# gorgonia/agogo

Measured on AMD Instinct MI355X. Metric: mcts_sims_per_sec, higher is better.
Workload: dtype f32 (Winograd F(5x5,3x3): fp32 transforms; transform-domain products as fp16x2 = each fp32 operand scaled by a power of two and split into 2 fp16 pieces (22-23 significand bits, absolute error <= 2^-38 of the tensor range), 3 fp16 MFMAs per product, fp32 accumulate)

## Files before the change

### agogo_amd/capi.py

```python
import ctypes as C
import os

import numpy as np

_HERE = os.path.dirname(os.path.abspath(__file__))
_LIB = None

NONE, BLACK, WHITE = 0, 1, 2
PASS, RESIGN = -1, -2
NO_MOVE = -32768
GAME_MNK, GAME_C4, GAME_KOMI, GAME_WQ = 0, 1, 2, 3
ENC_TWOPLANE, ENC_WQ = 0, 1
INF_NET, INF_DUMMY, INF_SCRIPT, INF_HASH, INF_UNIFORM, INF_CALLBACK = 0, 1, 2, 3, 4, 5
BN_DEGENERATE_EPS, BN_RUNNING, BN_IDENTITY = 0, 1, 2
COMPUTE_F32_MFMA, COMPUTE_BF16X3, COMPUTE_FP16X2, COMPUTE_WINO, COMPUTE_AUTO, COMPUTE_WINO_H2 = 0, 1, 2, 3, 4, 5
COMPUTE_FORCE = 0x100
LOSS_REFERENCE, LOSS_ALPHAZERO = 0, 1
PATH_FWD_F32, PATH_FWD_BF16X3, PATH_FWD_H2W, PATH_FWD_H2DMA, PATH_FWD_H2DMA3 = 1, 2, 3, 4, 5
PATH_WGRAD_F32, PATH_WGRAD_X3, PATH_WGRAD_H2, PATH_WGRAD_H2T3 = 1, 2, 3, 4
PATH_DGRAD_RAW, PATH_DGRAD_X3, PATH_DGRAD_WINO_H2 = 1, 2, 3
PATH_BN2_SCALAR, PATH_BN2_V = 1, 2
ROWS_WGRAD_CHUNKS, ROWS_SINGLE_PASS, ROWS_APPLY_RPB, ROWS_BWD2_RPB = 0, 1, 2, 3
ROWS_APPLY_BOARD_WORDS, ROWS_BWD2_BOARD_WORDS, ROWS_SPLIT_BLOCKS, ROWS_SPLIT_NEED = 4, 5, 6, 7
ROWS_HEAD_SECOND_FORM, ROWS_HEAD_CONV2_GRID, ROWS_HEAD_STATS_GRID, ROWS_HEAD_COST_GRID = 0, 1, 2, 3
# ... 148 lines not shown
    sig("agz_net_set_param", i32, vp, i32, pf, C.c_size_t)
    sig("agz_net_get_param", i32, vp, i32, pf, C.c_size_t)
    sig("agz_net_set_bn_stats", i32, vp, i32, pf, pf, C.c_size_t)
    sig("agz_net_init_random", i32, vp, u64)
    sig("agz_net_commit", i32, vp)
    sig("agz_net_infer", i32, vp, pf, i32, pf, pf)
    sig("agz_net_infer_dev", i32, vp, vp, i32, vp, vp)
    sig("agz_host_alloc", i32, vp, C.c_size_t, pvp)
    sig("agz_host_free", i32, vp, vp)
    sig("agz_mcts_to_dot", i32, vp, i32, C.c_char_p, C.c_size_t, C.POINTER(C.c_size_t))
    sig("agz_mcts_set_timeout_ms", i32, vp, i32)
    sig("agz_mcts_last_simulations", i32, vp, C.POINTER(C.c_int64))
    sig("agz_net_set_latency_mode", i32, vp, i32)
    sig("agz_net_set_tower_queues", i32, vp, i32)
    sig("agz_net_set_compute_mode", i32, vp, i32)
    sig("agz_net_flops_per_eval", f64, vp)
    sig("agz_net_save", i32, vp, C.c_char_p)
    sig("agz_net_load", i32, vp, C.c_char_p)
    sig("agz_arena_get_results", i32, vp, C.POINTER(C.c_int64), C.POINTER(C.c_int64), C.POINTER(C.c_int64))
    sig("agz_trainer_create", i32, vp, C.POINTER(NetConf), pvp)
    sig("agz_trainer_create_tied", i32, vp, C.POINTER(NetConf), pvp)
    sig("agz_trainer_is_tied", i32, vp, C.POINTER(i32))
    sig("agz_trainer_destroy", None, vp)
    sig("agz_trainer_num_params", i32, vp)
    sig("agz_trainer_param_info", i32, vp, i32, C.c_char_p, C.c_size_t, C.POINTER(C.c_size_t))
    sig("agz_trainer_set_param", i32, vp, i32, pf, C.c_size_t)
    sig("agz_trainer_get_param", i32, vp, i32, pf, C.c_size_t)
    sig("agz_trainer_get_grad", i32, vp, i32, pf, C.c_size_t)
    sig("agz_trainer_init_random", i32, vp, u64)
    sig("agz_trainer_batch", i32, vp, pf, pf, pf, C.c_float, pf)
    sig("agz_trainer_forward_backward", i32, vp, pf, pf, pf, pf)
    sig("agz_trainer_forward_backward_dev", i32, vp, vp, vp, vp, pf)
    sig("agz_trainer_apply", i32, vp, C.c_float, C.c_float)
    sig("agz_trainer_grads_dev", i32, vp, pvp, C.POINTER(C.c_size_t))
    sig("agz_trainer_set_solver", i32, vp, C.POINTER(SolverConf))
    sig("agz_trainer_get_solver", i32, vp, C.POINTER(SolverConf))
    sig("agz_trainer_get_velocity", i32, vp, i32, pf, C.c_size_t)
    sig("agz_trainer_set_velocity", i32, vp, i32, pf, C.c_size_t)
    sig("agz_trainer_reset_solver", i32, vp)
    sig("agz_trainer_set_adam", i32, vp, C.POINTER(AdamConf))
    sig("agz_trainer_get_adam", i32, vp, C.POINTER(AdamConf), C.POINTER(C.c_uint64))
    sig("agz_trainer_get_moments", i32, vp, i32, pf, pf, C.c_size_t)
    sig("agz_trainer_set_moments", i32, vp, i32, pf, pf, C.c_size_t)
    sig("agz_trainer_set_bn_tracking", i32, vp, i32, C.c_float)
    sig("agz_trainer_get_bn_tracking", i32, vp, C.POINTER(C.c_int), C.POINTER(C.c_float), C.POINTER(C.c_double))
    sig("agz_trainer_num_bn", i32, vp)
    sig("agz_trainer_get_bn_stats", i32, vp, i32, pf, pf, C.c_size_t)
    sig("agz_trainer_set_bn_stats", i32, vp, i32, pf, pf, C.c_size_t, C.c_double)
    sig("agz_trainer_reset_bn_stats", i32, vp)
    sig("agz_trainer_eval", i32, vp, pf, pf, pf, pf)
    sig("agz_trainer_eval_dev", i32, vp, vp, vp, vp, pf)
    sig("agz_trainer_set_loss", i32, vp, i32)
    sig("agz_trainer_get_loss", i32, vp, C.POINTER(C.c_int))
    sig("agz_trainer_get_costs", i32, vp, pf, pf)
    sig("agz_trainer_set_compute_mode", i32, vp, i32)
    sig("agz_train", i32, vp, pf, pf, pf, i32, i32, u64, pf)
    sig("agz_trainer_export", i32, vp, vp)
    sig("agz_trainer_save", i32, vp, C.c_char_p)
    sig("agz_trainer_load", i32, vp, C.c_char_p)
    sig("agz_arena_create", i32, vp, C.POINTER(GameConf), C.POINTER(MctsConf), i32, u64, i32, pvp)
    sig("agz_arena_destroy", None, vp)
    sig("agz_arena_set_inferencer", i32, vp, i32, i32, vp)
    sig("agz_arena_reset", i32, vp, pu8)
    sig("agz_arena_play", i32, vp, i32, i32)
    sig("agz_arena_selfplay", i32, vp, C.c_int64, i32)
    sig("agz_arena_set_parallel", i32, vp, i32)
    sig("agz_arena_set_leaf_symmetry", i32, vp, i32, u64)
    sig("agz_mcts_set_leaf_symmetry", i32, vp, i32, u64)
    sig("agz_symmetry_map", i32, i32, i32, pi)
    sig("agz_symmetry_inverse", i32, i32)
    sig("agz_leaf_symmetry_of", i32, u64, pi, i32, i32, C.POINTER(C.c_int))
    sig("agz_examples_augment_dihedral", i32, vp)
    sig("agz_symmetry_boards", i32, vp, pf, i32, i32, i32, pf)
    pnc, pu64 = C.POINTER(NoiseConf), C.POINTER(C.c_uint64)
    sig("agz_arena_set_root_noise", i32, vp, pnc)
    sig("agz_arena_get_root_noise", i32, vp, pnc)
    sig("agz_arena_root_noise", i32, vp, i32, i32, pu64, pi, pf, i32, C.POINTER(C.c_int))
    sig("agz_mcts_set_root_noise", i32, vp, pnc)
    sig("agz_mcts_root_noise", i32, vp, pu64, pi, pf, i32, C.POINTER(C.c_int))
    sig("agz_root_noise_of", i32, u64, i32, C.c_float, pf)
    ppc, pi32, pi64 = C.POINTER(PlayoutCapConf), C.POINTER(C.c_int32), C.POINTER(C.c_int64)
    sig("agz_arena_set_playout_cap", i32, vp, ppc)
    sig("agz_arena_get_playout_cap", i32, vp, ppc)
    sig("agz_arena_playout_cap", i32, vp, i32, pu64, pi32, pi32, pi32)
    sig("agz_arena_playout_cap_counts", i32, vp, pi64, pi64)
    sig("agz_playout_cap_of", i32, u64, u64, C.c_int32, C.c_float, pi32)
    pfc, pu8, pu32 = C.POINTER(ForcedConf), C.POINTER(C.c_uint8), C.POINTER(C.c_uint32)
    sig("agz_arena_set_forced_playouts", i32, vp, pfc)
    sig("agz_arena_get_forced_playouts", i32, vp, pfc)
    sig("agz_root_select_of", i32, pu32, pf, pf, pu8, i32, i32, C.c_float, C.c_float, C.POINTER(C.c_int), C.POINTER(C.c_int))
    sig("agz_pruned_target_of", i32, pi, pu32, pf, pf, i32, i32, i32, C.c_float, C.c_float, C.c_float, pu32, pf)
    ptc = C.POINTER(TargetConf)
    sig("agz_arena_set_policy_target", i32, vp, ptc)
    sig("agz_arena_get_policy_target", i32, vp, ptc)
    sig("agz_visit_target_of", i32, pi, C.POINTER(C.c_uint32), i32, i32, C.c_float, pf)
    sig("agz_arena_begin_move", i32, vp)
    sig("agz_arena_simulate", i32, vp, i32)
    sig("agz_arena_end_move", i32, vp, i32)
    sig("agz_arena_apply_moves", i32, vp, pi)
    sig("agz_arena_get_stats", i32, vp, C.POINTER(ArenaStats))
    sig("agz_arena_get_game", i32, vp, i32, pi, C.POINTER(GameState))
    sig("agz_arena_get_history", i32, vp, i32, pi, i32, pi)
    sig("agz_arena_root_children", i32, vp, i32, i32, pi, pu, pf, pf, i32, pi)
    sig("agz_arena_tree_nodes", i32, vp, i32, i32, pi)
    sig("agz_arena_get_examples", i32, vp, pf, pf, pf, pi, i32, pi)
    sig("agz_arena_clear_examples", i32, vp)
    sig("agz_arena_drop_labelled_examples", i32, vp)
    sig("agz_arena_examples_dev", i32, vp, pvp, pvp, pvp, pi)
    i64, pi64 = C.c_int64, C.POINTER(C.c_int64)
    sig("agz_train_dev", i32, vp, vp, vp, vp, i32, i32, u64, pf)
    sig("agz_examples_create", i32, vp, i32, i32, i32, i32, pvp)
    sig("agz_examples_destroy", None, vp)
    sig("agz_examples_count", i32, vp, pi64)
    sig("agz_examples_clear", i32, vp)
    sig("agz_examples_append_arena", i32, vp, vp)
    sig("agz_examples_append_dev", i32, vp, vp, vp, vp, i64)
    sig("agz_examples_append_host", i32, vp, pf, pf, pf, i64)
    sig("agz_examples_get", i32, vp, pf, pf, pf, i64, pi64)
    sig("agz_examples_augment_rotate", i32, vp)
    sig("agz_examples_prepare", i32, vp, i32, i32, u64, pi)
    sig("agz_examples_tensors_dev", i32, vp, pvp, pvp, pvp, pi64, pi)
    sig("agz_examples_get_tensors", i32, vp, pf, pf, pf)
    sig("agz_examples_raw_dev", i32, vp, pvp, pvp, pvp)
    sig("agz_replay_create", i32, vp, i32, i32, i32, i32, i64, pvp)
    sig("agz_replay_create_packed", i32, vp, i32, i32, i32, i32, i64, pf, i32, pvp)
    sig("agz_encoder_palette", i32, i32, pf, pi)
    sig("agz_replay_pack_host", i32, pf, i64, i32, i32, pf, i32, pu, pi64)
    sig("agz_replay_storage", i32, vp, pi, pi64, pi64)
    sig("agz_replay_destroy", None, vp)
    sig("agz_replay_count", i32, vp, pi64, C.POINTER(C.c_uint64), pi64)
    sig("agz_replay_clear", i32, vp)
    sig("agz_replay_append_examples", i32, vp, vp)
    sig("agz_replay_append_dev", i32, vp, vp, vp, vp, i64)
    sig("agz_replay_append_host", i32, vp, pf, pf, pf, i64)
    sig("agz_replay_get", i32, vp, i64, i64, pf, pf, pf)
    sig("agz_replay_sample_dev", i32, vp, i32, u64, u64, i32, vp, vp, vp)
    sig("agz_replay_sample", i32, vp, i32, u64, u64, i32, pf, pf, pf)
    sig("agz_replay_draw", i32, u64, u64, i32, i64, i32, pi64, pi)
    sig("agz_train_replay", i32, vp, vp, i32, u64, i32, pf)
    sig("agz_replay_sample_slice_dev", i32, vp, i32, i32, i32, u64, u64, i32, vp, vp, vp)
    sig("agz_replay_sample_slice", i32, vp, i32, i32, i32, u64, u64, i32, pf, pf, pf)
    sig("agz_replay_digest", i32, vp, C.POINTER(C.c_uint64))
    sig("agz_replay_digest_host", i32, pf, pf, pf, i64, i32, i32, i32, C.POINTER(C.c_uint64))
    sig("agz_replay_save", i32, vp, C.c_char_p)
    sig("agz_replay_load", i32, vp, C.c_char_p)
    sig("agz_replay_set_ckpt_staging", i32, vp, C.c_size_t)
    sig("agz_train_replay_sharded", i32, vp, vp, i32, u64, i32, i32, pf)
    sig("agz_rotate_boards", i32, vp, pf, i32, i32, i32, pf)
    sig("agz_ctx_prof_set_stride", i32, vp, i32, i32)
    sig("agz_wino_stages", i32, vp, pf, pf, i32, i32, i32, i32, i32, pf, pf)
    sig("agz_wino_h2_tile", i32, i32, i32)
    sig("agz_net_set_wino_h2_form", i32, vp, i32)
    sig("agz_net_set_wino_h2_gemm", i32, vp, i32)
    sig("agz_net_wino_h2_last_rows", i32, vp, C.POINTER(C.c_int), C.POINTER(C.c_int))
    sig("agz_net_last_paths", i32, vp, C.POINTER(C.c_int), C.POINTER(C.c_int), C.POINTER(C.c_int))
    sig("agz_net_tower_out", i32, vp, i32, pf)
    sig("agz_net_min_same_batch", i32, vp, i32, i32, C.POINTER(C.c_int))
    sig("agz_arena_set_prep_compact", i32, vp, i32)
    sig("agz_arena_set_split", i32, vp, i32)
    sig("agz_arena_split_steps", i32, vp, C.POINTER(C.c_int64), C.POINTER(C.c_int64), C.POINTER(C.c_int))
    sig("agz_trainer_set_dma_forward", i32, vp, i32)
    sig("agz_trainer_last_paths", i32, vp, i32, C.POINTER(C.c_int), C.POINTER(C.c_int), C.POINTER(C.c_int), C.POINTER(C.c_int))
    sig("agz_trainer_last_rows", i32, vp, i32, C.POINTER(C.c_int32))
    sig("agz_trainer_last_planes", i32, vp, i32, C.POINTER(C.c_int), C.POINTER(C.c_uint32), C.POINTER(C.c_uint32))
    sig("agz_arena_last_prep_batch", i32, vp, C.POINTER(C.c_int), C.POINTER(C.c_int))
    sig("agz_arena_set_cap_compact", i32, vp, i32)
    sig("agz_arena_last_cap_batch", i32, vp, C.POINTER(C.c_int), C.POINTER(C.c_int))
    sig("agz_arena_debug_counter", i32, vp, i32, C.POINTER(C.c_int64))
    sig("agz_arena_pool_capacity", i32, vp, C.POINTER(C.c_int), C.POINTER(C.c_int))
    sig("agz_wino_h2_chained", i32, i32, i32, i32)
    sig("agz_arena_random_moves", i32, vp, pi, u64)
    sig("agz_arena_set_state", i32, vp, i32, C.POINTER(State))
    sig("agz_arena_save", i32, vp, C.c_char_p)
    sig("agz_arena_load", i32, vp, C.c_char_p)
    sig("agz_arena_set_ckpt_staging", i32, vp, C.c_size_t)
    sig("agz_arena_examples_labelled_dev", i32, vp, pvp)
    sig("agz_mcts_create", i32, vp, C.POINTER(GameConf), C.POINTER(MctsConf), u64, i32, pvp)
    sig("agz_mcts_destroy", None, vp)
    sig("agz_mcts_set_inferencer", i32, vp, i32, vp)
    sig("agz_mcts_set_inferencer_callback", i32, vp, INFER_FN, vp, i32)
    sig("agz_arena_set_inferencer_callback", i32, vp, i32, INFER_FN, vp, i32)
    sig("agz_arena_set_pool_policy", i32, vp, i32)
    sig("agz_mcts_set_pool_policy", i32, vp, i32)
    sig("agz_mcts_set_parallel", i32, vp, i32)
    sig("agz_mcts_set_game", i32, vp, C.POINTER(State))
    sig("agz_mcts_search", i32, vp, i32, pi)
    sig("agz_mcts_policies", i32, vp, pf, i32)
    sig("agz_mcts_root_children", i32, vp, pi, pu, pf, pf, i32, pi)
    sig("agz_mcts_nodes", i32, vp, pi)
    sig("agz_mcts_children", i32, vp, i32, pi, pi, pu, pf, pf, i32, pi)
    sig("agz_mcts_get_stats", i32, vp, C.POINTER(ArenaStats))
    sig("agz_mcts_reset", i32, vp)
    sig("agz_comm_init_all", i32, pvp, i32, pvp)
    sig("agz_comm_unique_id", i32, vp)
    sig("agz_comm_init_rank", i32, vp, i32, i32, vp, pvp)
    sig("agz_comm_destroy", None, vp)
    sig("agz_comm_rank", i32, vp)
    sig("agz_comm_size", i32, vp)
    sig("agz_examples_allgather", i32, vp, vp)
    sig("agz_trainer_allreduce", i32, vp, vp)
    sig("agz_trainer_forward_backward_allreduce", i32, vp, vp, pf, pf, pf, pf)
    sig("agz_trainer_forward_backward_allreduce_dev", i32, vp, vp, vp, vp, vp, pf)
    sig("agz_comm_debug_fail_slice", i32, vp, i32)
    sig("agz_trainer_create_sharded", i32, vp, C.POINTER(NetConf), pvp)
    sig("agz_trainer_create_sharded_tied", i32, vp, C.POINTER(NetConf), pvp)
    sig("agz_trainer_shard", i32, vp, C.POINTER(i32), C.POINTER(i32), C.POINTER(i32))
    sig("agz_comm_debug_fail_layer", i32, vp, i32)
    _LIB = L
    return L


def _check(r, what=""):
    if r != 0:
        raise AgzError("%s failed (%d): %s" % (what, r, lib().agz_last_error().decode(errors="replace")))


def _pf(a):
    return a.ctypes.data_as(C.POINTER(C.c_float))


def _pi(a):
    return a.ctypes.data_as(C.POINTER(C.c_int32))


class Ctx:
    def __init__(self, device=0):
        self.h = C.c_void_p()
        self._children = []
        _check(lib().agz_ctx_create(device, C.byref(self.h)), "agz_ctx_create")

    def _adopt(self, child):
        import weakref
        self._children.append(weakref.ref(child))

    def close(self):
        if self.h:
            kids = [r() for r in self._children]
            for k in sorted([k for k in kids if k is not None], key=lambda k: 0 if isinstance(k, Arena) else 1):
                k.close()
            self._children = []
            for p in list(getattr(self, "_pinned", {}).values()):
                lib().agz_host_free(self.h, C.c_void_p(p))
            self._pinned = {}
            lib().agz_ctx_destroy(self.h)
            self.h = C.c_void_p()

    def __del__(self):
        try:
            self.close()
        except Exception:
            pass

    def host_array(self, shape, dtype=np.float32):
        n = int(np.prod(shape)) * np.dtype(dtype).itemsize
        p = C.c_void_p()
        _check(lib().agz_host_alloc(self.h, max(n, 1), C.byref(p)), "agz_host_alloc")
        arr = np.ctypeslib.as_array((C.c_char * max(n, 1)).from_address(p.value)).view(dtype)[: int(np.prod(shape))].reshape(shape)
        self._pinned = getattr(self, "_pinned", {})
        self._pinned[arr.ctypes.data] = p.value
        return arr

    def host_free(self, arr):
        p = getattr(self, "_pinned", {}).pop(arr.ctypes.data, None)
        if p is not None and self.h:
            _check(lib().agz_host_free(self.h, C.c_void_p(p)), "agz_host_free")

    def sync(self):
        _check(lib().agz_ctx_sync(self.h), "agz_ctx_sync")

    def stream(self):
        return lib().agz_ctx_stream(self.h)

    def prof_enable(self, on=True, classes=None):
        if on and classes is not None:
            mask = 0
            for k in classes:
                mask |= 1 << (k + 1)
            _check(lib().agz_ctx_prof_enable(self.h, mask), "agz_ctx_prof_enable")
            return
        return self._prof_enable_all(on)

    def prof_set_stride(self, klass, stride):
        _check(lib().agz_ctx_prof_set_stride(self.h, int(klass), int(stride)), "agz_ctx_prof_set_stride")

    def _prof_enable_all(self, on=True):
        _check(lib().agz_ctx_prof_enable(self.h, int(on)), "agz_ctx_prof_enable")

    def prof_read(self, klass):
        n, ms = C.c_int64(0), C.c_double(0)
        _check(lib().agz_ctx_prof_read(self.h, klass, C.byref(n), C.byref(ms)), "agz_ctx_prof_read")
        return n.value, ms.value


class Net:

    def __init__(self, ctx, K, SharedLayers, FC, Width, Height, Features, ActionSpace, BatchSize=256,
                 bn_mode=BN_DEGENERATE_EPS, bn_eps=1e-5):
        self.ctx = ctx
        self.conf = NetConf(K, SharedLayers, FC, BatchSize, Width, Height, Features, ActionSpace, bn_mode, bn_eps)
        self.h = C.c_void_p()
        _check(lib().agz_net_create(ctx.h, C.byref(self.conf), C.byref(self.h)), "agz_net_create")
        ctx._adopt(self)

    def close(self):
        if self.h and self.ctx.h:
            lib().agz_net_destroy(self.h)
        self.h = C.c_void_p()

    def __del__(self):
        try:
            self.close()
        except Exception:
            pass

    def num_params(self):
        return lib().agz_net_num_params(self.h)

    def param_info(self, i):
        name = C.create_string_buffer(128)
        n = C.c_size_t(0)
        _check(lib().agz_net_param_info(self.h, i, name, 128, C.byref(n)), "agz_net_param_info")
        return name.value.decode(), n.value

    def set_param(self, i, v):
        a = np.ascontiguousarray(v, dtype=np.float32).ravel()
        _check(lib().agz_net_set_param(self.h, i, _pf(a), a.size), "agz_net_set_param")

    def get_param(self, i):
        _, n = self.param_info(i)
        a = np.zeros(n, dtype=np.float32)
        _check(lib().agz_net_get_param(self.h, i, _pf(a), a.size), "agz_net_get_param")
        return a

    def set_bn_stats(self, bi, mean, var):
        m = np.ascontiguousarray(mean, dtype=np.float32)
        v = np.ascontiguousarray(var, dtype=np.float32)
        _check(lib().agz_net_set_bn_stats(self.h, bi, _pf(m), _pf(v), m.size), "agz_net_set_bn_stats")

    def init_random(self, seed):
        _check(lib().agz_net_init_random(self.h, seed), "agz_net_init_random")

    def commit(self):
        _check(lib().agz_net_commit(self.h), "agz_net_commit")

    def infer(self, planes):
        c = self.conf
        x = np.ascontiguousarray(planes, dtype=np.float32).reshape(-1, c.Features, c.Height, c.Width)
        B = x.shape[0]
        pol = np.zeros((B, c.ActionSpace), dtype=np.float32)
        val = np.zeros(B, dtype=np.float32)
        _check(lib().agz_net_infer(self.h, _pf(x), B, _pf(pol), _pf(val)), "agz_net_infer")
        return pol, val

    def set_compute_mode(self, mode):
        _check(lib().agz_net_set_compute_mode(self.h, int(mode)), "agz_net_set_compute_mode")

    def set_latency_mode(self, on=True):
        _check(lib().agz_net_set_latency_mode(self.h, int(on)), "agz_net_set_latency_mode")

    def set_tower_queues(self, queues):
        _check(lib().agz_net_set_tower_queues(self.h, int(queues)), "agz_net_set_tower_queues")

    def set_wino_h2_form(self, form):
        _check(lib().agz_net_set_wino_h2_form(self.h, int(form)), "agz_net_set_wino_h2_form")

    def set_wino_h2_gemm(self, variant):
        _check(lib().agz_net_set_wino_h2_gemm(self.h, int(variant)), "agz_net_set_wino_h2_gemm")

    def wino_h2_last_rows(self):
        r, c = C.c_int(0), C.c_int(0)
        _check(lib().agz_net_wino_h2_last_rows(self.h, C.byref(r), C.byref(c)), "agz_net_wino_h2_last_rows")
        return r.value, c.value

    def last_paths(self):
        i, b, h = C.c_int(0), C.c_int(0), C.c_int(0)
        _check(lib().agz_net_last_paths(self.h, C.byref(i), C.byref(b), C.byref(h)), "agz_net_last_paths")
        return i.value, b.value, h.value

    def tower_out(self, B):
        c = self.conf
        t = np.zeros((int(B), c.K, c.Height, c.Width), dtype=np.float32)
        _check(lib().agz_net_tower_out(self.h, int(B), _pf(t)), "agz_net_tower_out")
        return t

    def min_same_batch(self, n, G):
        b = C.c_int(0)
        _check(lib().agz_net_min_same_batch(self.h, int(n), int(G), C.byref(b)), "agz_net_min_same_batch")
        return b.value

    def infer_dev(self, planes_ptr, B, policy_ptr, value_ptr):
        _check(lib().agz_net_infer_dev(self.h, C.c_void_p(planes_ptr), B, C.c_void_p(policy_ptr),
                                       C.c_void_p(value_ptr)), "agz_net_infer_dev")

    def flops_per_eval(self):
        return lib().agz_net_flops_per_eval(self.h)

    def save(self, path):
        _check(lib().agz_net_save(self.h, os.fsencode(path)), "agz_net_save")

    def load(self, path):
        _check(lib().agz_net_load(self.h, os.fsencode(path)), "agz_net_load")


class Trainer:

    def __init__(self, ctx, K, SharedLayers, FC, Width, Height, Features, ActionSpace, BatchSize, bn_eps=1e-5, tied=False):
        self.ctx = ctx
        self.conf = NetConf(K, SharedLayers, FC, BatchSize, Width, Height, Features, ActionSpace, 0, bn_eps)
        self.h = C.c_void_p()
        if tied:
            _check(lib().agz_trainer_create_tied(ctx.h, C.byref(self.conf), C.byref(self.h)), "agz_trainer_create_tied")
        else:
            _check(lib().agz_trainer_create(ctx.h, C.byref(self.conf), C.byref(self.h)), "agz_trainer_create")
        ctx._adopt(self)

    def is_tied(self):
        v = C.c_int(0)
        _check(lib().agz_trainer_is_tied(self.h, C.byref(v)), "agz_trainer_is_tied")
        return bool(v.value)

    @classmethod
    def sharded(cls, ctx, comm, K, SharedLayers, FC, Width, Height, Features, ActionSpace, BatchSize, bn_eps=1e-5, tied=False):
        assert comm.ctx is ctx, "the communicator belongs to another context"
        self = cls.__new__(cls)
        self.ctx, self.comm = ctx, comm
        self.conf = NetConf(K, SharedLayers, FC, BatchSize, Width, Height, Features, ActionSpace, 0, bn_eps)
        self.h = C.c_void_p()
        if tied:
            _check(lib().agz_trainer_create_sharded_tied(comm.h, C.byref(self.conf), C.byref(self.h)), "agz_trainer_create_sharded_tied")
        else:
            _check(lib().agz_trainer_create_sharded(comm.h, C.byref(self.conf), C.byref(self.h)), "agz_trainer_create_sharded")
        ctx._adopt(self)
        return self

    def shard(self):
        r0, n, nr = C.c_int(0), C.c_int(0), C.c_int(0)
        _check(lib().agz_trainer_shard(self.h, C.byref(r0), C.byref(n), C.byref(nr)), "agz_trainer_shard")
        return r0.value, n.value, nr.value

    def close(self):
        if self.h and self.ctx.h:
            lib().agz_trainer_destroy(self.h)
        self.h = C.c_void_p()

    def __del__(self):
        try:
            self.close()
        except Exception:
            pass

    def num_params(self):
        return lib().agz_trainer_num_params(self.h)

    def param_info(self, i):
        name = C.create_string_buffer(128)
        n = C.c_size_t(0)
        _check(lib().agz_trainer_param_info(self.h, i, name, 128, C.byref(n)), "agz_trainer_param_info")
        return name.value.decode(), n.value

    def set_param(self, i, v):
        a = np.ascontiguousarray(v, dtype=np.float32).ravel()
        _check(lib().agz_trainer_set_param(self.h, i, _pf(a), a.size), "agz_trainer_set_param")

    def get_param(self, i):
        a = np.zeros(self.param_info(i)[1], np.float32)
        _check(lib().agz_trainer_get_param(self.h, i, _pf(a), a.size), "agz_trainer_get_param")
        return a

    def get_grad(self, i):
        a = np.zeros(self.param_info(i)[1], np.float32)
        _check(lib().agz_trainer_get_grad(self.h, i, _pf(a), a.size), "agz_trainer_get_grad")
        return a

    def init_random(self, seed):
        _check(lib().agz_trainer_init_random(self.h, seed), "agz_trainer_init_random")

    def batch(self, planes, pi, v, lr=0.1):
        x = np.ascontiguousarray(planes, np.float32)
        p = np.ascontiguousarray(pi, np.float32)
        vv = np.ascontiguousarray(v, np.float32)
        c = C.c_float(0)
        _check(lib().agz_trainer_batch(self.h, _pf(x), _pf(p), _pf(vv), lr, C.byref(c)), "agz_trainer_batch")
        return c.value

    def forward_backward(self, planes, pi, v):
        x = np.ascontiguousarray(planes, np.float32)
        p = np.ascontiguousarray(pi, np.float32)
        vv = np.ascontiguousarray(v, np.float32)
        c = C.c_float(0)
        _check(lib().agz_trainer_forward_backward(self.h, _pf(x), _pf(p), _pf(vv), C.byref(c)), "agz_trainer_forward_backward")
        return c.value

    def forward_backward_dev(self, planes_ptr, pi_ptr, v_ptr, want_cost=True):
        c = C.c_float(0)
        _check(lib().agz_trainer_forward_backward_dev(self.h, C.c_void_p(planes_ptr), C.c_void_p(pi_ptr), C.c_void_p(v_ptr),
                                                      C.byref(c) if want_cost else None), "agz_trainer_forward_backward_dev")
        return c.value if want_cost else None

    def apply(self, lr=0.1, grad_scale=1.0):
        _check(lib().agz_trainer_apply(self.h, lr, grad_scale), "agz_trainer_apply")

    def set_solver(self, momentum=0.0, l2reg=0.0, clip=0.0, reserved=0):
        sc = SolverConf(momentum, l2reg, clip, reserved)
        _check(lib().agz_trainer_set_solver(self.h, C.byref(sc)), "agz_trainer_set_solver")

    def get_solver(self):
        sc = SolverConf()
        _check(lib().agz_trainer_get_solver(self.h, C.byref(sc)), "agz_trainer_get_solver")
        return {"momentum": sc.momentum, "l2reg": sc.l2reg, "clip": sc.clip}

    def get_velocity(self, i):
        a = np.zeros(self.param_info(i)[1], np.float32)
        _check(lib().agz_trainer_get_velocity(self.h, i, _pf(a), a.size), "agz_trainer_get_velocity")
        return a

    def set_velocity(self, i, v):
        a = np.ascontiguousarray(v, dtype=np.float32).ravel()
        _check(lib().agz_trainer_set_velocity(self.h, i, _pf(a), a.size), "agz_trainer_set_velocity")

    def reset_solver(self):
        _check(lib().agz_trainer_reset_solver(self.h), "agz_trainer_reset_solver")
# ... 938 lines not shown
```

### agogo_amd/csrc/conv_wino_h2c.hpp

```cpp
#pragma once

__device__ __forceinline__ unsigned h2c_img(int row, int slot) { return maps::h2c_img(row, slot); }

template <int NK, int PFA>
__global__ __launch_bounds__(256, 2) void wino_gemm_h2c_kernel(WinoH2Args h) {
  const WinoArgs& a = h.w;
  constexpr int SA = 128 * 128, SB = 256 * 128;
  __shared__ __attribute__((aligned(16))) unsigned char lds[SA + SB];

  const int n_nt = a.Ntot >> 8;
  const int per_pos = a.n_mtiles * n_nt;
  const int nblk = h.npos * per_pos;
  const int id = blockIdx.x;
  int q = nblk >> 3, rr = nblk & 7, xcd = id & 7, slot = id >> 3;
  int tile = (xcd < rr ? xcd * (q + 1) : rr * (q + 1) + (xcd - rr) * q) + slot;
  const int pos = tile / per_pos;
  const int rem = tile - pos * per_pos;
  const int m_tile = rem / n_nt, n_tile = rem - m_tile * n_nt;

  const int tid = threadIdx.x, lane = tid & 63, wid = tid >> 6;
  const int wm = wid >> 1, wn = wid & 1;
  const unsigned st_lds = h2c_img(tid >> 3, tid & 7);
  const char* abase = reinterpret_cast<const char*>(a.V) + ((size_t)m_tile * h.npos + pos) * (size_t)NK * SA + (size_t)tid * 16;
  const char* bbase = reinterpret_cast<const char*>(h.U2c) + (((size_t)pos * NK) * n_nt + n_tile) * (size_t)SB + (size_t)tid * 16;
// ... 370 lines not shown
  const unsigned m_slot = (unsigned)h.npos * m_pos;
  const unsigned m_lane = (unsigned)((t0 >> 7) - sl0) * m_slot + (unsigned)(((tc & 127) * 64 + pr * 4) * 4);
  const int bpt = 128 / a.TPB;
  auto m_row = [&](int cls, int S) -> unsigned {
    const int idx = maps::rows_row(cls, a.nty, a.ntx, 0, ty, tx);
    if (idx < 0) return 0x80000000u;
    const int p = maps::pack_slot_row(S, bpt, maps::rows_per_board(cls, a.nty, a.ntx), b, idx);
    return (unsigned)((p >> 7) - sl0) * m_slot + (unsigned)(((p & 127) * 64 + pr * 4) * 4);
  };
  const unsigned m_lane_r = h.live_r ? m_row(maps::ROWS_R, h.pk.S_r) : m_lane, m_lane_c = h.live_c ? m_row(maps::ROWS_C, h.pk.S_c) : m_lane;
  auto m_voff = [&](int xi, int nu) -> unsigned {
    const int cls = maps::rows_class(true, true, AL, xi, nu);
    return cls == maps::ROWS_R ? m_lane_r : (cls == maps::ROWS_C ? m_lane_c : m_lane);
  };
  float Y[TM][TM][4];
#pragma unroll
  for (int k = 0; k < TM; k++)
#pragma unroll
    for (int l = 0; l < TM; l++)
#pragma unroll
      for (int e = 0; e < 4; e++) Y[k][l][e] = 0.f;
  float4 m[2][AL];
#pragma unroll
  for (int xi = 0; xi < AL; xi++) m[0][xi] = h2_ldf4(mr, m_voff(xi, 0), (unsigned)(xi * AL) * m_pos);
#pragma unroll
  for (int nu = 0; nu < AL; nu++) {
    if (nu + 1 < AL) {
#pragma unroll
      for (int xi = 0; xi < AL; xi++) m[(nu + 1) & 1][xi] = h2_ldf4(mr, m_voff(xi, nu + 1), (unsigned)(xi * AL + nu + 1) * m_pos);
    }
    float mm[4][AL], oo[4][TM];
#pragma unroll
    for (int xi = 0; xi < AL; xi++) { const float4 v = m[nu & 1][xi]; mm[0][xi] = v.x; mm[1][xi] = v.y; mm[2][xi] = v.z; mm[3][xi] = v.w; }
#pragma unroll
    for (int e = 0; e < 4; e++) wino_atv<TM>(mm[e], oo[e]);
#pragma unroll
    for (int k = 0; k < TM; k++)
#pragma unroll
      for (int e = 0; e < 4; e++) {
        float yl[TM];
#pragma unroll
        for (int l = 0; l < TM; l++) yl[l] = Y[k][l][e];
        wino_at_acc<TM>(nu, yl, oo[e][k]);
#pragma unroll
        for (int l = 0; l < TM; l++) Y[k][l][e] = yl[l];
      }
    __builtin_amdgcn_sched_barrier(0);
  }
  const char* ep = reinterpret_cast<const char*>(a.ep);
  const unsigned e_lane = (unsigned)(32 * s + 2 * pr) * 16u, e_pix = (unsigned)a.Cout_p * 16u;
  float mx = 0.f;
  float* yb = LAST ? a.y + (size_t)b * a.Hp * a.Wp * a.Cout_p + 32 * s + 2 * pr : nullptr;
#pragma unroll
  for (int k = 0; k < TM; k++) {
    const int hh = TM * ty + k, hc = hh < a.H ? hh : a.H - 1;
#pragma unroll
    for (int l = 0; l < TM; l++) {
      const int ww = TM * tx + l, wc = ww < a.W ? ww : a.W - 1;
      const char* e = ep + (size_t)(hc * a.W + wc) * e_pix + e_lane;
      const float4 E0 = *reinterpret_cast<const float4*>(e), E1 = *reinterpret_cast<const float4*>(e + 16);
      float va = (Y[k][l][0] * un0) * E0.x + E0.y, vb = (Y[k][l][1] * un0) * E0.z + E0.w;
      float vc = (Y[k][l][2] * un0) * E1.x + E1.y, vd = (Y[k][l][3] * un0) * E1.z + E1.w;
      va = va > 0.f ? va : 0.f; vb = vb > 0.f ? vb : 0.f; vc = vc > 0.f ? vc : 0.f; vd = vd > 0.f ? vd : 0.f;
      const float y0 = va + vb, y1 = vc + vd;
      if (live && hh < a.H && ww < a.W) {
        if (LAST) *reinterpret_cast<float2*>(yb + ((size_t)(hh + 1) * a.Wp + (ww + 1)) * a.Cout_p) = make_float2(y0, y1);
        else *reinterpret_cast<float2*>(&ys[((size_t)bl * HW + hh * a.W + ww) * 32 + 2 * pr]) = make_float2(y0, y1);
        mx = fmaxf(mx, fmaxf(y0, y1));
      }
    }
    __builtin_amdgcn_sched_barrier(0);
  }
  if (LAST) return;
#pragma unroll
  for (int o = 8; o > 0; o >>= 1) mx = fmaxf(mx, __shfl_xor(mx, o, 64));
  if (pr == 0 && live) h.wm_out[(size_t)t * NS + s] = mx;
  float ax;
  if (h.amax_true) ax = __uint_as_float(reinterpret_cast<const unsigned*>(h.amax_true)[b]);
  else {
    const int wmpb = a.TPB * NS;
    const float* wp = h.wm_prev + (size_t)b * wmpb;
    ax = 0.f;
    for (int i = pr; i < wmpb; i += 16) ax = fmaxf(ax, wp[i]);
#pragma unroll
    for (int o = 8; o > 0; o >>= 1) ax = fmaxf(ax, __shfl_xor(ax, o, 64));
  }
  const float bound = h.g1 * ax + h.g0;
  const unsigned bbits = __float_as_uint(bound);
  if (s == 0 && tt == 0 && pr == 0 && live) h.amax_next[b] = bbits;
  float sb, inv_;
  wino_h2_scales(bbits, WT::VSHIFT, &sb, &inv_);
  __syncthreads();
  const float* yl = ys + (size_t)bl * HW * 32 + 2 * pr;
  float tmx[AL][AL], tmy[AL][AL];
#pragma unroll
  for (int j = 0; j < AL; j++) {
    const int ww = TM * tx + j - 1;
    const bool okx = ww >= 0 && ww < a.W;
    const int wc = ww < 0 ? 0 : (ww < a.W ? ww : a.W - 1);
    float dx[AL], dy[AL], ox[AL], oy[AL];
#pragma unroll
    for (int i = 0; i < AL; i++) {
      const int hh = TM * ty + i - 1;
      const bool ok = okx && hh >= 0 && hh < a.H;
      const int hc = hh < 0 ? 0 : (hh < a.H ? hh : a.H - 1);
      const float2 d = *reinterpret_cast<const float2*>(yl + (size_t)(hc * a.W + wc) * 32);
      dx[i] = ok ? d.x : 0.f; dy[i] = ok ? d.y : 0.f;
    }
    wino_btv<TM>(dx, ox);
    wino_btv<TM>(dy, oy);
#pragma unroll
    for (int i = 0; i < AL; i++) { tmx[i][j] = ox[i]; tmy[i][j] = oy[i]; }
  }
  const float sv = live ? sb : 0.f;
  const __amdgpu_buffer_rsrc_t vr = h2_rsrc(reinterpret_cast<const char*>(a.V) + ((size_t)(t0 >> 7) * h.npos * NS + s) * 16384);
  const unsigned v_lane = (unsigned)(((t0 & 127) + (tid >> 6) * 4) * 128 + lane * 4);
  const unsigned v_pos = (unsigned)NS * 16384u;
#pragma unroll
  for (int i = 0; i < AL; i++) {
    float ox[AL], oy[AL];
    wino_btv<TM>(tmx[i], ox);
    wino_btv<TM>(tmy[i], oy);
#pragma unroll
    for (int j = 0; j < AL; j++) {
      unsigned lo;
      const unsigned hi = wino_h2_pack(ox[j] * sv, oy[j] * sv, &lo);
      const auto s16 = __builtin_amdgcn_permlane16_swap(hi, lo, false, false);
      const unsigned e0 = s16[0], e1 = s16[1];
      const auto s32 = __builtin_amdgcn_permlane32_swap(e0, e1, false, false);
      const unsigned w0 = s32[0], w1 = s32[1];
      __builtin_amdgcn_raw_buffer_store_b32(w0, vr, v_lane, (unsigned)(i * AL + j) * v_pos, 0);
      __builtin_amdgcn_raw_buffer_store_b32(w1, vr, v_lane + 256u, (unsigned)(i * AL + j) * v_pos, 0);
    }
  }
}

typedef float f2c __attribute__((ext_vector_type(2)));
template <int TM> __device__ __forceinline__ void wino_atv_p(const f2c* m, f2c* o);
template <> __device__ __forceinline__ void wino_atv_p<4>(const f2c* m, f2c* o) {
  const f2c s12 = m[1] + m[2], d12 = m[1] - m[2], s34 = m[3] + m[4], d34 = m[3] - m[4];
  o[0] = m[0] + s12 + s34;
  o[1] = d12 + 2.f * d34;
  o[2] = s12 + 4.f * s34;
  o[3] = d12 + 8.f * d34 + m[5];
}
template <> __device__ __forceinline__ void wino_atv_p<5>(const f2c* m, f2c* o) {
  const f2c s12 = m[1] + m[2], d12 = m[1] - m[2], s34 = m[3] + m[4], d34 = m[3] - m[4];
  o[0] = m[0] + s12 + s34 + m[5];
  o[1] = d12 + 0.5f * d34 + 2.f * m[5];
  o[2] = s12 + 0.25f * s34 + 4.f * m[5];
  o[3] = d12 + 0.125f * d34 + 8.f * m[5];
  o[4] = s12 + 0.0625f * s34 + 16.f * m[5] + m[6];
}
template <int TM> __device__ __forceinline__ void wino_at_acc_p(int nu, f2c* Y, f2c t);
template <> __device__ __forceinline__ void wino_at_acc_p<5>(int nu, f2c* Y, f2c t) {
  switch (nu) {
    case 0: Y[0] += t; break;
    case 1: Y[0] += t; Y[1] += t; Y[2] += t; Y[3] += t; Y[4] += t; break;
    case 2: Y[0] += t; Y[1] -= t; Y[2] += t; Y[3] -= t; Y[4] += t; break;
    case 3: Y[0] += t; Y[1] += 0.5f * t; Y[2] += 0.25f * t; Y[3] += 0.125f * t; Y[4] += 0.0625f * t; break;
    case 4: Y[0] += t; Y[1] -= 0.5f * t; Y[2] += 0.25f * t; Y[3] -= 0.125f * t; Y[4] += 0.0625f * t; break;
    case 5: Y[0] += t; Y[1] += 2.f * t; Y[2] += 4.f * t; Y[3] += 8.f * t; Y[4] += 16.f * t; break;
    default: Y[4] += t; break;
  }
}
template <> __device__ __forceinline__ void wino_at_acc_p<4>(int nu, f2c* Y, f2c t) {
  switch (nu) {
    case 0: Y[0] += t; break;
    case 1: Y[0] += t; Y[1] += t; Y[2] += t; Y[3] += t; break;
    case 2: Y[0] += t; Y[1] -= t; Y[2] += t; Y[3] -= t; break;
    case 3: Y[0] += t; Y[1] += 2.f * t; Y[2] += 4.f * t; Y[3] += 8.f * t; break;
    case 4: Y[0] += t; Y[1] -= 2.f * t; Y[2] += 4.f * t; Y[3] -= 8.f * t; break;
    default: Y[3] += t; break;
  }
}
template <int TM> __device__ __forceinline__ f2c wino_bt_row_p(int i, const f2c* d);
template <> __device__ __forceinline__ f2c wino_bt_row_p<5>(int i, const f2c* d) {
  switch (i) {
    case 0: return -0.5f * d[0] + 0.25f * d[1] + 2.5f * d[2] - 1.25f * d[3] - 2.f * d[4] + d[5];
    case 1: return 0.5f * d[1] + 0.25f * d[2] - 2.25f * d[3] - d[4] + d[5];
    case 2: return -0.5f * d[1] + 0.75f * d[2] + 1.75f * d[3] - 3.f * d[4] + d[5];
    case 3: return d[1] + 1.5f * d[2] - 2.f * d[3] - 1.5f * d[4] + d[5];
    case 4: return -d[1] + 2.5f * (d[2] - d[4]) + d[5];
    case 5: return 0.25f * d[1] - 1.25f * d[3] + d[5];
    default: return -0.5f * d[1] + 0.25f * d[2] + 2.5f * d[3] - 1.25f * d[4] - 2.f * d[5] + d[6];
  }
}
template <> __device__ __forceinline__ f2c wino_bt_row_p<4>(int i, const f2c* d) {
  switch (i) {
    case 0: return 4.f * d[0] - 5.f * d[2] + d[4];
    case 1: return -4.f * d[1] - 4.f * d[2] + d[3] + d[4];
    case 2: return 4.f * d[1] - 4.f * d[2] - d[3] + d[4];
    case 3: return -2.f * d[1] - d[2] + 2.f * d[3] + d[4];
    case 4: return 2.f * d[1] - d[2] - 2.f * d[3] + d[4];
    default: return 4.f * d[1] - 5.f * d[3] + d[5];
  }
}
template <int TM> __device__ __forceinline__ void wino_btv_p(const f2c* d, f2c* o) {
#pragma unroll
  for (int i = 0; i < TM + 2; i++) o[i] = wino_bt_row_p<TM>(i, d);
}

template <int TM, bool NT = true>
__global__ __launch_bounds__(256, 2) void wino_oip_h2c_kernel(WinoH2Args h) {
  constexpr int MAUX = 0, VAUX = NT ? 2 : 0;
  using WT = WinoT<TM>;
  constexpr int AL = WT::AL, NPRE = AL - 3;
  const WinoArgs& a = h.w;
  extern __shared__ __attribute__((aligned(16))) float ys[];
  const int tid = threadIdx.x, tl = tid >> 4, pr = tid & 15, lane = tid & 63;
  const int NS = a.C >> 5;
  const int PH = TM * a.nty + 2, PW = TM * a.ntx + 2;
  const int bpg = 16 / a.TPB;
  const int n_groups = (a.T + 15) >> 4, n_items = n_groups * NS;
  const int tt = tl % a.TPB, bl = tl / a.TPB;
  const int ty = tt / a.ntx, tx = tt - ty * a.ntx;
  for (int i = tid; i < bpg * PH * PW * 32; i += 256) ys[i] = 0.f;
  const __amdgpu_buffer_rsrc_t mr = h2_rsrc(a.Mb);
  const __amdgpu_buffer_rsrc_t vr = h2_rsrc(a.V);
  const unsigned m_lane = (unsigned)((tl * 64 + pr * 4) * 4);
  const unsigned v_lane = (unsigned)((((tid >> 6) * 4) * 128) + lane * 4);
  const unsigned e_pix = (unsigned)a.Cout_p * 16u;
  constexpr unsigned OOB = 0x80000000u;
  const int S_r = h.pk.S_r, S_c = h.pk.S_c;
  const unsigned m_dq = (unsigned)(h.npos * NS - 1) * 32768u, v_dq = (unsigned)(h.npos * NS - 1) * 16384u;
  const unsigned gr_r = h.live_r ? (unsigned)(bpg * maps::rows_per_board(maps::ROWS_R, a.nty, a.ntx)) : 16u;
  const unsigned gr_c = h.live_c ? (unsigned)(bpg * maps::rows_per_board(maps::ROWS_C, a.nty, a.ntx)) : 16u;
  auto m_row = [&](int cls) -> unsigned {
    const int r = maps::rows_row(cls, a.nty, a.ntx, bl, ty, tx);
    return r < 0 ? OOB : (unsigned)((r * 64 + pr * 4) * 4);
  };
  auto v_row = [&](int cls, int k) -> unsigned {
    const int tv = (tid >> 6) * 4 + 2 * k + (lane >> 5), ttv = tv % a.TPB;
    const int r = maps::rows_row(cls, a.nty, a.ntx, tv / a.TPB, ttv / a.ntx, ttv % a.ntx);
    return r < 0 ? OOB : (unsigned)(r * 128 + (lane & 31) * 4);
  };
  const unsigned m_lane_r = h.live_r ? m_row(maps::ROWS_R) : m_lane, m_lane_c = h.live_c ? m_row(maps::ROWS_C) : m_lane;
  const unsigned v0_r = h.live_r ? v_row(maps::ROWS_R, 0) : v_lane, v1_r = h.live_r ? v_row(maps::ROWS_R, 1) : v_lane + 256u;
  const unsigned v0_c = h.live_c ? v_row(maps::ROWS_C, 0) : v_lane, v1_c = h.live_c ? v_row(maps::ROWS_C, 1) : v_lane + 256u;
  float* const ybase = ys + ((size_t)bl * PH * PW + (size_t)(TM * ty) * PW + TM * tx) * 32 + 2 * pr;
  unsigned okmask = 0;
#pragma unroll
  for (int k = 0; k < TM; k++)
#pragma unroll
    for (int l = 0; l < TM; l++) okmask |= (TM * ty + k < a.H && TM * tx + l < a.W) ? 1u << (k * TM + l) : 0u;
  const __amdgpu_buffer_rsrc_t er = h2_rsrc(a.ep);
  float4 m[NPRE][AL];
  auto m_soff = [&](int g, int s, int xi, int nu) -> unsigned {
    const int cls = maps::rows_class(true, true, AL, xi, nu);
    const unsigned gr = cls == maps::ROWS_R ? gr_r : (cls == maps::ROWS_C ? gr_c : 16u);
    const int S = cls == maps::ROWS_R ? S_r : (cls == maps::ROWS_C ? S_c : 1);
    return (unsigned)(((maps::pack_group_slot0(S, g) * h.npos + xi * AL + nu) * NS + s)) * 32768u + maps::pack_group_rg0(S, g, gr) * 256u;
  };
  auto m_voff = [&](int g, int xi, int nu) -> unsigned {
    const int cls = maps::rows_class(true, true, AL, xi, nu);
    if (cls == maps::ROWS_R) return m_lane_r + maps::pack_q(S_r, maps::pack_group_rg0(S_r, g, gr_r), m_lane_r, 8) * m_dq;
    if (cls == maps::ROWS_C) return m_lane_c + maps::pack_q(S_c, maps::pack_group_rg0(S_c, g, gr_c), m_lane_c, 8) * m_dq;
    return m_lane;
  };
  int item = blockIdx.x;
  {
    const int g = __builtin_amdgcn_readfirstlane(item / NS), s = __builtin_amdgcn_readfirstlane(item - (item / NS) * NS);
#pragma unroll
    for (int nu = 0; nu < NPRE; nu++)
#pragma unroll
      for (int xi = 0; xi < AL; xi++) m[nu][xi] = h2_ldf4<MAUX>(mr, m_voff(g, xi, nu), m_soff(g, s, xi, nu));
  }
  __syncthreads();
  for (; item < n_items; item += gridDim.x) {
    const int g = __builtin_amdgcn_readfirstlane(item / NS), s = __builtin_amdgcn_readfirstlane(item - (item / NS) * NS);
    const int t = g * 16 + tl;
    const bool live = t < a.T;
    const int b = live ? g * bpg + bl : (a.T - 1) / a.TPB;
    float s_, un0;
    wino_h2_scales(h.amax_in[b], WT::VSHIFT, &s_, &un0);
    f2c Y[TM][TM][2];
#pragma unroll
    for (int k = 0; k < TM; k++)
#pragma unroll
      for (int l = 0; l < TM; l++) { Y[k][l][0] = f2c{0.f, 0.f}; Y[k][l][1] = f2c{0.f, 0.f}; }
#pragma unroll
    for (int nu = 0; nu < AL; nu++) {
      f2c c0[AL], c1[AL], o0[TM], o1[TM];
#pragma unroll
      for (int xi = 0; xi < AL; xi++) {
        const float4 v = m[nu % NPRE][xi];
        c0[xi] = f2c{v.x, v.y}; c1[xi] = f2c{v.z, v.w};
      }
      if (nu + NPRE < AL) {
#pragma unroll
        for (int xi = 0; xi < AL; xi++) m[nu % NPRE][xi] = h2_ldf4<MAUX>(mr, m_voff(g, xi, nu + NPRE), m_soff(g, s, xi, nu + NPRE));
      }
      wino_atv_p<TM>(c0, o0);
      wino_atv_p<TM>(c1, o1);
#pragma unroll
      for (int k = 0; k < TM; k++) {
        f2c y0[TM], y1[TM];
#pragma unroll
        for (int l = 0; l < TM; l++) { y0[l] = Y[k][l][0]; y1[l] = Y[k][l][1]; }
        wino_at_acc_p<TM>(nu, y0, o0[k]);
        wino_at_acc_p<TM>(nu, y1, o1[k]);
#pragma unroll
        for (int l = 0; l < TM; l++) { Y[k][l][0] = y0[l]; Y[k][l][1] = y1[l]; }
      }
      __builtin_amdgcn_sched_barrier(0);
    }
    __builtin_amdgcn_sched_barrier(0);
    unsigned e_base = (unsigned)(32 * s + 2 * pr) * 16u + (unsigned)((TM * ty) * a.W + TM * tx) * e_pix;
    asm volatile("" : "+v"(e_base));
    float4 E[2][TM][2];
    auto load_e = [&](int buf, int k) {
#pragma unroll
      for (int l = 0; l < TM; l++) {
        const bool ok = (okmask >> (k * TM + l)) & 1u;
        const unsigned off = e_base + (ok ? (unsigned)(k * a.W + l) * e_pix : 0u);
        E[buf][l][0] = h2_ldf4(er, off, 0);
        E[buf][l][1] = h2_ldf4(er, off + 16u, 0);
      }
    };
    load_e(0, 0);
    float mxv = 0.f;
    float* yw = ybase;
    asm volatile("" : "+v"(yw));
#pragma unroll
    for (int k = 0; k < TM; k++) {
      if (k + 1 < TM) load_e((k + 1) & 1, k + 1);
#pragma unroll
      for (int l = 0; l < TM; l++) {
        const bool ok = live && ((okmask >> (k * TM + l)) & 1u);
        const float4 E0 = E[k & 1][l][0], E1 = E[k & 1][l][1];
        const f2c u0 = Y[k][l][0] * un0, u1 = Y[k][l][1] * un0;
        float va = u0.x * E0.x + E0.y, vb = u0.y * E0.z + E0.w;
        float vc = u1.x * E1.x + E1.y, vd = u1.y * E1.z + E1.w;
        va = va > 0.f ? va : 0.f; vb = vb > 0.f ? vb : 0.f; vc = vc > 0.f ? vc : 0.f; vd = vd > 0.f ? vd : 0.f;
        const float y0 = ok ? va + vb : 0.f, y1 = ok ? vc + vd : 0.f;
        *reinterpret_cast<float2*>(yw + ((k + 1) * PW + l + 1) * 32) = make_float2(y0, y1);
        mxv = fmaxf(mxv, fmaxf(y0, y1));
      }
      __builtin_amdgcn_sched_barrier(0);
    }
#pragma unroll
    for (int o = 8; o > 0; o >>= 1) mxv = fmaxf(mxv, __shfl_xor(mxv, o, 64));
    if (pr == 0 && live) h.wm_out[(size_t)t * NS + s] = mxv;
    float ax;
    if (h.amax_true) ax = __uint_as_float(reinterpret_cast<const unsigned*>(h.amax_true)[b]);
    else {
      const int wmpb = a.TPB * NS;
      const float* wp = h.wm_prev + (size_t)b * wmpb;
      ax = 0.f;
      for (int i = pr; i < wmpb; i += 16) ax = fmaxf(ax, wp[i]);
#pragma unroll
      for (int o = 8; o > 0; o >>= 1) ax = fmaxf(ax, __shfl_xor(ax, o, 64));
    }
    const float bound = h.g1 * ax + h.g0;
    const unsigned bbits = __float_as_uint(bound);
    if (s == 0 && tt == 0 && pr == 0 && live) h.amax_next[b] = bbits;
    float sb, inv_;
    wino_h2_scales(bbits, WT::VSHIFT, &sb, &inv_);
    const float sv = live ? sb : 0.f;
    __syncthreads();
    {
      const int nx = item + (int)gridDim.x < n_items ? item + (int)gridDim.x : item;
      const int g2 = __builtin_amdgcn_readfirstlane(nx / NS), s2 = __builtin_amdgcn_readfirstlane(nx - (nx / NS) * NS);
#pragma unroll
      for (int nu = 0; nu < NPRE; nu++)
#pragma unroll
        for (int xi = 0; xi < AL; xi++) m[nu][xi] = h2_ldf4<MAUX>(mr, m_voff(g2, xi, nu), m_soff(g2, s2, xi, nu));
    }
    __builtin_amdgcn_sched_barrier(0);
    const unsigned v_pos = (unsigned)NS * 16384u;
    const unsigned v_slot = (unsigned)h.npos * v_pos;
    const unsigned rg0_r = maps::pack_group_rg0(S_r, g, gr_r), rg0_c = maps::pack_group_rg0(S_c, g, gr_c);
    const unsigned v_g = (unsigned)(g >> 3) * v_slot + (unsigned)s * 16384u + (unsigned)(g & 7) * 2048u;
    const unsigned v_g_r = maps::pack_group_slot0(S_r, g) * v_slot + (unsigned)s * 16384u + rg0_r * 128u;
    const unsigned v_g_c = maps::pack_group_slot0(S_c, g) * v_slot + (unsigned)s * 16384u + rg0_c * 128u;
    auto v_voff = [&](int cls, int k) -> unsigned {
      if (cls == maps::ROWS_R) { const unsigned o = k ? v1_r : v0_r; return o + maps::pack_q(S_r, rg0_r, o, 7) * v_dq; }
      if (cls == maps::ROWS_C) { const unsigned o = k ? v1_c : v0_c; return o + maps::pack_q(S_c, rg0_c, o, 7) * v_dq; }
      return k ? v_lane + 256u : v_lane;
    };
    const float* yr = ybase;
    asm volatile("" : "+v"(yr));
#pragma unroll
    for (int i0 = 0; i0 < AL; i0 += 3) {
      constexpr int NRMAX = 3;
      const int nr = AL - i0 < NRMAX ? AL - i0 : NRMAX;
      f2c tmr[NRMAX][AL];
#pragma unroll
      for (int j = 0; j < AL; j++) {
        f2c d[AL];
#pragma unroll
        for (int ii = 0; ii < AL; ii++) {
          const float2 v = *reinterpret_cast<const float2*>(yr + (ii * PW + j) * 32);
          d[ii] = f2c{v.x, v.y};
        }
#pragma unroll
        for (int r = 0; r < NRMAX; r++)
          if (r < nr) tmr[r][j] = wino_bt_row_p<TM>(i0 + r, d);
      }
      __builtin_amdgcn_sched_barrier(0);
#pragma unroll
      for (int r = 0; r < NRMAX; r++) {
        if (r >= nr) continue;
        const int i = i0 + r;
        f2c o[AL];
        wino_btv_p<TM>(tmr[r], o);
#pragma unroll
        for (int j = 0; j < AL; j++) {
          unsigned lo;
          const unsigned hi = wino_h2_pack(o[j].x * sv, o[j].y * sv, &lo);
          const auto s16 = __builtin_amdgcn_permlane16_swap(hi, lo, false, false);
          const unsigned e0 = s16[0], e1 = s16[1];
          const auto s32 = __builtin_amdgcn_permlane32_swap(e0, e1, false, false);
          const unsigned w0 = s32[0], w1 = s32[1];
          const int cls = maps::rows_class(true, true, AL, i, j);
          const unsigned v_so = (cls == maps::ROWS_R ? v_g_r : (cls == maps::ROWS_C ? v_g_c : v_g)) + (unsigned)(i * AL + j) * v_pos;
          __builtin_amdgcn_raw_buffer_store_b32(w0, vr, v_voff(cls, 0), v_so, VAUX);
          __builtin_amdgcn_raw_buffer_store_b32(w1, vr, v_voff(cls, 1), v_so, VAUX);
        }
      }
      __builtin_amdgcn_sched_barrier(0);
    }
    __syncthreads();
  }
}

static void wino_build_u2c(const std::vector<_Float16>& u2, std::vector<_Float16>& u2c, int npos, int Ntot, int C, int Cout_p) {
  const int NC = C / 32, NT = Ntot / 256;
  u2c.assign(u2.size(), (_Float16)0.f);
  for (int pos = 0; pos < npos; pos++)
    for (int kc = 0; kc < NC; kc++)
      for (int nn = 0; nn < Ntot; nn++) {
        const int s = nn >> 6, j2 = nn & 63, ch = 32 * s + (j2 >> 1), br = j2 & 1, n = br * Cout_p + ch;
        for (int p = 0; p < 2; p++) {
          const _Float16* src = &u2[((((size_t)pos * NC + kc) * 2 + p) * Ntot + n) * 32];
          _Float16* dst = &u2c[((((size_t)pos * NC + kc) * NT + (nn >> 8)) * 256 + (nn & 255)) * 64 + p * 32];
          for (int k = 0; k < 32; k++) dst[k] = src[k];
        }
      }
}

static inline bool wino_h2c_ok(int H, int W, int tm, int Kp) {
  const int tpb = ceil_div(H, tm) * ceil_div(W, tm);
  const int nk = Kp / 32;
  return Kp % 128 == 0 && 16 % tpb == 0 && (nk == 4 || nk == 8 || nk == 12 || nk == 16) &&
         (size_t)(16 / tpb) * (tm * ceil_div(H, tm) + 2) * (tm * ceil_div(W, tm) + 2) * 128 <= 80 * 1024;
}

static void wino_h2c_geometry(WinoH2Args& h) {
  WinoArgs& a = h.w;
  const int tm = h.tm == 5 ? 5 : 4;
  h.tm = tm; h.npos = (tm + 2) * (tm + 2);
  a.nty = ceil_div(a.H, tm); a.ntx = ceil_div(a.W, tm); a.TPB = a.nty * a.ntx; a.T = a.B * a.TPB;
  h.rsh = 7; h.rmask = 127; h.rA = (unsigned)h.npos * 128u; h.rB = 128u;
  a.n_mtiles = ceil_div(a.T, 128); a.n_ntiles = ceil_div(a.Ntot, 128);
  h.in_swap = 1; h.cform = 1; h.wm_per_board = 0;
  h.pk = maps::pack_grid(tm + 2, a.nty, a.ntx, a.B, a.Ntot >> 8, h.live_r, h.live_c);
}
static int wino_h2c_gemm_tiles(const WinoH2Args& h) {
  int n = 0;
  for (int pos = 0; pos < h.npos; pos++) n += maps::pack_pos_used(h.pk, pos);
  return n * h.pk.n_nt;
}
constexpr int WINO_H2_GEMM_DEFAULT = 1;
static inline int wino_h2c_gemm_variant(const WinoH2Args& h) { return h.gemm_variant > 0 ? h.gemm_variant : WINO_H2_GEMM_DEFAULT; }
static inline bool wino_h2c_dma_ok(const WinoH2Args& h) {
  return wino_h2_rows(h.npos, (size_t)h.w.T) * h.w.C * 4 < ((size_t)1 << 31) && (size_t)h.npos * h.w.C * h.w.Ntot * 4 < ((size_t)1 << 31);
}
static inline bool wino_h2c_fits31(const WinoH2Args& h) { return wino_h2_rows(h.npos, (size_t)h.w.T) * h.w.Ntot * 4 < ((size_t)1 << 31); }
static bool wino_h2c_oip_ready(agz_ctx* ctx) {
  if (!(ctx->func_attr_state & 2u)) {
    const bool ok = hipFuncSetAttribute(reinterpret_cast<const void*>(&wino_oip_h2c_kernel<5>), hipFuncAttributeMaxDynamicSharedMemorySize, 80 * 1024) == hipSuccess &&
                    hipFuncSetAttribute(reinterpret_cast<const void*>(&wino_oip_h2c_kernel<4>), hipFuncAttributeMaxDynamicSharedMemorySize, 80 * 1024) == hipSuccess;
    if (!ok) (void)hipGetLastError();
    ctx->func_attr_state |= 2u | (ok ? 1u : 0u);
  }
  return (ctx->func_attr_state & 1u) != 0;
}
static void wino_h2c_rows(agz_ctx* ctx, WinoH2Args& h, int oi_variant, bool keep_all) {
  wino_h2c_geometry(h);
  h.live_r = h.live_c = 0;
  const int gemm = wino_h2c_gemm_variant(h) & 15;
  const maps::WinoRows g = maps::wino_rows(h.w.H, h.w.W, h.tm);
  if (keep_all || gemm != 1 || oi_variant != 4 || !wino_h2c_dma_ok(h) || !wino_h2c_fits31(h) || !maps::rows_short_ok(g) || !wino_h2c_oip_ready(ctx)) return;
  h.live_r = g.dead_y ? maps::rows_slot_live(g, maps::ROWS_R) : 0;
  h.live_c = g.dead_x ? maps::rows_slot_live(g, maps::ROWS_C) : 0;
  wino_h2c_geometry(h);
}
static void wino_h2c_in(agz_ctx* ctx, WinoH2Args& h, hipStream_t st) {
  wino_h2c_geometry(h);
  h.fuse_prev = 0; h.amax_self = const_cast<unsigned*>(h.amax_in);
  ProfScopeOn ps(ctx, AGZ_PROF_WINO_IN, st == ctx->stream.raw());
  const size_t n_in = (size_t)h.w.T * (h.w.C / 2);
  if (h.tm == 5) hipLaunchKernelGGL(wino_in_h2_kernel<5>, dim3((unsigned)((n_in + 255) / 256)), dim3(256), 0, st, h);
  else hipLaunchKernelGGL(wino_in_h2_kernel<4>, dim3((unsigned)((n_in + 255) / 256)), dim3(256), 0, st, h);
}
static void wino_h2c_gemm(agz_ctx* ctx, WinoH2Args& h, hipStream_t st) {
  wino_h2c_geometry(h);
  ProfScopeOn ps(ctx, AGZ_PROF_WINO_GEMM, st == ctx->stream.raw());
  const dim3 g(h.npos * h.w.n_mtiles * (h.w.Ntot >> 8));
  const bool dma_ok = wino_h2c_dma_ok(h);
  const int variant_all = wino_h2c_gemm_variant(h);
  const int variant = variant_all & 15, mode = (variant_all >> 4) & 3;
  const int n_slabs = h.w.Ntot >> 7;
  if (variant == 2 && dma_ok && (h.w.C >> 5) == 8 && h.w.Ntot % 256 == 0 && ctx->num_cus / 8 >= n_slabs) {
    const dim3 gp((unsigned)(8 * ((ctx->num_cus / 8) / n_slabs) * n_slabs));
    switch (mode) {
      case 1: hipLaunchKernelGGL(wino_gemm_h2p_kernel<1>, gp, dim3(256), 0, st, h); break;
      case 2: hipLaunchKernelGGL(wino_gemm_h2p_kernel<2>, gp, dim3(256), 0, st, h); break;
      case 3: hipLaunchKernelGGL(wino_gemm_h2p_kernel<3>, gp, dim3(256), 0, st, h); break;
      default: hipLaunchKernelGGL(wino_gemm_h2p_kernel<0>, gp, dim3(256), 0, st, h); break;
    }
    return;
  }
  const dim3 gd((unsigned)wino_h2c_gemm_tiles(h));
  if (dma_ok && h.temporal_stores && (h.w.C >> 5) == 8) { hipLaunchKernelGGL((wino_gemm_h2g_kernel<8, false>), gd, dim3(256), 0, st, h); return; }
  if (dma_ok) {
    switch (h.w.C >> 5) {
      case 4: hipLaunchKernelGGL((wino_gemm_h2g_kernel<4>), gd, dim3(256), 0, st, h); return;
      case 8: hipLaunchKernelGGL((wino_gemm_h2g_kernel<8>), gd, dim3(256), 0, st, h); return;
      case 12: hipLaunchKernelGGL((wino_gemm_h2g_kernel<12>), gd, dim3(256), 0, st, h); return;
      default: hipLaunchKernelGGL((wino_gemm_h2g_kernel<16>), gd, dim3(256), 0, st, h); return;
    }
  }
  switch (h.w.C >> 5) {
    case 4: hipLaunchKernelGGL((wino_gemm_h2c_kernel<4, 2>), g, dim3(256), 0, st, h); break;
    case 8: hipLaunchKernelGGL((wino_gemm_h2c_kernel<8, 2>), g, dim3(256), 0, st, h); break;
    case 12: hipLaunchKernelGGL((wino_gemm_h2c_kernel<12, 2>), g, dim3(256), 0, st, h); break;
    default: hipLaunchKernelGGL((wino_gemm_h2c_kernel<16, 2>), g, dim3(256), 0, st, h); break;
  }
}
static void wino_h2c_oi(agz_ctx* ctx, WinoH2Args& h, bool last, hipStream_t st, int variant = 4) {
  wino_h2c_geometry(h);
  ProfScopeOn ps(ctx, AGZ_PROF_WINO_OUT, st == ctx->stream.raw());
  const WinoArgs& a = h.w;
  const dim3 g((unsigned)ceil_div(a.T, 16), (unsigned)(a.C >> 5));
  const size_t shm = last ? 0 : (size_t)(16 / a.TPB) * a.H * a.W * 32 * sizeof(float);
  const bool fits31 = wino_h2c_fits31(h);
  if (variant == 4 && !last && fits31 && wino_h2c_oip_ready(ctx)) {
    const size_t shp = (size_t)(16 / a.TPB) * (h.tm * a.nty + 2) * (h.tm * a.ntx + 2) * 32 * sizeof(float);
    const int items = ceil_div(a.T, 16) * (a.C >> 5);
    const dim3 gp((unsigned)std::min(items, 2 * ctx->num_cus));
    if (h.tm == 5 && h.temporal_stores) {
      (void)hipFuncSetAttribute(reinterpret_cast<const void*>(&wino_oip_h2c_kernel<5, false>), hipFuncAttributeMaxDynamicSharedMemorySize, 80 * 1024);
      hipLaunchKernelGGL((wino_oip_h2c_kernel<5, false>), gp, dim3(256), shp, st, h);
      return;
    }
    if (h.tm == 5) hipLaunchKernelGGL((wino_oip_h2c_kernel<5>), gp, dim3(256), shp, st, h);
    else hipLaunchKernelGGL((wino_oip_h2c_kernel<4>), gp, dim3(256), shp, st, h);
    return;
  }
  if (h.tm == 5) {
    if (last) hipLaunchKernelGGL((wino_oi_h2c_kernel<5, true>), g, dim3(256), shm, st, h);
    else hipLaunchKernelGGL((wino_oi_h2c_kernel<5, false>), g, dim3(256), shm, st, h);
  } else {
    if (last) hipLaunchKernelGGL((wino_oi_h2c_kernel<4, true>), g, dim3(256), shm, st, h);
    else hipLaunchKernelGGL((wino_oi_h2c_kernel<4, false>), g, dim3(256), shm, st, h);
  }
}
```

### agogo_amd/csrc/conv_x3.hpp

```cpp
#pragma once

typedef short bf16x8_t __attribute__((ext_vector_type(8)));
typedef unsigned u32x4_t __attribute__((ext_vector_type(4)));

__device__ __forceinline__ void x3_split(float v, unsigned& h, unsigned& m, unsigned& l) {
  unsigned hu = __float_as_uint(v) & 0xffff0000u;
  float r = v - __uint_as_float(hu);
  unsigned mu = __float_as_uint(r) & 0xffff0000u;
  float r2 = r - __uint_as_float(mu);
  h = hu; m = mu; l = __float_as_uint(r2);
}
__device__ __forceinline__ unsigned x3_pack(unsigned e0, unsigned e1) { return __builtin_amdgcn_perm(e1, e0, 0x07060302u); }

__device__ __forceinline__ unsigned x3_lds_off(int row, int half) { return (unsigned)(row * 32 + ((half ^ ((row >> 3) & 1)) << 4)); }

__device__ __forceinline__ void x3_amax_flush(unsigned* amax, int b, float m, int lane) {
#pragma unroll
  for (int o = 16; o > 0; o >>= 1) m = fmaxf(m, __shfl_xor(m, o, 64));
  if ((lane & 31) == 0) atomicMax(&amax[b], __float_as_uint(m));
}
#define X3_EPILOGUE \
  int amx_b = -1; float amx_m = 0.f;    \
  _Pragma("unroll") \
  for (int i = 0; i < 2; i++) { \
  _Pragma("unroll") \
    for (int r = 0; r < 16; r++) { \
      int row = (wm * 2 + i) * 32 + (r & 3) + 8 * (r >> 2) + 4 * (lane >> 5); \
      int m = m0 + row; \
      const bool mvalid = m < a.M; \
      if (!mvalid) m = a.M - 1; \
      int b = m / a.HW, p = m - b * a.HW; \
      int h = p / a.W, w = p - h * a.W; \
      size_t obase = ((size_t)b * a.HpWp + (h + 1) * a.Wp + (w + 1)) * a.Cout_p; \
      if (DUAL) { \
        int c = n_tile * (BNT / 2) + wn * 32 + (lane & 31); \
        if (mvalid && c < a.Cout_p) { \
          float4 e = reinterpret_cast<const float4*>(a.ep)[(size_t)p * a.Cout_p + c]; \
          float va = acc[i][0][r] * e.x + e.y; \
          float vb = acc[i][1][r] * e.z + e.w; \
          va = va > 0.f ? va : 0.f; \
          vb = vb > 0.f ? vb : 0.f; \
          float s = va + vb; \
          a.y[obase + c] = s > 0.f ? s : 0.f; \
        } \
      } else { \
        if (a.amax_out && mvalid && b != amx_b) {    \
          if (amx_b >= 0) x3_amax_flush(a.amax_out, amx_b, amx_m, lane); \
          amx_b = b; amx_m = 0.f; \
        } \
  _Pragma("unroll") \
        for (int j = 0; j < 2; j++) { \
          int c = n0 + (wn * 2 + j) * 32 + (lane & 31); \
          if (mvalid && c < a.Cout_p) { \
            if (a.raw) { \
              a.y[obase + c] = acc[i][j][r]; \
            } else { \
              float2 e = reinterpret_cast<const float2*>(a.ep)[(size_t)p * a.Cout_p + c]; \
              float v = acc[i][j][r] * e.x + e.y; \
              v = v > 0.f ? v : 0.f; \
              a.y[obase + c] = v; \
              amx_m = fmaxf(amx_m, v); \
            } \
          } \
        } \
      } \
    } \
  } \
  if (!DUAL && a.amax_out && amx_b >= 0) x3_amax_flush(a.amax_out, amx_b, amx_m, lane);

template <bool DUAL>
__global__ __launch_bounds__(256, 3) void conv3x3_x3_kernel(ConvArgs a, const unsigned short* __restrict__ w3) {
  constexpr int BM = 128, BNT = 128;
  constexpr int PIECE = 128 * 32;
  constexpr int STAGE = 6 * PIECE;
  __shared__ __attribute__((aligned(16))) unsigned char lds[2 * STAGE];

  const int nblk = a.n_mtiles * a.n_ntiles;
  const int id = blockIdx.x;
  int q = nblk >> 3, rr = nblk & 7, xcd = id & 7, slot = id >> 3;
  int tile = (xcd < rr ? xcd * (q + 1) : rr * (q + 1) + (xcd - rr) * q) + slot;
  const int m_tile = tile / a.n_ntiles, n_tile = tile - m_tile * a.n_ntiles;
  const int m0 = m_tile * BM, n0 = n_tile * BNT;

  const int tid = threadIdx.x, lane = tid & 63, wid = tid >> 6;
  const int wm = wid >> 1, wn = wid & 1;

  const int srow = tid >> 1, shalf = tid & 1;
  int a_goff;
  {
    int m = m0 + srow;
    if (m >= a.M) m = a.M - 1;
    int b = m / a.HW, p = m - b * a.HW;
    int h = p / a.W, w = p - h * a.W;
    a_goff = ((b * a.HpWp) + (h + 1) * a.Wp + (w + 1)) * a.Cin_p + shalf * 8;
  }
  int nrow = n0 + srow;
  if (nrow >= a.Ntot) nrow = a.Ntot - 1;
  const int b_goff = nrow * 16 + shalf * 8;
  const size_t piece_stride = (size_t)a.Ntot * 16;
  const unsigned s_off = x3_lds_off(srow, shalf);
  const int NC = a.Cin_p >> 4;
  const int NK = 9 * NC;

  f32x16 acc[2][2];
#pragma unroll
  for (int i = 0; i < 2; i++)
#pragma unroll
    for (int j = 0; j < 2; j++)
#pragma unroll
      for (int r = 0; r < 16; r++) acc[i][j][r] = 0.f;

  unsigned fa[2], fb[2];
#pragma unroll
  for (int i = 0; i < 2; i++) fa[i] = x3_lds_off((wm * 2 + i) * 32 + (lane & 31), lane >> 5);
  if (DUAL) {
    fb[0] = x3_lds_off(wn * 32 + (lane & 31), lane >> 5);
    fb[1] = x3_lds_off(64 + wn * 32 + (lane & 31), lane >> 5);
  } else {
    fb[0] = x3_lds_off((wn * 2 + 0) * 32 + (lane & 31), lane >> 5);
    fb[1] = x3_lds_off((wn * 2 + 1) * 32 + (lane & 31), lane >> 5);
  }

  float4 xa0, xa1, ya0, ya1;
  u32x4_t xb0, xb1, xb2, yb0, yb1, yb2;
  const char* xbase = reinterpret_cast<const char*>(a.x);
  const char* wbase = reinterpret_cast<const char*>(w3);
  const unsigned a_gbyte = (unsigned)a_goff * 4u, b_gbyte = (unsigned)b_goff * 2u;
  const unsigned piece_bytes = (unsigned)(piece_stride * 2);
  int f_kx = 0, f_ky = 0, f_n = 0;
  const unsigned row_step = (unsigned)(a.Cin_p * 4), line_step = (unsigned)((a.Wp - 2) * a.Cin_p * 4);
  const unsigned chunk_back = (unsigned)((2 * a.Wp + 2) * a.Cin_p * 4) - 64u;
  unsigned xo_ = a_gbyte - (unsigned)((a.Wp + 1) * a.Cin_p * 4), wo_ = b_gbyte;
#define X3_ADVANCE()                                                                          \
  if (f_n + 1 < NK) {       \
    f_n++;                                                                                    \
    wo_ += 3u * piece_bytes;                                                                  \
    if (f_kx < 2) { f_kx++; xo_ += row_step; }                                                \
    else if (f_ky < 2) { f_kx = 0; f_ky++; xo_ += line_step; }                                \
    else { f_kx = 0; f_ky = 0; xo_ -= chunk_back; }                                           \
  }
#define X3_GLOAD(A0, A1, B0, B1, B2)                                                          \
  A0 = *reinterpret_cast<const float4*>(xbase + xo_);                                         \
  A1 = *reinterpret_cast<const float4*>(xbase + xo_ + 16u);                                   \
  B0 = *reinterpret_cast<const u32x4_t*>(wbase + wo_);                                        \
  B1 = *reinterpret_cast<const u32x4_t*>(wbase + wo_ + piece_bytes);                          \
  B2 = *reinterpret_cast<const u32x4_t*>(wbase + wo_ + 2u * piece_bytes);                     \
  X3_ADVANCE()
#define X3_STORE_A(A0, A1, BUF)                                                              \
  {                                                                                          \
    unsigned char* st_ = lds + (BUF) * STAGE;                                                \
    const float v_[8] = {A0.x, A0.y, A0.z, A0.w, A1.x, A1.y, A1.z, A1.w};                    \
    unsigned h_[8], m_[8], l_[8];                                                            \
    _Pragma("unroll") for (int e = 0; e < 8; e++) x3_split(v_[e], h_[e], m_[e], l_[e]);      \
    u32x4_t ph_ = {x3_pack(h_[0], h_[1]), x3_pack(h_[2], h_[3]), x3_pack(h_[4], h_[5]), x3_pack(h_[6], h_[7])}; \
    u32x4_t pm_ = {x3_pack(m_[0], m_[1]), x3_pack(m_[2], m_[3]), x3_pack(m_[4], m_[5]), x3_pack(m_[6], m_[7])}; \
    u32x4_t pl_ = {x3_pack(l_[0], l_[1]), x3_pack(l_[2], l_[3]), x3_pack(l_[4], l_[5]), x3_pack(l_[6], l_[7])}; \
    *reinterpret_cast<u32x4_t*>(st_ + 0 * PIECE + s_off) = ph_;                              \
    *reinterpret_cast<u32x4_t*>(st_ + 1 * PIECE + s_off) = pm_;                              \
    *reinterpret_cast<u32x4_t*>(st_ + 2 * PIECE + s_off) = pl_;                              \
  }
#define X3_STORE_B(B0, B1, B2, BUF)                                                          \
  {                                                                                          \
    unsigned char* st_ = lds + (BUF) * STAGE;                                                \
    *reinterpret_cast<u32x4_t*>(st_ + 3 * PIECE + s_off) = B0;                               \
    *reinterpret_cast<u32x4_t*>(st_ + 4 * PIECE + s_off) = B1;                               \
    *reinterpret_cast<u32x4_t*>(st_ + 5 * PIECE + s_off) = B2;                               \
  }
#define X3_SB
#define X3_MF(I, J, PA, PB) acc[I][J] = __builtin_amdgcn_mfma_f32_32x32x16_bf16(A_[I][PA], B_[J][PB], acc[I][J], 0, 0, 0);
#define X3_QUAD(PA, PB) X3_MF(0, 0, PA, PB) X3_MF(0, 1, PA, PB) X3_MF(1, 0, PA, PB) X3_MF(1, 1, PA, PB)
#define X3_ITER(BUF, XA0, XA1, XB0, XB1, XB2, YA0, YA1, YB0, YB1, YB2)                       \
  {                                                                                          \
    const unsigned char* st = lds + (BUF) * STAGE;                                           \
    bf16x8_t A_[2][3], B_[2][3];                                                             \
    _Pragma("unroll") for (int p = 0; p < 3; p++) {                                          \
      _Pragma("unroll") for (int i = 0; i < 2; i++) A_[i][p] = *reinterpret_cast<const bf16x8_t*>(st + p * PIECE + fa[i]);       \
      _Pragma("unroll") for (int j = 0; j < 2; j++) B_[j][p] = *reinterpret_cast<const bf16x8_t*>(st + (3 + p) * PIECE + fb[j]); \
    }                                                                                        \
    X3_SB                                                                                    \
    X3_QUAD(2, 0) X3_SB                                                                      \
    X3_GLOAD(YA0, YA1, YB0, YB1, YB2) X3_SB                                                  \
    X3_QUAD(0, 2) X3_SB                                                                      \
    X3_STORE_A(XA0, XA1, (BUF) ^ 1) X3_SB                                                    \
    X3_QUAD(1, 1) X3_QUAD(1, 0) X3_SB                                                        \
    X3_STORE_B(XB0, XB1, XB2, (BUF) ^ 1) X3_SB                                               \
    X3_QUAD(0, 1) X3_QUAD(0, 0) X3_SB                                                        \
    __syncthreads();                                                                         \
  }

  X3_GLOAD(ya0, ya1, yb0, yb1, yb2)
  X3_GLOAD(xa0, xa1, xb0, xb1, xb2)
  X3_STORE_A(ya0, ya1, 0)
  X3_STORE_B(yb0, yb1, yb2, 0)
  __syncthreads();
  for (int it = 0; it < NK; it += 2) {
    X3_ITER(0, xa0, xa1, xb0, xb1, xb2, ya0, ya1, yb0, yb1, yb2)
    if (it + 1 < NK) X3_ITER(1, ya0, ya1, yb0, yb1, yb2, xa0, xa1, xb0, xb1, xb2)
  }

  X3_EPILOGUE
}
```

### agogo_amd/csrc/net.hip

```cpp
#include "net.hpp"
#include "gemm_maps.hpp"

#include <cmath>
#include <cstdio>
#include <cstring>
#include <type_traits>

typedef float f32x16 __attribute__((ext_vector_type(16)));
typedef float f32x4 __attribute__((ext_vector_type(4)));

namespace agz {

struct ConvArgs {
  const float* x;
  const float* w;
  const void* ep;
  float* y;
  int M, HW, W, Wp, HpWp;
  int Cin_p, Cout_p, Ntot;
  int n_mtiles, n_ntiles;
  int raw;
  int splits;
  int per;
  float* ws;
  const unsigned* amax_in;
  float w_unscale;
  const unsigned* w_amax_dev;
  unsigned* amax_out;
};

__device__ __forceinline__ int swz_off(int row, int chunk) { return row * 32 + ((chunk ^ ((row >> 1) & 7)) << 2); }

template <int WM, int WN, int MT, bool DUAL>
__device__ __forceinline__ void conv_tile(const ConvArgs& a, float* lds, const int m0, const int n_tile, const int split) {
  constexpr int BM = WM * MT * 32;
  constexpr int BNT = WN * 64;
  static_assert(WM * WN == 4, "4 waves");
  constexpr int STAGE = (BM + BNT) * 32;
  const int n0 = n_tile * BNT;

  const int tid = threadIdx.x, lane = tid & 63, wid = tid >> 6;
  const int wm = wid / WN, wn = wid % WN;

  constexpr int A_PER_T = BM * 8 / 256;
  constexpr int B_PER_T = BNT * 8 / 256;
  static_assert((A_PER_T == 4 || A_PER_T == 2) && (B_PER_T == 4 || B_PER_T == 2), "staging layout");
  const int chunk = tid & 7;
  int a_goff[A_PER_T], a_loff[A_PER_T];
#pragma unroll
  for (int i = 0; i < A_PER_T; i++) {
    int row = (tid >> 3) + 32 * i;
    int m = m0 + row;
    if (m >= a.M) m = a.M - 1;
    int b = m / a.HW, p = m - b * a.HW;
    int h = p / a.W, w = p - h * a.W;
    a_goff[i] = ((b * a.HpWp) + (h + 1) * a.Wp + (w + 1)) * a.Cin_p + chunk * 4;
    a_loff[i] = swz_off(row, chunk);
  }
  int b_goff[B_PER_T], b_loff[B_PER_T];
#pragma unroll
  for (int i = 0; i < B_PER_T; i++) {
    int row = (tid >> 3) + 32 * i;
    int n = n0 + row;
    if (n >= a.Ntot) n = a.Ntot - 1;
    b_goff[i] = n * a.Cin_p + chunk * 4;
    b_loff[i] = swz_off(row, chunk);
  }
  const int NC = a.Cin_p >> 5;
  const int NKall = 9 * NC;
  const int it0 = split * a.per;
  const int NK = (it0 + a.per < NKall) ? it0 + a.per : NKall;
  const int w_tap_stride = a.Ntot * a.Cin_p;

  float4 ra0, ra1, ra2, ra3, rb0, rb1, rb2, rb3;
  float4 sa0, sa1, sa2, sa3, sb0, sb1, sb2, sb3;
  int xo_, wo_;
#define AGZ_TILE_OFFS(IT)                                                                   \
  {                                                                                         \
    int t_ = (IT) < NK ? (IT) : NK - 1;                                                     \
    int tap_ = t_ / NC, cc_ = t_ - tap_ * NC;                                               \
    int ky_ = tap_ / 3, kx_ = tap_ - ky_ * 3;                                               \
    xo_ = ((ky_ - 1) * a.Wp + (kx_ - 1)) * a.Cin_p + cc_ * 32;                              \
    wo_ = tap_ * w_tap_stride + cc_ * 32;                                                   \
  }
#define AGZ_GLA(R, I) if constexpr ((I) < A_PER_T) R = *reinterpret_cast<const float4*>(a.x + a_goff[(I) < A_PER_T ? (I) : 0] + xo_);
#define AGZ_GLB(R, I) if constexpr ((I) < B_PER_T) R = *reinterpret_cast<const float4*>(a.w + b_goff[(I) < B_PER_T ? (I) : 0] + wo_);
#define AGZ_LSA(R, I, BUF) if constexpr ((I) < A_PER_T) *reinterpret_cast<float4*>(lds + (BUF) * STAGE + a_loff[(I) < A_PER_T ? (I) : 0]) = R;
#define AGZ_LSB(R, I, BUF) if constexpr ((I) < B_PER_T) *reinterpret_cast<float4*>(lds + (BUF) * STAGE + BM * 32 + b_loff[(I) < B_PER_T ? (I) : 0]) = R;
#define AGZ_SB __builtin_amdgcn_sched_barrier(0);

  f32x16 acc[MT][2];
#pragma unroll
  for (int i = 0; i < MT; i++)
#pragma unroll
    for (int j = 0; j < 2; j++)
#pragma unroll
      for (int r = 0; r < 16; r++) acc[i][j][r] = 0.f;

  int a_row[MT], b_row[2];
#pragma unroll
  for (int i = 0; i < MT; i++) a_row[i] = (wm * MT + i) * 32 + (lane & 31);
  if (DUAL) {
    b_row[0] = wn * 32 + (lane & 31);
    b_row[1] = WN * 32 + wn * 32 + (lane & 31);
  } else {
    b_row[0] = (wn * 2 + 0) * 32 + (lane & 31);
    b_row[1] = (wn * 2 + 1) * 32 + (lane & 31);
  }
  const int khalf = lane >> 5;

  const unsigned lds_base = (unsigned)(size_t)((__attribute__((address_space(3))) float*)lds);
  unsigned a_addr[MT], b_addr[2], a_sw[MT], b_sw[2];
#pragma unroll
  for (int i = 0; i < MT; i++) { a_addr[i] = lds_base + a_row[i] * 128; a_sw[i] = (a_row[i] >> 1) & 7; }
#pragma unroll
  for (int j = 0; j < 2; j++) { b_addr[j] = lds_base + BM * 128 + b_row[j] * 128; b_sw[j] = (b_row[j] >> 1) & 7; }
  f32x4 f0a[MT], f0b[2], f1a[MT], f1b[2];
#pragma unroll
  for (int i = 0; i < MT; i++) { f0a[i] = f32x4{0.f, 0.f, 0.f, 0.f}; f1a[i] = f0a[i]; }
#pragma unroll
  for (int j = 0; j < 2; j++) { f0b[j] = f32x4{0.f, 0.f, 0.f, 0.f}; f1b[j] = f0b[j]; }
#define AGZ_LDSR(DST, ADDR) asm volatile("ds_read_b128 %0, %1" : "+v"(DST) : "v"(ADDR));
#define AGZ_FRAG_READ(AV, BV, KS, BUF)                                                                            \
  {                                                                                                               \
    _Pragma("unroll") for (int i = 0; i < MT; i++) {                                                              \
      unsigned ad_ = a_addr[i] + (BUF) * (STAGE * 4) + (((2 * (KS) + khalf) ^ a_sw[i]) << 4);                     \
      AGZ_LDSR(AV[i], ad_)                                                                                        \
    }                                                                                                             \
    _Pragma("unroll") for (int j = 0; j < 2; j++) {                                                               \
      unsigned ad_ = b_addr[j] + (BUF) * (STAGE * 4) + (((2 * (KS) + khalf) ^ b_sw[j]) << 4);                     \
      AGZ_LDSR(BV[j], ad_)                                                                                        \
    }                                                                                                             \
  }
#define AGZ_WAIT_LGKM(N) asm volatile("s_waitcnt lgkmcnt(%0)" ::"n"(N)); __builtin_amdgcn_sched_barrier(0);
#define AGZ_MQ(AV, BV, C)                                                                                         \
  _Pragma("unroll") for (int i = 0; i < MT; i++) _Pragma("unroll") for (int j = 0; j < 2; j++)                    \
      acc[i][j] = __builtin_amdgcn_mfma_f32_32x32x2f32(AV[i].C, BV[j].C, acc[i][j], 0, 0, 0);
  constexpr int NRD = MT + 2;
  constexpr int NWA = A_PER_T, NWB = B_PER_T;

#define AGZ_ITER(IT, BUF, XA0, XA1, XA2, XA3, XB0, XB1, XB2, XB3, YA0, YA1, YA2, YA3, YB0, YB1, YB2, YB3)         \
  {                                                                                                               \
    AGZ_TILE_OFFS((IT) + 2)                                                                                       \
    AGZ_FRAG_READ(f0a, f0b, 0, BUF)                                                                               \
    AGZ_FRAG_READ(f1a, f1b, 1, BUF)                                                                               \
    AGZ_WAIT_LGKM(NRD)                                                              \
    AGZ_MQ(f0a, f0b, x) AGZ_SB AGZ_GLA(YA0, 0) AGZ_SB AGZ_MQ(f0a, f0b, y) AGZ_SB AGZ_GLA(YA1, 1)                  \
    AGZ_SB AGZ_MQ(f0a, f0b, z) AGZ_SB AGZ_GLA(YA2, 2) AGZ_SB AGZ_MQ(f0a, f0b, w) AGZ_SB AGZ_GLA(YA3, 3)           \
    AGZ_SB AGZ_FRAG_READ(f0a, f0b, 2, BUF)                                                                        \
    AGZ_WAIT_LGKM(NRD)                                                                              \
    AGZ_MQ(f1a, f1b, x) AGZ_SB AGZ_GLB(YB0, 0) AGZ_SB AGZ_MQ(f1a, f1b, y) AGZ_SB AGZ_GLB(YB1, 1)                  \
    AGZ_SB AGZ_MQ(f1a, f1b, z) AGZ_SB AGZ_GLB(YB2, 2) AGZ_SB AGZ_MQ(f1a, f1b, w) AGZ_SB AGZ_GLB(YB3, 3)           \
    AGZ_SB AGZ_FRAG_READ(f1a, f1b, 3, BUF)                                                                        \
    AGZ_WAIT_LGKM(NRD)                                                                              \
    AGZ_MQ(f0a, f0b, x) AGZ_SB AGZ_LSA(XA0, 0, (BUF) ^ 1) AGZ_SB AGZ_MQ(f0a, f0b, y) AGZ_SB AGZ_LSA(XA1, 1, (BUF) ^ 1) \
    AGZ_SB AGZ_MQ(f0a, f0b, z) AGZ_SB AGZ_LSA(XA2, 2, (BUF) ^ 1) AGZ_SB AGZ_MQ(f0a, f0b, w) AGZ_SB AGZ_LSA(XA3, 3, (BUF) ^ 1) \
    AGZ_SB                                                                                                        \
    AGZ_WAIT_LGKM(NWA)                 \
    AGZ_MQ(f1a, f1b, x) AGZ_SB AGZ_LSB(XB0, 0, (BUF) ^ 1) AGZ_SB AGZ_MQ(f1a, f1b, y) AGZ_SB AGZ_LSB(XB1, 1, (BUF) ^ 1) \
    AGZ_SB AGZ_MQ(f1a, f1b, z) AGZ_SB AGZ_LSB(XB2, 2, (BUF) ^ 1) AGZ_SB AGZ_MQ(f1a, f1b, w) AGZ_SB AGZ_LSB(XB3, 3, (BUF) ^ 1) \
    AGZ_SB                                                                                                        \
    __syncthreads();                                                                                              \
  }
  (void)NWB;
  AGZ_TILE_OFFS(it0)
  AGZ_GLA(sa0, 0) AGZ_GLA(sa1, 1) AGZ_GLA(sa2, 2) AGZ_GLA(sa3, 3) AGZ_GLB(sb0, 0) AGZ_GLB(sb1, 1) AGZ_GLB(sb2, 2) AGZ_GLB(sb3, 3)
  AGZ_TILE_OFFS(it0 + 1)
  AGZ_GLA(ra0, 0) AGZ_GLA(ra1, 1) AGZ_GLA(ra2, 2) AGZ_GLA(ra3, 3) AGZ_GLB(rb0, 0) AGZ_GLB(rb1, 1) AGZ_GLB(rb2, 2) AGZ_GLB(rb3, 3)
  AGZ_LSA(sa0, 0, 0) AGZ_LSA(sa1, 1, 0) AGZ_LSA(sa2, 2, 0) AGZ_LSA(sa3, 3, 0) AGZ_LSB(sb0, 0, 0) AGZ_LSB(sb1, 1, 0) AGZ_LSB(sb2, 2, 0) AGZ_LSB(sb3, 3, 0)
  __syncthreads();
  for (int it = it0; it < NK; it += 2) {
    AGZ_ITER(it, 0, ra0, ra1, ra2, ra3, rb0, rb1, rb2, rb3, sa0, sa1, sa2, sa3, sb0, sb1, sb2, sb3)
    if (it + 1 < NK) AGZ_ITER(it + 1, 1, sa0, sa1, sa2, sa3, sb0, sb1, sb2, sb3, ra0, ra1, ra2, ra3, rb0, rb1, rb2, rb3)
  }
#undef AGZ_ITER
#undef AGZ_WAIT_LGKM
#undef AGZ_LDSR
#undef AGZ_MQ
#undef AGZ_FRAG_READ
#undef AGZ_SB
#undef AGZ_LSB
// ... 93 lines not shown

template <bool DUAL>
__global__ __launch_bounds__(256) void splitk_epilogue_kernel(ConvArgs a, int half) {
  const int C4 = a.Cout_p >> 2;
  size_t idx = (size_t)blockIdx.x * blockDim.x + threadIdx.x;
  if (idx >= (size_t)a.M * C4) return;
  int m = (int)(idx / C4), c = ((int)(idx - (size_t)m * C4)) << 2;
  int b = m / a.HW, p = m - b * a.HW;
  int h = p / a.W, w = p - h * a.W;
  float4* out = reinterpret_cast<float4*>(a.y + ((size_t)b * a.HpWp + (h + 1) * a.Wp + (w + 1)) * a.Cout_p + c);
  const size_t sstride = (size_t)a.M * a.Ntot;
  if (DUAL) {
    int ca = (c / half) * 2 * half + (c % half);
    const float* row = a.ws + (size_t)m * a.Ntot + ca;
    float4 sa = {0.f, 0.f, 0.f, 0.f}, sb = {0.f, 0.f, 0.f, 0.f};
#pragma unroll 6
    for (int s = 0; s < a.splits; s++) {
      float4 va = *reinterpret_cast<const float4*>(row + s * sstride);
      float4 vb = *reinterpret_cast<const float4*>(row + s * sstride + half);
      sa.x += va.x; sa.y += va.y; sa.z += va.z; sa.w += va.w;
      sb.x += vb.x; sb.y += vb.y; sb.z += vb.z; sb.w += vb.w;
    }
    const float4* e = reinterpret_cast<const float4*>(a.ep) + (size_t)p * a.Cout_p + c;
    float r[4];
    const float av[4] = {sa.x, sa.y, sa.z, sa.w}, bv[4] = {sb.x, sb.y, sb.z, sb.w};
#pragma unroll
    for (int q = 0; q < 4; q++) {
      float4 eq = e[q];
      float va = av[q] * eq.x + eq.y, vb = bv[q] * eq.z + eq.w;
      va = va > 0.f ? va : 0.f; vb = vb > 0.f ? vb : 0.f;
      float t = va + vb;
      r[q] = t > 0.f ? t : 0.f;
    }
    *out = float4{r[0], r[1], r[2], r[3]};
  } else {
    const float* row = a.ws + (size_t)m * a.Ntot + c;
    float4 sa = {0.f, 0.f, 0.f, 0.f};
#pragma unroll 6
    for (int s = 0; s < a.splits; s++) {
      float4 va = *reinterpret_cast<const float4*>(row + s * sstride);
      sa.x += va.x; sa.y += va.y; sa.z += va.z; sa.w += va.w;
    }
    if (a.raw) { *out = sa; return; }
    const float2* e = reinterpret_cast<const float2*>(a.ep) + (size_t)p * a.Cout_p + c;
    const float av[4] = {sa.x, sa.y, sa.z, sa.w};
    float r[4];
#pragma unroll
    for (int q = 0; q < 4; q++) { float v = av[q] * e[q].x + e[q].y; r[q] = v > 0.f ? v : 0.f; }
    *out = float4{r[0], r[1], r[2], r[3]};
  }
}

__global__ void pack_planes_kernel(const float* __restrict__ planes, float* __restrict__ out, int B, int F, int H, int W,
                                   int Fp) {
  int idx = blockIdx.x * blockDim.x + threadIdx.x;
  int total = B * H * W * Fp;
  if (idx >= total) return;
  int c = idx % Fp;
  int p = idx / Fp;
  int w = p % W, h = (p / W) % H, b = p / (W * H);
  float v = c < F ? planes[((size_t)(b * F + c) * H + h) * W + w] : 0.f;
  out[(((size_t)b * (H + 2) + h + 1) * (W + 2) + w + 1) * Fp + c] = v;
}

struct HeadArgs {
  const float* x;
  const float* conv;
  const float* bn;
  const float* Wp; const float* bp; const float* W1; const float* b1; const float* W2; const float* b2;
  float* policy; float* value;
  int H, W, HW, Wp_, HpWp, Kp, A, FC;
  float* feat;
  float* cols;
};

__device__ __forceinline__ float wave_sum(float v) {
#pragma unroll
  for (int o = 32; o > 0; o >>= 1) v += __shfl_xor(v, o, 64);
  return v;
}

__global__ __launch_bounds__(256) void heads_kernel(HeadArgs a) {
  extern __shared__ float sm[];
  float* feat = sm;
  float* red = sm + 3 * a.HW;
  float* hid = red + 8;
  const int b = blockIdx.x, tid = threadIdx.x, lane = tid & 63, wid = tid >> 6;
  for (int p = wid; p < a.HW; p += 4) {
    int h = p / a.W, w = p - h * a.W;
    const float* xp = a.x + ((size_t)b * a.HpWp + (h + 1) * a.Wp_ + (w + 1)) * a.Kp;
    float s0 = 0.f, s1 = 0.f, s2 = 0.f;
    for (int c = lane * 4; c < a.Kp; c += 256) {
      float4 xv = *reinterpret_cast<const float4*>(xp + c);
      float4 w0 = *reinterpret_cast<const float4*>(a.conv + c);
      float4 w1 = *reinterpret_cast<const float4*>(a.conv + a.Kp + c);
      float4 w2 = *reinterpret_cast<const float4*>(a.conv + 2 * a.Kp + c);
      s0 += xv.x * w0.x + xv.y * w0.y + xv.z * w0.z + xv.w * w0.w;
      s1 += xv.x * w1.x + xv.y * w1.y + xv.z * w1.z + xv.w * w1.w;
      s2 += xv.x * w2.x + xv.y * w2.y + xv.z * w2.z + xv.w * w2.w;
    }
    s0 = wave_sum(s0); s1 = wave_sum(s1); s2 = wave_sum(s2);
    if (lane == 0) {
      float v0 = s0 * a.bn[(0 * a.HW + p) * 2] + a.bn[(0 * a.HW + p) * 2 + 1];
      float v1 = s1 * a.bn[(1 * a.HW + p) * 2] + a.bn[(1 * a.HW + p) * 2 + 1];
      float v2 = s2 * a.bn[(2 * a.HW + p) * 2] + a.bn[(2 * a.HW + p) * 2 + 1];
      feat[p] = v0 > 0.f ? v0 : 0.f;
      feat[a.HW + p] = v1 > 0.f ? v1 : 0.f;
      feat[2 * a.HW + p] = v2 > 0.f ? v2 : 0.f;
    }
  }
  __syncthreads();
  float lmax = -INFINITY;
  float logit[2];
  for (int r = 0, j = tid; r < 2; r++, j += 256) {
    float s = 0.f;
    if (j < a.A) {
      for (int i = 0; i < 2 * a.HW; i++) s += feat[i] * a.Wp[(size_t)i * a.A + j];
      s += a.bp[j];
      lmax = fmaxf(lmax, s);
    }
    logit[r] = s;
  }
  for (int o = 32; o > 0; o >>= 1) lmax = fmaxf(lmax, __shfl_xor(lmax, o, 64));
  if (lane == 0) red[wid] = lmax;
  __syncthreads();
  float mx = fmaxf(fmaxf(red[0], red[1]), fmaxf(red[2], red[3]));
  float lsum = 0.f;
  for (int r = 0, j = tid; r < 2; r++, j += 256) {
    if (j < a.A) { logit[r] = expf(logit[r] - mx); lsum += logit[r]; }
  }
  lsum = wave_sum(lsum);
  if (lane == 0) red[4 + wid] = lsum;
  __syncthreads();
  float tot = red[4] + red[5] + red[6] + red[7];
  for (int r = 0, j = tid; r < 2; r++, j += 256)
    if (j < a.A) a.policy[(size_t)b * a.A + j] = logit[r] / tot;
  for (int j = tid; j < a.FC; j += 256) {
    float s = 0.f;
    const float* f2 = feat + 2 * a.HW;
    for (int i = 0; i < a.HW; i++) s += f2[i] * a.W1[(size_t)i * a.FC + j];
    s += a.b1[j];
    hid[j] = s > 0.f ? s : 0.f;
  }
  __syncthreads();
  float o = 0.f;
  for (int j = tid; j < a.FC; j += 256) o += hid[j] * a.W2[j];
  o = wave_sum(o);
  __syncthreads();
  if (lane == 0) red[wid] = o;
  __syncthreads();
  if (tid == 0) a.value[b] = tanhf(red[0] + red[1] + red[2] + red[3] + a.b2[0]);
}

__global__ __launch_bounds__(256) void heads_feat_kernel(HeadArgs a) {
  const int b = blockIdx.y, lane = threadIdx.x & 63, p = blockIdx.x * 4 + (threadIdx.x >> 6);
  if (p >= a.HW) return;
  int h = p / a.W, w = p - h * a.W;
  const float* xp = a.x + ((size_t)b * a.HpWp + (h + 1) * a.Wp_ + (w + 1)) * a.Kp;
  float s0 = 0.f, s1 = 0.f, s2 = 0.f;
  for (int c = lane * 4; c < a.Kp; c += 256) {
    float4 xv = *reinterpret_cast<const float4*>(xp + c);
    float4 w0 = *reinterpret_cast<const float4*>(a.conv + c);
    float4 w1 = *reinterpret_cast<const float4*>(a.conv + a.Kp + c);
    float4 w2 = *reinterpret_cast<const float4*>(a.conv + 2 * a.Kp + c);
    s0 += xv.x * w0.x + xv.y * w0.y + xv.z * w0.z + xv.w * w0.w;
    s1 += xv.x * w1.x + xv.y * w1.y + xv.z * w1.z + xv.w * w1.w;
    s2 += xv.x * w2.x + xv.y * w2.y + xv.z * w2.z + xv.w * w2.w;
  }
  s0 = wave_sum(s0); s1 = wave_sum(s1); s2 = wave_sum(s2);
  if (lane == 0) {
    float* f = a.feat + (size_t)b * 3 * a.HW;
    float v0 = s0 * a.bn[(0 * a.HW + p) * 2] + a.bn[(0 * a.HW + p) * 2 + 1];
    float v1 = s1 * a.bn[(1 * a.HW + p) * 2] + a.bn[(1 * a.HW + p) * 2 + 1];
    float v2 = s2 * a.bn[(2 * a.HW + p) * 2] + a.bn[(2 * a.HW + p) * 2 + 1];
    f[p] = v0 > 0.f ? v0 : 0.f;
    f[a.HW + p] = v1 > 0.f ? v1 : 0.f;
    f[2 * a.HW + p] = v2 > 0.f ? v2 : 0.f;
  }
}
__global__ __launch_bounds__(1024) void heads_fc_kernel(HeadArgs a) {
  __shared__ float part[16][64];
  const int b = blockIdx.y, lane = threadIdx.x & 63, wv = threadIdx.x >> 6;
  const int col = blockIdx.x * 64 + lane;
  const bool is_pol = col < a.A;
  const int j = is_pol ? col : col - a.A;
  const bool live = col < a.A + a.FC;
  const int rows = is_pol ? 2 * a.HW : a.HW, ld = is_pol ? a.A : a.FC;
  const float* Wm = is_pol ? a.Wp : a.W1;
  const float* f = a.feat + (size_t)b * 3 * a.HW + (is_pol ? 0 : 2 * a.HW);
  const int chunk = (rows + 15) >> 4;
  int i0 = wv * chunk, i1 = i0 + chunk < rows ? i0 + chunk : rows;
  float s = 0.f;
  if (live) {
    int i = i0;
    for (; i + 16 <= i1; i += 16) {
      float fv[16], wv_[16];
#pragma unroll
      for (int u = 0; u < 16; u++) { fv[u] = f[i + u]; wv_[u] = Wm[(size_t)(i + u) * ld + j]; }
#pragma unroll
      for (int u = 0; u < 16; u++) s = fmaf(fv[u], wv_[u], s);
    }
    {
      float fv[16], wv_[16];
#pragma unroll
      for (int u = 0; u < 16; u++) { const bool ok = i + u < i1; const int r = ok ? i + u : 0; fv[u] = ok ? f[r] : 0.f; wv_[u] = Wm[(size_t)r * ld + j]; }
#pragma unroll
      for (int u = 0; u < 16; u++) if (i + u < i1) s = fmaf(fv[u], wv_[u], s);
    }
  }
  part[wv][lane] = s;
  __syncthreads();
  if (wv == 0 && live) {
    float t = 0.f;
#pragma unroll
    for (int q = 0; q < 16; q++) t += part[q][lane];
    t += is_pol ? a.bp[j] : a.b1[j];
    if (!is_pol) t = t > 0.f ? t : 0.f;
    a.cols[(size_t)b * (a.A + a.FC) + col] = t;
  }
}
template <int NB>
__global__ __launch_bounds__(1024) void heads_fc_nb_kernel(HeadArgs a, int B) {
  __shared__ float part[NB][16][64];
  const int b0 = blockIdx.y * NB, lane = threadIdx.x & 63, wv = __builtin_amdgcn_readfirstlane(threadIdx.x >> 6);
  const int col = blockIdx.x * 64 + lane;
  const bool is_pol = col < a.A;
  const int j = is_pol ? col : col - a.A;
  const bool live = col < a.A + a.FC;
  const int rows = is_pol ? 2 * a.HW : a.HW, ld = is_pol ? a.A : a.FC;
  const float* Wm = is_pol ? a.Wp : a.W1;
  const float* f[NB];
#pragma unroll
  for (int n = 0; n < NB; n++) f[n] = a.feat + (size_t)min(b0 + n, B - 1) * 3 * a.HW + (is_pol ? 0 : 2 * a.HW);
  const int chunk = (rows + 15) >> 4;
  int i0 = wv * chunk, i1 = i0 + chunk < rows ? i0 + chunk : rows;
  float s[NB];
#pragma unroll
  for (int n = 0; n < NB; n++) s[n] = 0.f;
  if (live) {
    int i = i0;
    for (; i + 16 <= i1; i += 16) {
      float wv_[16];
#pragma unroll
      for (int u = 0; u < 16; u++) wv_[u] = Wm[(size_t)(i + u) * ld + j];
#pragma unroll
      for (int n = 0; n < NB; n++) {
        float fv[16];
#pragma unroll
        for (int u = 0; u < 16; u++) fv[u] = f[n][i + u];
#pragma unroll
        for (int u = 0; u < 16; u++) s[n] = fmaf(fv[u], wv_[u], s[n]);
      }
    }
    {
      float wv_[16];
#pragma unroll
      for (int u = 0; u < 16; u++) { const int r = i + u < i1 ? i + u : 0; wv_[u] = Wm[(size_t)r * ld + j]; }
#pragma unroll
      for (int n = 0; n < NB; n++) {
        float fv[16];
#pragma unroll
        for (int u = 0; u < 16; u++) { const bool ok = i + u < i1; fv[u] = ok ? f[n][ok ? i + u : 0] : 0.f; }
#pragma unroll
        for (int u = 0; u < 16; u++) if (i + u < i1) s[n] = fmaf(fv[u], wv_[u], s[n]);
      }
    }
  }
#pragma unroll
  for (int n = 0; n < NB; n++) part[n][wv][lane] = s[n];
  __syncthreads();
  if (live && wv < NB && b0 + wv < B) {
    float t = 0.f;
#pragma unroll
    for (int q = 0; q < 16; q++) t += part[wv][q][lane];
    t += is_pol ? a.bp[j] : a.b1[j];
    if (!is_pol) t = t > 0.f ? t : 0.f;
    a.cols[(size_t)(b0 + wv) * (a.A + a.FC) + col] = t;
  }
}
__global__ __launch_bounds__(256) void heads_out_kernel(HeadArgs a) {
  __shared__ float red[8];
  const int b = blockIdx.x, tid = threadIdx.x, lane = tid & 63, wid = tid >> 6;
  const float* cols = a.cols + (size_t)b * (a.A + a.FC);
  float lmax = -INFINITY;
  float logit[2];
  for (int r = 0, j = tid; r < 2; r++, j += 256) {
    logit[r] = j < a.A ? cols[j] : 0.f;
    if (j < a.A) lmax = fmaxf(lmax, logit[r]);
  }
  for (int o = 32; o > 0; o >>= 1) lmax = fmaxf(lmax, __shfl_xor(lmax, o, 64));
  if (lane == 0) red[wid] = lmax;
  __syncthreads();
  float mx = fmaxf(fmaxf(red[0], red[1]), fmaxf(red[2], red[3]));
  float lsum = 0.f;
  for (int r = 0, j = tid; r < 2; r++, j += 256)
    if (j < a.A) { logit[r] = expf(logit[r] - mx); lsum += logit[r]; }
  lsum = wave_sum(lsum);
  if (lane == 0) red[4 + wid] = lsum;
  __syncthreads();
  float tot = red[4] + red[5] + red[6] + red[7];
  for (int r = 0, j = tid; r < 2; r++, j += 256)
    if (j < a.A) a.policy[(size_t)b * a.A + j] = logit[r] / tot;
  float o = 0.f;
  for (int j = tid; j < a.FC; j += 256) o += cols[a.A + j] * a.W2[j];
  o = wave_sum(o);
  __syncthreads();
  if (lane == 0) red[wid] = o;
  __syncthreads();
  if (tid == 0) a.value[b] = tanhf(red[0] + red[1] + red[2] + red[3] + a.b2[0]);
}

}

using namespace agz;

void agz_net::free_device() {
  auto f = [](float*& p) { if (p) { hipFree(p); p = nullptr; } };
  f(d_w_init); f(d_w_init_t); f(d_ep_init);
  if (d_w3_init) { hipFree(d_w3_init); d_w3_init = nullptr; }
  for (auto& p : d_w_dual) f(p);
  for (auto& p : d_ep_dual) f(p);
  for (auto& p : d_w3_dual) if (p) { hipFree(p); p = nullptr; }
  for (auto& p : d_w2_dual) if (p) { hipFree(p); p = nullptr; }
  if (d_amax) { hipFree(d_amax); d_amax = nullptr; }
  amax_cap = 0;
  for (auto& p : d_u3_dual) if (p) { hipFree(p); p = nullptr; }
  for (auto& p : d_u2_dual) if (p) { hipFree(p); p = nullptr; }
  d_u2_dual.clear();
  for (auto& p : d_u2_tin) if (p) hipFree(p);
  d_u2_tin.clear();
  for (auto& p : d_u2_colun) if (p) hipFree(p);
  d_u2_colun.clear();
  free_u2c();
  for (auto& p : d_ep_h2) if (p) hipFree(p);
  d_ep_h2.clear();
  if (d_ep_init_h2) { hipFree(d_ep_init_h2); d_ep_init_h2 = nullptr; }
  f(d_wV); f(d_wM);
  wino_chunk_cap = 0; wino_v_cap = 0;
  d_w_dual.clear(); d_ep_dual.clear(); d_w3_dual.clear(); d_w2_dual.clear(); d_u3_dual.clear();
  f(d_head_conv); f(d_head_bn); f(d_Wp); f(d_bp); f(d_W1); f(d_b1); f(d_W2); f(d_b2);
  f(d_act_in); f(d_actA); f(d_actB); f(d_planes); f(d_policy); f(d_value); f(d_ws); f(d_hs);
  ws_cap = 0; hs_cap = 0;
  max_batch = 0;
}

int agz_net::ensure_batch(int B) {
  if (B <= max_batch) return AGZ_OK;
  AGZ_REQUIRE((size_t)B * Hp * Wp * (size_t)std::max(Kp, Fp) < ((size_t)1 << 31), AGZ_E_UNSUPPORTED,
              "agz_net: batch %d too large for 32-bit activation offsets (%d x %d board, %d channels)", B, H, W, Kp);
  auto f = [](float*& p) { if (p) { hipFree(p); p = nullptr; } };
  f(d_act_in); f(d_actA); f(d_actB); f(d_planes); f(d_policy); f(d_value);
  size_t px = (size_t)B * Hp * Wp;
  AGZ_HIP_TRY(hipMalloc(&d_act_in, px * Fp * sizeof(float)));
  AGZ_HIP_TRY(hipMalloc(&d_actA, px * Kp * sizeof(float)));
  AGZ_HIP_TRY(hipMalloc(&d_actB, px * Kp * sizeof(float)));
  AGZ_HIP_TRY(hipMalloc(&d_planes, (size_t)B * conf.Features * HW * sizeof(float)));
  AGZ_HIP_TRY(hipMalloc(&d_policy, (size_t)B * conf.ActionSpace * sizeof(float)));
  AGZ_HIP_TRY(hipMalloc(&d_value, (size_t)B * sizeof(float)));
  AGZ_HIP_TRY(hipMemsetAsync(d_act_in, 0, px * Fp * sizeof(float), ctx->stream));
  AGZ_HIP_TRY(hipMemsetAsync(d_actA, 0, px * Kp * sizeof(float), ctx->stream));
  AGZ_HIP_TRY(hipMemsetAsync(d_actB, 0, px * Kp * sizeof(float), ctx->stream));
  max_batch = B;
  return AGZ_OK;
}

static int splitk_per(int NC) { return NC; }
template <int WM, int WN, int MT, bool DUAL>
static int launch_conv(agz_ctx* ctx, ConvArgs& a, float** ws = nullptr, size_t* ws_cap = nullptr) {
  const int klass = DUAL ? AGZ_PROF_CONV : AGZ_PROF_CONV_INIT;
  constexpr int BM = WM * MT * 32, BNT = WN * 64;
  a.n_ntiles = ceil_div(a.Ntot, BNT);
  a.n_mtiles = ceil_div(a.M, BM);
  const int tiles = a.n_mtiles * a.n_ntiles;
  const int NK = 9 * (a.Cin_p >> 5);
  a.splits = 1; a.per = NK; a.ws = nullptr;
  if (ws && NK > splitk_per(a.Cin_p >> 5)) {
    a.per = splitk_per(a.Cin_p >> 5);
    a.splits = ceil_div(NK, a.per);
    size_t need = (size_t)a.splits * a.M * a.Ntot;
    if (need > *ws_cap) {
      AGZ_HIP_TRY(hipStreamSynchronize(ctx->stream));
      if (*ws) hipFree(*ws);
      *ws = nullptr; *ws_cap = 0;
      AGZ_HIP_TRY(hipMalloc(ws, need * sizeof(float)));
      *ws_cap = need;
    }
    a.ws = *ws;
  }
  ProfScope ps(ctx, klass);
  dim3 grid(tiles, a.splits), block(256);
  hipLaunchKernelGGL((conv3x3_mfma_kernel<WM, WN, MT, DUAL>), grid, block, 0, ctx->stream, a);
  if (a.splits > 1) {
    size_t n = (size_t)a.M * (a.Cout_p / 4);
    hipLaunchKernelGGL((splitk_epilogue_kernel<DUAL>), dim3((unsigned)((n + 255) / 256)), dim3(256), 0, ctx->stream, a, BNT / 2);
  }
  return AGZ_OK;
}

int agz::conv3x3_raw(agz_ctx* ctx, const float* x, const float* w, float* y, int B, int H, int W, int Cin_p, int Cout_p) {
  ConvArgs a{};
  a.M = B * H * W; a.HW = H * W; a.W = W; a.Wp = W + 2; a.HpWp = (H + 2) * (W + 2);
  a.x = x; a.w = w; a.ep = nullptr; a.y = y; a.Cin_p = Cin_p; a.Cout_p = Cout_p; a.Ntot = Cout_p; a.raw = 1;
  if (Cout_p % 128 == 0) launch_conv<2, 2, 2, false>(ctx, a); else launch_conv<4, 1, 1, false>(ctx, a);
  AGZ_HIP_TRY(hipGetLastError());
  return AGZ_OK;
}

int agz::split_w3(agz_ctx* ctx, const float* w, unsigned short* w3, int N, int Cin_p) {
  size_t total = (size_t)9 * N * Cin_p;
  hipLaunchKernelGGL(split_w3_kernel, dim3((unsigned)((total + 255) / 256)), dim3(256), 0, ctx->stream, w, w3, N, Cin_p);
  AGZ_HIP_TRY(hipGetLastError());
  return AGZ_OK;
}

int agz::conv3x3_raw_x3(agz_ctx* ctx, const float* x, const unsigned short* w3, float* y, int B, int H, int W, int Cin_p, int Cout_p) {
  AGZ_REQUIRE(Cin_p % 16 == 0, AGZ_E_INVALID, "conv3x3_raw_x3: Cin %d not a multiple of 16", Cin_p);
  AGZ_REQUIRE((size_t)B * (H + 2) * (W + 2) * Cin_p * sizeof(float) < ((size_t)1 << 32), AGZ_E_UNSUPPORTED, "conv3x3_raw_x3: tensor above 4 GiB");
  ConvArgs a{};
  a.M = B * H * W; a.HW = H * W; a.W = W; a.Wp = W + 2; a.HpWp = (H + 2) * (W + 2);
  a.x = x; a.w = nullptr; a.ep = nullptr; a.y = y; a.Cin_p = Cin_p; a.Cout_p = Cout_p; a.Ntot = Cout_p; a.raw = 1;
  a.n_ntiles = ceil_div(Cout_p, 128); a.n_mtiles = ceil_div(a.M, 128); a.splits = 1;
  ProfScope ps(ctx, AGZ_PROF_CONV_INIT);
  hipLaunchKernelGGL((conv3x3_x3_kernel<false>), dim3(a.n_mtiles * a.n_ntiles), dim3(256), 0, ctx->stream, a, w3);
  AGZ_HIP_TRY(hipGetLastError());
  return AGZ_OK;
}

__global__ __launch_bounds__(256) void w_absmax_kernel(const float* __restrict__ w, size_t n, unsigned* __restrict__ out_bits) {
  __shared__ unsigned sm[4];
  unsigned m = 0;
  for (size_t i = (size_t)blockIdx.x * 256 + threadIdx.x; i < n; i += (size_t)gridDim.x * 256) {
    const unsigned a = __float_as_uint(w[i]) & 0x7fffffffu;
    m = a > m ? a : m;
  }
  for (int o = 32; o > 0; o >>= 1) { const unsigned t = (unsigned)__shfl_xor((int)m, o, 64); m = t > m ? t : m; }
  if ((threadIdx.x & 63) == 0) sm[threadIdx.x >> 6] = m;
  __syncthreads();
  if (threadIdx.x == 0) {
    const unsigned a = sm[0] > sm[1] ? sm[0] : sm[1], b = sm[2] > sm[3] ? sm[2] : sm[3];
    atomicMax(out_bits, a > b ? a : b);
  }
}
__global__ __launch_bounds__(256) void split_w2_kernel(const float* __restrict__ w, _Float16* __restrict__ w2, int N, int Cin_p, const unsigned* __restrict__ wmax,
                                                       unsigned* __restrict__ board_words, int B, unsigned* __restrict__ wmax_next) {
  const size_t idx = (size_t)blockIdx.x * 256 + threadIdx.x;
  if (blockIdx.x == 0) {
    for (int b = threadIdx.x; b < B; b += 256) board_words[b] = 0u;
    if (threadIdx.x == 0) *wmax_next = 0u;
  }
  if (idx >= (size_t)9 * N * Cin_p) return;
  const int ci = (int)(idx % Cin_p);
  const size_t r = idx / Cin_p;
  const int n = (int)(r % N), t = (int)(r / N);
  float s, inv;
  h2_scales(*wmax, &s, &inv);
  const float xs = w[idx] * s;
  const _Float16 hi = (_Float16)xs;
  const _Float16 lo = (_Float16)(xs - (float)hi);
  const size_t base = (((size_t)((ci >> 5) * 9 + t) * 2) * N + n) * 32 + (ci & 31);
  w2[base] = hi;
  w2[base + (size_t)N * 32] = lo;
}
bool agz::conv3x3_raw_h2_fits(int B, int H, int W, int Cin_p, int Cout_p) {
  return Cin_p % 32 == 0 && Cout_p % 256 == 0 && (size_t)B * (H + 2) * (W + 2) * (size_t)std::max(Cin_p, Cout_p) * sizeof(float) < ((size_t)1 << 32);
}
static int raw_h2_weights(agz_ctx* ctx, const float* w, int B, int Cin_p, int Cout_p, WinoRawScratch* sc, unsigned** wmax_out) {
  hipStream_t s = ctx->stream;
  const size_t w_elems = (size_t)9 * Cout_p * Cin_p;
  if (sc->w2_cap < w_elems * 2) {
    if (sc->w2) hipFree(sc->w2);
    sc->w2 = nullptr; sc->w2_cap = 0;
    AGZ_HIP_TRY(hipMalloc(&sc->w2, w_elems * 2 * sizeof(_Float16)));
    sc->w2_cap = w_elems * 2;
  }
  if (sc->h2_b_cap < B) {
    if (sc->h2_words) hipFree(sc->h2_words);
    sc->h2_words = nullptr; sc->h2_b_cap = 0;
    AGZ_HIP_TRY(hipMalloc(&sc->h2_words, ((size_t)B + 2) * sizeof(unsigned)));
// ... 230 lines not shown
    const std::vector<float>& e = h_ep_dual[l];
    const bool more = l + 1 < conf.SharedLayers;
    e2.assign(e.size(), 0.f);
    for (int p = 0; p < hw; p++)
      for (int c = 0; c < Kp; c++) {
        const float tn = more ? tins[l + 1][c] : 1.0f;
        const size_t o = ((size_t)p * Kp + c) * 4;
        e2[o + 0] = e[o + 0] * coluns[l][c] * tn; e2[o + 1] = e[o + 1] * tn;
        e2[o + 2] = e[o + 2] * coluns[l][Kp + c] * tn; e2[o + 3] = e[o + 3] * tn;
      }
    if (chained) {
      double g1 = 0.0, g0 = 0.0;
      for (int p = 0; p < hw; p++)
        for (int c = 0; c < Kp; c++) {
          const double tn = more ? tins[l + 1][c] : 1.0;
          const size_t o = ((size_t)p * Kp + c) * 4;
          g1 = std::max(g1, tn * (std::fabs((double)e[o + 0]) * l1s[l][c] + std::fabs((double)e[o + 2]) * l1s[l][Kp + c]));
          g0 = std::max(g0, tn * (std::max((double)e[o + 1], 0.0) + std::max((double)e[o + 3], 0.0)));
        }
      wino_g1[l] = (float)(g1 * (1.0 + 1e-6)); wino_g0[l] = (float)(g0 * (1.0 + 1e-6));
    }
    AGZ_HIP_TRY(hipMalloc(&d_ep_h2[l], e2.size() * 4));
    AGZ_HIP_TRY(hipMemcpyAsync(d_ep_h2[l], e2.data(), e2.size() * 4, hipMemcpyHostToDevice, ctx->stream));
    AGZ_HIP_TRY(hipStreamSynchronize(ctx->stream));
  }
  if (conf.SharedLayers > 0) {
    e2.assign(h_ep_init.size(), 0.f);
    for (int p = 0; p < hw; p++)
      for (int c = 0; c < Kp; c++) {
        const size_t o = ((size_t)p * Kp + c) * 2;
        e2[o] = h_ep_init[o] * tins[0][c]; e2[o + 1] = h_ep_init[o + 1] * tins[0][c];
      }
    AGZ_HIP_TRY(hipMalloc(&d_ep_init_h2, e2.size() * 4));
    AGZ_HIP_TRY(hipMemcpyAsync(d_ep_init_h2, e2.data(), e2.size() * 4, hipMemcpyHostToDevice, ctx->stream));
    AGZ_HIP_TRY(hipStreamSynchronize(ctx->stream));
  }
  return AGZ_OK;
}

agz_net::FwdPlan agz_net::fwd_plan(int B) const {
  const int M = B * HW;
  FwdPlan p{};
  auto n_tiles128 = [&](int ntot) { return ceil_div(M, 128) * ceil_div(ntot, 128); };
  p.half_init = cfg == 0 && n_tiles128(Kp) < ctx->num_cus;
  p.half_dual = cfg == 0 && n_tiles128(2 * Kp) < ctx->num_cus;
  const int tiles_dual = cfg != 0 ? ceil_div(M, 128) * ceil_div(2 * Kp, 64) : ceil_div(M, 64) * ceil_div(2 * Kp, 128);
  p.small = latency_mode && Kp >= 64 &&
            (tiles_dual * 4 <= ctx->num_cus || (Kp >= 256 && tiles_dual <= ctx->num_cus));
  p.forced_split = compute_force && cfg == 0 && conf.SharedLayers > 0 &&
                   (this->compute_mode == AGZ_COMPUTE_WINO_H2 || this->compute_mode == AGZ_COMPUTE_WINO ||
                    this->compute_mode == AGZ_COMPUTE_BF16X3 || this->compute_mode == AGZ_COMPUTE_FP16X2);
  p.latency = p.small && !p.forced_split;
  const int spread_max = 64;
  p.heads_spread = p.small || (latency_mode && (B <= spread_max || Kp >= 256));
  p.heads_nb = B >= 32;
  p.split_ok = cfg == 0 && !p.latency && (!p.half_dual || compute_force) && conf.SharedLayers > 0 &&
               (size_t)B * Hp * Wp * Kp * sizeof(float) < ((size_t)1 << 32);
  {
    const int npos = (wino_tm + 2) * (wino_tm + 2), tpb = ceil_div(H, wino_tm) * ceil_div(W, wino_tm);
    p.wino_wide = (2 * Kp) % 256 == 0 && (size_t)npos * ceil_div(B * tpb, 128) * ((2 * Kp) / 256) >= (size_t)ctx->num_cus;
  }
  return p;
}

int agz_net::min_same_batch(int n, int G) const {
  if (n >= G) return G;
  const FwdPlan want = fwd_plan(G);
  auto same = [&](int B) {
    const FwdPlan q = fwd_plan(B);
    return q.half_init == want.half_init && q.half_dual == want.half_dual && q.small == want.small && q.forced_split == want.forced_split &&
           q.latency == want.latency && q.heads_spread == want.heads_spread && q.split_ok == want.split_ok && q.heads_nb == want.heads_nb && q.wino_wide == want.wino_wide;
  };
  if (same(n)) return n;
  for (int B = 16; B < G; B *= 2)
    if (B > n && same(B)) return B;
  return G;
}

agz_net::H2Tower agz_net::wino_h2_tower(int B) const {
  H2Tower t{};
  t.npos = (wino_tm + 2) * (wino_tm + 2);
  t.tpb = ceil_div(H, wino_tm) * ceil_div(W, wino_tm);
  static const int chunk_env = [] { const char* e = getenv("AGZ_WINO_H2_CHUNK"); return e ? atoi(e) : 0; }();
  static const int queues_env = [] { const char* e = getenv("AGZ_WINO_H2_QUEUES"); return e ? atoi(e) : 0; }();
  const int queues_want = queues_env > 0 ? queues_env : (tower_queues > 0 ? tower_queues : (B >= 256 ? 2 : 1));
  const int chunk_max = (int)std::min<size_t>((size_t)B, ((((size_t)1 << 32) - 1) / ((size_t)t.npos * Kp * 4) - 127) / t.tpb);
  t.chunk = chunk_env >= 1 ? std::min(chunk_env, chunk_max) : chunk_max;
  t.ns = (queues_want == 2 && B >= 64) ? 2 : 1;
  if (t.ns == 2 && t.chunk >= B) t.chunk = (B + 1) / 2;
  t.v_elems = wino_h2_rows(t.npos, (size_t)t.chunk * t.tpb) * Kp; t.m_elems = 2 * t.v_elems;
  static const int form_env = [] { const char* e = getenv("AGZ_WINO_H2_FORM"); return e ? atoi(e) : -1; }();
  t.form_want = wino_form >= 0 ? wino_form : form_env;
  t.chained = t.form_want != 0 && (int)d_u2c_dual.size() == conf.SharedLayers && agz::wino_h2c_ok(H, W, wino_tm, Kp);
  t.n_scr = t.chained ? ceil_div(B, t.chunk) : t.ns;
  t.wm_board = t.chained ? (size_t)t.tpb * (Kp >> 5) * 2 : (size_t)t.tpb * (Kp >> 6);
  return t;
}

int agz_net::wino_h2_reserve(int B, const H2Tower& t, bool* amax_moved) {
  if (t.v_elems * t.n_scr > wino_v_cap) {
    AGZ_HIP_TRY(hipStreamSynchronize(ctx->stream));
    if (ctx->stream2) AGZ_HIP_TRY(hipStreamSynchronize(ctx->stream2));
    if (d_wV) hipFree(d_wV);
    if (d_wM) hipFree(d_wM);
    d_wV = d_wM = nullptr; wino_chunk_cap = 0;
    AGZ_HIP_TRY(hipMalloc(&d_wV, t.v_elems * t.n_scr * sizeof(float)));
    AGZ_HIP_TRY(hipMalloc(&d_wM, t.m_elems * t.n_scr * sizeof(float)));
    wino_v_cap = t.v_elems * t.n_scr; wino_chunk_cap = 0;
  }
  const size_t need_amax = (size_t)(conf.SharedLayers + 1) * B + t.wm_board * B;
  if (need_amax > amax_cap) {
    AGZ_HIP_TRY(hipStreamSynchronize(ctx->stream));
    if (ctx->stream2) AGZ_HIP_TRY(hipStreamSynchronize(ctx->stream2));
    if (d_amax) hipFree(d_amax);
    d_amax = nullptr; amax_cap = 0;
    AGZ_HIP_TRY(hipMalloc(&d_amax, need_amax * sizeof(unsigned)));
    amax_cap = need_amax;
    if (amax_moved) *amax_moved = true;
  }
  return AGZ_OK;
}

void agz_net::wino_h2c_block(int l, int B, int b0, int ci, const H2Tower& t, hipStream_t st, float* cur, float* nxt) {
  const size_t wmb = (size_t)t.tpb * (Kp >> 5);
  const bool last = l + 1 == conf.SharedLayers;
  float* d_wave_max = reinterpret_cast<float*>(d_amax + (size_t)(conf.SharedLayers + 1) * B);
  WinoH2Args hh{};
  WinoArgs& wa = hh.w;
  wa.x = cur + (size_t)b0 * Hp * Wp * Kp; wa.y = nxt + (size_t)b0 * Hp * Wp * Kp;
  wa.V = d_wV + (size_t)ci * t.v_elems; wa.Mb = d_wM + (size_t)ci * t.m_elems; wa.ep = d_ep_h2[l];
  wa.B = std::min(t.chunk, B - b0); wa.H = H; wa.W = W; wa.Hp = Hp; wa.Wp = Wp; wa.C = Kp; wa.Cout_p = Kp; wa.Ntot = 2 * Kp;
  hh.U2c = d_u2c_dual[l]; hh.w_unscale = 1.f; hh.tm = wino_tm;
  hh.amax_in = d_amax + (size_t)l * B + b0;
  hh.amax_next = last ? nullptr : d_amax + (size_t)(l + 1) * B + b0;
  hh.amax_true = l == 0 ? reinterpret_cast<const float*>(d_amax + b0) : nullptr;
  hh.wm_prev = d_wave_max + ((size_t)((l + 1) & 1) * B + b0) * wmb;
  hh.wm_out = d_wave_max + ((size_t)(l & 1) * B + b0) * wmb;
  hh.g1 = wino_g1[l]; hh.g0 = wino_g0[l];
  {
    static const int gemm_env = [] {
      const char* e = getenv("AGZ_WINO_H2_GEMM");
      const int v = e ? atoi(e) : 0;
      if (v == 0 || (((v & 63) == 1 || (v & 63) == 2) && (v >> 6) <= 3)) return v;
      fprintf(stderr, "libagz: AGZ_WINO_H2_GEMM=%s ignored (want 1 or 2, optionally + 64 and / or + 128)\n", e);
      return 0;
    }();
    const int gv = wino_gemm > 0 ? wino_gemm : gemm_env;
    hh.gemm_variant = gv & 63; hh.temporal_stores = (gv >> 6) & 1;
    agz::wino_h2c_rows(ctx, hh, t.form_want == 1 ? 1 : 4, ((gv >> 7) & 1) != 0);
    wino_live_r = hh.live_r; wino_live_c = hh.live_c;
  }
  if (l == 0) agz::wino_h2c_in(ctx, hh, st);
  agz::wino_h2c_gemm(ctx, hh, st);
  agz::wino_h2c_oi(ctx, hh, last, st, t.form_want == 1 ? 1 : 4);
}

void agz_net::heads_spread_range(agz::HeadArgs h, bool nb4, int B, int b0, int nb, hipStream_t st) {
  h.x += (size_t)b0 * Hp * Wp * Kp;
  h.feat = d_hs + (size_t)b0 * 3 * HW; h.cols = d_hs + (size_t)B * 3 * HW + (size_t)b0 * (conf.ActionSpace + conf.FC);
  h.policy += (size_t)b0 * conf.ActionSpace; h.value += b0;
  hipLaunchKernelGGL(heads_feat_kernel, dim3(ceil_div(HW, 4), nb), dim3(256), 0, st, h);
  if (nb4)
    hipLaunchKernelGGL(heads_fc_nb_kernel<4>, dim3(ceil_div(conf.ActionSpace + conf.FC, 64), ceil_div(nb, 4)), dim3(1024), 0, st, h, nb);
  else
    hipLaunchKernelGGL(heads_fc_kernel, dim3(ceil_div(conf.ActionSpace + conf.FC, 64), nb), dim3(1024), 0, st, h);
  hipLaunchKernelGGL(heads_out_kernel, dim3(nb), dim3(256), 0, st, h);
}

bool agz_net::half_ok(int B) const {
  if (!committed || B < 2 || B > max_batch || (B & 1) || (B / 2) % 4 != 0 || cfg != 0 || conf.SharedLayers <= 0) return false;
  if (min_same_batch(B / 2, B) != B / 2) return false;
  const FwdPlan plan = fwd_plan(B);
  int mode = compute_mode;
  if (mode == AGZ_COMPUTE_AUTO) mode = !d_u2_dual.empty() ? AGZ_COMPUTE_WINO_H2 : AGZ_COMPUTE_BF16X3;
  if (!plan.split_ok || plan.latency || mode != AGZ_COMPUTE_WINO_H2 || !plan.heads_spread || !plan.heads_nb) return false;
  if ((int)d_u2_dual.size() != conf.SharedLayers || !d_ep_init_h2) return false;
  if (!d_w3_init || Kp % 128 != 0 || (size_t)B * Hp * Wp * Fp * sizeof(float) >= ((size_t)1 << 32)) return false;
  const H2Tower t = wino_h2_tower(B);
  return t.chained && t.ns == 2 && t.chunk * 2 == B;
}

int agz_net::forward_half_reserve(int B) {
  const H2Tower t = wino_h2_tower(B);
  int r = wino_h2_reserve(B, t, nullptr);
  if (r != AGZ_OK) return r;
  const size_t need = (size_t)B * (3 * HW + conf.ActionSpace + conf.FC);
  if (need > hs_cap) {
    AGZ_HIP_TRY(hipStreamSynchronize(ctx->stream));
    if (d_hs) hipFree(d_hs);
    d_hs = nullptr; hs_cap = 0;
    AGZ_HIP_TRY(hipMalloc(&d_hs, need * sizeof(float)));
    hs_cap = need;
  }
  return AGZ_OK;
}

int agz_net::forward_half(int B, int half, hipStream_t st, float* policy_dev, float* value_dev, hipEvent_t mid) {
  const int nb = B / 2, b0 = half * nb;
  const FwdPlan plan = fwd_plan(B);
  const H2Tower t = wino_h2_tower(B);
  last_tower = nullptr; last_tower_B = 0;
  ConvArgs a{};
  a.M = nb * HW; a.HW = HW; a.W = W; a.Wp = Wp; a.HpWp = Hp * Wp;
  a.x = d_act_in + (size_t)b0 * Hp * Wp * Fp; a.w = d_w_init; a.ep = d_ep_init_h2; a.y = d_actA + (size_t)b0 * Hp * Wp * Kp;
  a.Cin_p = Fp; a.Cout_p = Kp; a.Ntot = Kp;
  a.n_ntiles = ceil_div(a.Ntot, 128); a.n_mtiles = ceil_div(a.M, 128);
  a.splits = 1; a.per = 0; a.ws = nullptr; a.raw = 0;
  AGZ_HIP_TRY(hipMemsetAsync(d_amax + b0, 0, (size_t)nb * sizeof(unsigned), st));
  a.amax_out = d_amax + b0;
  hipLaunchKernelGGL((conv3x3_x3_kernel<false>), dim3(a.n_mtiles * a.n_ntiles), dim3(256), 0, st, a, d_w3_init);
  const int L = conf.SharedLayers;
  for (int l = 0; l < L; l++) {
    wino_h2c_block(l, B, b0, half, t, st, d_actA, d_actB);
    if (mid && l == L / 2) AGZ_HIP_TRY(hipEventRecord(mid, st));
  }
  HeadArgs h{};
  h.x = d_actB; h.conv = d_head_conv; h.bn = d_head_bn; h.Wp = d_Wp; h.bp = d_bp; h.W1 = d_W1; h.b1 = d_b1; h.W2 = d_W2;
  h.b2 = d_b2; h.policy = policy_dev; h.value = value_dev;
  h.H = H; h.W = W; h.HW = HW; h.Wp_ = Wp; h.HpWp = Hp * Wp; h.Kp = Kp; h.A = conf.ActionSpace; h.FC = conf.FC;
  heads_spread_range(h, plan.heads_nb, B, b0, nb, st);
  AGZ_HIP_TRY(hipGetLastError());
  return AGZ_OK;
}

int agz_net::forward_packed(int B, float* policy_dev, float* value_dev) {
  AGZ_REQUIRE(committed, AGZ_E_STATE, "agz_net: infer before agz_net_commit");
  AGZ_REQUIRE(B >= 1 && B <= max_batch, AGZ_E_INVALID, "agz_net: batch %d exceeds allocated %d", B, max_batch);
  ConvArgs a{};
  a.M = B * HW; a.HW = HW; a.W = W; a.Wp = Wp; a.HpWp = Hp * Wp;
  a.x = d_act_in; a.w = d_w_init; a.ep = d_ep_init; a.y = d_actA;
  a.Cin_p = Fp; a.Cout_p = Kp; a.Ntot = Kp;
  const FwdPlan plan = fwd_plan(B);
  const bool half_init = plan.half_init, half_dual = plan.half_dual, latency = plan.latency, heads_spread = plan.heads_spread, split_ok = plan.split_ok;
  float** wsp = latency ? &d_ws : nullptr;
  int compute_mode = this->compute_mode;
  if (compute_mode == AGZ_COMPUTE_AUTO) compute_mode = !d_u2_dual.empty() ? AGZ_COMPUTE_WINO_H2 : AGZ_COMPUTE_BF16X3;
  const bool use_h2 = split_ok && compute_mode == AGZ_COMPUTE_FP16X2;
  const bool wino_ok = split_ok && compute_mode == AGZ_COMPUTE_WINO;
  const bool wino_h2_ok = split_ok && compute_mode == AGZ_COMPUTE_WINO_H2;
  if (wino_h2_ok && d_ep_init_h2) a.ep = d_ep_init_h2;
  if (use_h2 && (size_t)B > amax_cap) {
    AGZ_HIP_TRY(hipStreamSynchronize(ctx->stream));
    if (d_amax) hipFree(d_amax);
    d_amax = nullptr; amax_cap = 0;
    AGZ_HIP_TRY(hipMalloc(&d_amax, (size_t)B * sizeof(unsigned)));
    amax_cap = (size_t)B;
  }
  bool lat_h2 = latency && cfg == 0 && this->compute_mode != AGZ_COMPUTE_F32_MFMA && conf.SharedLayers > 0 &&
                (int)d_lat_w2.size() == conf.SharedLayers && agz::conv_lat_ok(Kp, Kp, Wp) && ceil_div(HW, agz::LAT_ROWS) * (Kp / 8) <= 256;
  for (int l = 0; lat_h2 && l < conf.SharedLayers; l++) lat_h2 = d_lat_w2[l] != nullptr;
  const int in_groups = ceil_div(HW, agz::LAT_IN_PIX), in_words = in_groups * (Kp / 64);
  const bool lat_in = lat_h2 && Fp == 32 && Kp % 64 == 0 && in_words <= 256 && d_w_init_t;
  if (lat_h2 && lat_wmax_cap < B) {
    AGZ_HIP_TRY(hipStreamSynchronize(ctx->stream));
    for (auto& p2 : d_lat_wmax) { if (p2) hipFree(p2); p2 = nullptr; }
    lat_wmax_cap = 0;
    for (auto& p2 : d_lat_wmax) AGZ_HIP_TRY(hipMalloc(&p2, (size_t)B * 256 * sizeof(float)));
    lat_wmax_cap = B;
  }
  int rc;
  bool amax0_done = false;
  if (lat_in) {
    agz::LatInArgs li{};
    li.x = d_act_in; li.w = d_w_init_t; li.ep = reinterpret_cast<const float2*>(d_ep_init); li.t = d_lat_tin[0]; li.y = d_actA; li.words = d_lat_wmax[1];
    li.B = B; li.H = H; li.W = W; li.Hp = Hp; li.Wp = Wp; li.Cout_p = Kp; li.groups_per_board = in_groups;
    ProfScope ps(ctx, AGZ_PROF_CONV_INIT);
    hipLaunchKernelGGL(agz::lat_input_kernel, dim3(Kp / 64, B * in_groups), dim3(256), 0, ctx->stream, li);
    path_input = AGZ_NPATH_IN_LAT;
    rc = AGZ_OK;
  }
  else if (split_ok && compute_mode != AGZ_COMPUTE_F32_MFMA && d_w3_init && Kp % 128 == 0 &&
      (size_t)B * Hp * Wp * Fp * sizeof(float) < ((size_t)1 << 32)) {
    a.n_ntiles = ceil_div(a.Ntot, 128); a.n_mtiles = ceil_div(a.M, 128);
    a.splits = 1; a.per = 0; a.ws = nullptr; a.raw = 0;
    ProfScope ps(ctx, AGZ_PROF_CONV_INIT);
    if (wino_h2_ok && d_amax && amax_cap >= (size_t)B) {
      AGZ_HIP_TRY(hipMemsetAsync(d_amax, 0, (size_t)B * sizeof(unsigned), ctx->stream));
      a.amax_out = d_amax; amax0_done = true;
    }
    hipLaunchKernelGGL((conv3x3_x3_kernel<false>), dim3(a.n_mtiles * a.n_ntiles), dim3(256), 0, ctx->stream, a, d_w3_init);
    a.amax_out = nullptr;
    path_input = AGZ_NPATH_IN_X3;
    rc = AGZ_OK;
  }
  else if (cfg != 0) { rc = launch_conv<4, 1, 1, false>(ctx, a, wsp, &ws_cap); path_input = AGZ_NPATH_IN_F32_411; }
  else if (half_init) { rc = launch_conv<2, 2, 1, false>(ctx, a, wsp, &ws_cap); path_input = AGZ_NPATH_IN_F32_221; }
  else { rc = launch_conv<2, 2, 2, false>(ctx, a, wsp, &ws_cap); path_input = AGZ_NPATH_IN_F32_222; }
  if (rc != AGZ_OK) return rc;
  path_block = 0;
  float* cur = d_actA;
  float* nxt = d_actB;
  bool tower_done = false;
  if (!tower_done && wino_h2_ok) {
    AGZ_REQUIRE((int)d_u2_dual.size() == conf.SharedLayers, AGZ_E_STATE, "agz_net: Winograd fp16x2 weights not built");
    const bool wide = plan.wino_wide;
    const H2Tower tw = wino_h2_tower(B);
    const int chunk = tw.chunk, ns = tw.ns;
    const size_t v_elems = tw.v_elems, m_elems = tw.m_elems, wm_board = tw.wm_board;
    const bool chained = tw.chained;
    {
      bool amax_moved = false;
      const int rr = wino_h2_reserve(B, tw, &amax_moved);
      if (rr != AGZ_OK) return rr;
      if (amax_moved) amax0_done = false;
    }
    float* d_wave_max = reinterpret_cast<float*>(d_amax + (size_t)(conf.SharedLayers + 1) * B);
    if (!amax0_done)
      hipLaunchKernelGGL(board_amax_kernel, dim3(B), dim3(256), 0, ctx->stream, cur, d_amax, HW, W, Wp, Hp * Wp, Kp, (const float*)nullptr);
    if (ns == 2) {
      { const int rs = ctx->ensure_stream2(); if (rs != AGZ_OK) return rs; }
      AGZ_HIP_TRY(hipEventRecord(ctx->ev_fork, ctx->stream));
      AGZ_HIP_TRY(hipStreamWaitEvent(ctx->stream2, ctx->ev_fork, 0));
    }
    for (int l = 0; chained && l < conf.SharedLayers; l++) {
      ProfScope ps(ctx, AGZ_PROF_CONV);
      int ci = 0;
      const bool last = l + 1 == conf.SharedLayers;
      for (int b0 = 0; b0 < B; b0 += chunk, ci++)
        wino_h2c_block(l, B, b0, ci, tw, (ci % ns) ? ctx->stream2 : (hipStream_t)ctx->stream, cur, nxt);
      path_block = AGZ_NPATH_BLK_WINO_H2_CHAINED;
      if (last) std::swap(cur, nxt);
    }
    for (int l = 0; !chained && l < conf.SharedLayers; l++) {
      ProfScope ps(ctx, AGZ_PROF_CONV);
      int ci = 0;
      for (int b0 = 0; b0 < B; b0 += chunk, ci++) {
        const int q = ci % ns;
        WinoH2Args hh{};
        WinoArgs& wa = hh.w;
        wa.x = cur + (size_t)b0 * Hp * Wp * Kp; wa.y = nxt + (size_t)b0 * Hp * Wp * Kp;
        wa.V = d_wV + (size_t)q * v_elems; wa.Mb = d_wM + (size_t)q * m_elems; wa.ep = d_ep_h2[l];
        wa.B = std::min(chunk, B - b0); wa.H = H; wa.W = W; wa.Hp = Hp; wa.Wp = Wp; wa.C = Kp; wa.Cout_p = Kp; wa.Ntot = 2 * Kp;
        hh.U2 = d_u2_dual[l]; hh.w_unscale = 1.f; hh.tm = wino_tm;
        hh.t_in = nullptr; hh.col_unscale = nullptr; hh.t_next = nullptr;
        hh.amax_in = d_amax + (size_t)l * B + b0; hh.amax_out = d_amax + (size_t)(l + 1) * B + b0;
        hh.wave_max = d_wave_max + (size_t)b0 * wm_board;
        hh.fuse_prev = l > 0;
        wino_h2_launch(ctx, hh, wide, q ? ctx->stream2 : ctx->stream);
        path_block = wide ? AGZ_NPATH_BLK_WINO_H2_3K_WIDE : AGZ_NPATH_BLK_WINO_H2_3K;
      }
      std::swap(cur, nxt);
    }
    if (ns == 2) {
      AGZ_HIP_TRY(hipEventRecord(ctx->ev_join, ctx->stream2));
      AGZ_HIP_TRY(hipStreamWaitEvent(ctx->stream, ctx->ev_join, 0));
    }
    tower_done = true;
  }
  for (int l = 0; !tower_done && l < conf.SharedLayers; l++) {
    a.x = cur; a.w = d_w_dual[l]; a.ep = d_ep_dual[l]; a.y = nxt;
    a.Cin_p = Kp; a.Cout_p = Kp; a.Ntot = 2 * Kp;
    if (use_h2) {
      a.n_ntiles = ceil_div(a.Ntot, 128); a.n_mtiles = ceil_div(a.M, 128);
      a.splits = 1; a.per = 0; a.ws = nullptr; a.raw = 0;
      hipLaunchKernelGGL(board_amax_kernel, dim3(B), dim3(256), 0, ctx->stream, cur, d_amax, HW, W, Wp, Hp * Wp, Kp);
      a.amax_in = d_amax; a.w_unscale = w_unscale[l];
      ProfScope ps(ctx, AGZ_PROF_CONV);
      if ((2 * Kp) % 256 == 0) {
        a.n_ntiles = (2 * Kp) / 256;
        hipLaunchKernelGGL(conv3x3_h2w_kernel, dim3(a.n_mtiles * a.n_ntiles), dim3(256), 0, ctx->stream, a, d_w2_dual[l]);
        path_block = AGZ_NPATH_BLK_H2W;
      } else {
        hipLaunchKernelGGL(conv3x3_h2_kernel, dim3(a.n_mtiles * a.n_ntiles), dim3(256), 0, ctx->stream, a, d_w2_dual[l]);
        path_block = AGZ_NPATH_BLK_H2;
      }
      rc = AGZ_OK;
    }
    else if (wino_ok) {
      AGZ_REQUIRE((int)d_u3_dual.size() == conf.SharedLayers && d_u3_dual[l], AGZ_E_STATE, "agz_net: Winograd weights not built");
      static const int chunk_env = [] { const char* e = getenv("AGZ_WINO_CHUNK"); return e ? atoi(e) : 0; }();
      const int tpb = ceil_div(H, 4) * ceil_div(W, 4);
      const int chunk_max = (int)std::min<size_t>((size_t)B, (((size_t)1 << 32) - 1) / ((size_t)36 * tpb * Kp * 4));
      const int chunk = chunk_env >= 1 ? std::min(chunk_env, chunk_max) : chunk_max;
      if (chunk > wino_chunk_cap) {
        AGZ_HIP_TRY(hipStreamSynchronize(ctx->stream));
        if (d_wV) hipFree(d_wV);
        if (d_wM) hipFree(d_wM);
        d_wV = d_wM = nullptr; wino_chunk_cap = 0;
        AGZ_HIP_TRY(hipMalloc(&d_wV, (size_t)36 * chunk * tpb * Kp * sizeof(float)));
        AGZ_HIP_TRY(hipMalloc(&d_wM, (size_t)36 * chunk * tpb * 2 * Kp * sizeof(float)));
        wino_chunk_cap = chunk; wino_v_cap = 0;
      }
      ProfScope ps(ctx, AGZ_PROF_CONV);
      for (int b0 = 0; b0 < B; b0 += chunk) {
        WinoArgs wa{};
        wa.x = cur + (size_t)b0 * Hp * Wp * Kp; wa.y = nxt + (size_t)b0 * Hp * Wp * Kp;
        wa.V = d_wV; wa.Mb = d_wM; wa.U3 = d_u3_dual[l]; wa.ep = d_ep_dual[l];
        wa.B = std::min(chunk, B - b0); wa.H = H; wa.W = W; wa.Hp = Hp; wa.Wp = Wp; wa.C = Kp; wa.Cout_p = Kp; wa.Ntot = 2 * Kp;
        wino_launch(ctx, wa, WINO_IN | WINO_GEMM | WINO_OUT);
        path_block = AGZ_NPATH_BLK_WINO;
      }
      rc = AGZ_OK;
    }
    else if (split_ok && compute_mode == AGZ_COMPUTE_BF16X3) {
      a.n_ntiles = ceil_div(a.Ntot, 128); a.n_mtiles = ceil_div(a.M, 128);
      a.splits = 1; a.per = 0; a.ws = nullptr; a.raw = 0;
      ProfScope ps(ctx, AGZ_PROF_CONV);
      hipLaunchKernelGGL((conv3x3_x3_kernel<true>), dim3(a.n_mtiles * a.n_ntiles), dim3(256), 0, ctx->stream, a, d_w3_dual[l]);
      path_block = AGZ_NPATH_BLK_X3;
      rc = AGZ_OK;
    }
    else if (lat_h2) {
      const int gpb = ceil_div(HW, agz::LAT_ROWS), words = gpb * (Kp / 8);
      agz::LatH2Args la{};
      la.x = cur; la.w2 = d_lat_w2[l]; la.t_in = d_lat_tin[l]; la.col_unscale = d_lat_colun[l]; la.ep = d_ep_dual[l]; la.y = nxt;
      la.B = B; la.H = H; la.W = W; la.Hp = Hp; la.Wp = Wp; la.C = Kp; la.Cout_p = Kp; la.Ntot = 2 * Kp;
      la.groups_per_board = gpb;
      if (l == 0) {
        if (!lat_in) hipLaunchKernelGGL(agz::lat_board_words_kernel, dim3(B * 64), dim3(256), 0, ctx->stream, cur, (const float*)d_lat_tin[0], d_lat_wmax[1], HW, W, Wp, Hp * Wp, Kp, 64);
        la.wmax_in = d_lat_wmax[1]; la.n_in_words = lat_in ? in_words : 64;
      } else {
        la.wmax_in = d_lat_wmax[(l - 1) & 1]; la.n_in_words = words;
      }
      const bool more = l + 1 < conf.SharedLayers;
      la.t_next = more ? d_lat_tin[l + 1] : nullptr;
      la.wmax_out = more ? d_lat_wmax[l & 1] : nullptr;
      ProfScope ps(ctx, AGZ_PROF_CONV);
      agz::conv_lat_h2_launch(ctx, la);
      path_block = AGZ_NPATH_BLK_LAT_H2;
      rc = AGZ_OK;
    }
    else if (cfg != 0) { rc = launch_conv<4, 1, 1, true>(ctx, a, wsp, &ws_cap); path_block = a.splits > 1 ? AGZ_NPATH_BLK_F32_411_SPLITK : AGZ_NPATH_BLK_F32_411; }
    else if (half_dual) { rc = launch_conv<2, 2, 1, true>(ctx, a, wsp, &ws_cap); path_block = a.splits > 1 ? AGZ_NPATH_BLK_F32_221_SPLITK : AGZ_NPATH_BLK_F32_221; }
    else { rc = launch_conv<2, 2, 2, true>(ctx, a, wsp, &ws_cap); path_block = a.splits > 1 ? AGZ_NPATH_BLK_F32_222_SPLITK : AGZ_NPATH_BLK_F32_222; }
    if (rc != AGZ_OK) return rc;
    std::swap(cur, nxt);
  }
  HeadArgs h{};
  h.x = cur; h.conv = d_head_conv; h.bn = d_head_bn; h.Wp = d_Wp; h.bp = d_bp; h.W1 = d_W1; h.b1 = d_b1; h.W2 = d_W2;
  h.b2 = d_b2; h.policy = policy_dev; h.value = value_dev;
  h.H = H; h.W = W; h.HW = HW; h.Wp_ = Wp; h.HpWp = Hp * Wp; h.Kp = Kp; h.A = conf.ActionSpace; h.FC = conf.FC;
  last_tower = cur; last_tower_B = B;
  size_t smem = (size_t)(3 * HW + 8 + conf.FC) * sizeof(float);
// ... 272 lines not shown
        const float sb = wmax > 0.f ? std::ldexp(1.0f, 14 - ex) : 1.0f;
        n->w_unscale[l] = 1.0f / sb;
        std::vector<_Float16> w2((size_t)9 * NC32 * 2 * Ntot * 32);
        for (int t = 0; t < 9; t++) for (int nn = 0; nn < Ntot; nn++) for (int ci = 0; ci < Kp; ci++) {
          float xs = wt[((size_t)t * Ntot + nn) * Kp + ci] * sb;
          _Float16 hi = (_Float16)xs;
          _Float16 lo = (_Float16)(xs - (float)hi);
          size_t base = (((size_t)((ci / 32) * 9 + t) * 2) * Ntot + nn) * 32 + (ci % 32);
          w2[base] = hi;
          w2[base + (size_t)Ntot * 32] = lo;
        }
        if (n->d_w2_dual[l]) { hipFree(n->d_w2_dual[l]); n->d_w2_dual[l] = nullptr; }
        AGZ_HIP_TRY(hipMalloc(&n->d_w2_dual[l], w2.size() * 2));
        AGZ_HIP_TRY(hipMemcpyAsync(n->d_w2_dual[l], w2.data(), w2.size() * 2, hipMemcpyHostToDevice, s));
        AGZ_HIP_TRY(hipStreamSynchronize(s));
      }
      if (n->d_w3_dual[l]) { hipFree(n->d_w3_dual[l]); n->d_w3_dual[l] = nullptr; }
      AGZ_HIP_TRY(hipMalloc(&n->d_w3_dual[l], w3.size() * 2));
      AGZ_HIP_TRY(hipMemcpyAsync(n->d_w3_dual[l], w3.data(), w3.size() * 2, hipMemcpyHostToDevice, s));
      AGZ_HIP_TRY(hipStreamSynchronize(s));
      if (agz::conv_lat_ok(Kp, Kp, n->Wp)) {
        if ((int)n->d_lat_w2.size() != c.SharedLayers) {
          n->d_lat_w2.assign(c.SharedLayers, nullptr); n->d_lat_tin.assign(c.SharedLayers, nullptr); n->d_lat_colun.assign(c.SharedLayers, nullptr);
        }
        std::vector<float> tin(Kp, 1.0f), colun(Ntot, 1.0f), su(Ntot, 1.0f), rmax(Kp, 0.f), cmax(Ntot, 0.f);
        for (int t = 0; t < 9; t++) for (int nn = 0; nn < Ntot; nn++) for (int ci = 0; ci < Kp; ci++)
          rmax[ci] = std::max(rmax[ci], std::fabs(wt[((size_t)t * Ntot + nn) * Kp + ci]));
        for (int ci = 0; ci < Kp; ci++)
          if (rmax[ci] > 0.f && std::isfinite(rmax[ci])) { int ex = 0; std::frexp(rmax[ci], &ex); tin[ci] = std::ldexp(1.0f, std::max(-100, std::min(100, ex - 1))); }
        for (int t = 0; t < 9; t++) for (int nn = 0; nn < Ntot; nn++) for (int ci = 0; ci < Kp; ci++)
          cmax[nn] = std::max(cmax[nn], std::fabs(wt[((size_t)t * Ntot + nn) * Kp + ci] / tin[ci]));
        for (int nn = 0; nn < Ntot; nn++)
          if (cmax[nn] > 0.f && std::isfinite(cmax[nn])) { int ex = 0; std::frexp(cmax[nn], &ex); su[nn] = std::ldexp(1.0f, 14 - ex); colun[nn] = 1.0f / su[nn]; }
        std::vector<_Float16> l2((size_t)9 * (Kp / 32) * 2 * Ntot * 32);
        for (int t = 0; t < 9; t++) for (int nn = 0; nn < Ntot; nn++) for (int ci = 0; ci < Kp; ci++) {
          const float xs = wt[((size_t)t * Ntot + nn) * Kp + ci] / tin[ci] * su[nn];
          const _Float16 hi = (_Float16)xs;
          const _Float16 lo = (_Float16)(xs - (float)hi);
          const size_t base = (((size_t)((ci / 32) * 9 + t) * 2) * Ntot + nn) * 32 + (ci % 32);
          l2[base] = hi;
          l2[base + (size_t)Ntot * 32] = lo;
        }
        if (n->d_lat_w2[l]) { hipFree(n->d_lat_w2[l]); n->d_lat_w2[l] = nullptr; }
        AGZ_HIP_TRY(hipMalloc(&n->d_lat_w2[l], l2.size() * 2));
        AGZ_HIP_TRY(hipMemcpyAsync(n->d_lat_w2[l], l2.data(), l2.size() * 2, hipMemcpyHostToDevice, s));
        int r2;
        if ((r2 = upload(&n->d_lat_tin[l], tin, s)) != AGZ_OK) return r2;
        if ((r2 = upload(&n->d_lat_colun[l], colun, s)) != AGZ_OK) return r2;
        AGZ_HIP_TRY(hipStreamSynchronize(s));
      }
    }
    pi += 6; bi += 2;
  }
  {
    std::vector<float> hc((size_t)3 * Kp, 0.f), hb((size_t)3 * hw * 2, 0.f);
    const Param& pw = n->params[pi];
    for (int o = 0; o < 2; o++) for (int ci = 0; ci < K; ci++) hc[(size_t)o * Kp + ci] = pw.v[(size_t)o * K + ci];
    for (int o = 0; o < 2; o++) for (int p = 0; p < hw; p++)
      fold(bi, o, n->params[pi + 1], n->params[pi + 2], p, &hb[((size_t)o * hw + p) * 2], &hb[((size_t)o * hw + p) * 2 + 1]);
    pi += 3; bi++;
    int r;
    if ((r = upload(&n->d_Wp, n->params[pi].v, s)) != AGZ_OK) return r;
    if ((r = upload(&n->d_bp, n->params[pi + 1].v, s)) != AGZ_OK) return r;
    pi += 2;
    const Param& vw = n->params[pi];
    for (int ci = 0; ci < K; ci++) hc[(size_t)2 * Kp + ci] = vw.v[ci];
    for (int p = 0; p < hw; p++)
      fold(bi, 0, n->params[pi + 1], n->params[pi + 2], p, &hb[((size_t)2 * hw + p) * 2], &hb[((size_t)2 * hw + p) * 2 + 1]);
    pi += 3; bi++;
    if ((r = upload(&n->d_W1, n->params[pi].v, s)) != AGZ_OK) return r;
    if ((r = upload(&n->d_b1, n->params[pi + 1].v, s)) != AGZ_OK) return r;
    pi += 2;
    if ((r = upload(&n->d_W2, n->params[pi].v, s)) != AGZ_OK) return r;
    if ((r = upload(&n->d_b2, n->params[pi + 1].v, s)) != AGZ_OK) return r;
    pi += 2;
    if ((r = upload(&n->d_head_conv, hc, s)) != AGZ_OK) return r;
    if ((r = upload(&n->d_head_bn, hb, s)) != AGZ_OK) return r;
    (void)A; (void)FCn;
  }
  n->committed = true;
  for (auto& p : n->d_u2_dual) if (p) hipFree(p);
  n->d_u2_dual.clear();
  for (auto& p : n->d_u2_tin) if (p) hipFree(p);
  n->d_u2_tin.clear();
  for (auto& p : n->d_u2_colun) if (p) hipFree(p);
  n->d_u2_colun.clear();
  n->free_u2c();
  for (auto& p : n->d_ep_h2) if (p) hipFree(p);
  n->d_ep_h2.clear();
  if (n->d_ep_init_h2) { hipFree(n->d_ep_init_h2); n->d_ep_init_h2 = nullptr; }
  if (n->compute_mode == AGZ_COMPUTE_WINO && n->cfg == 0) return n->build_wino_weights();
  if ((n->compute_mode == AGZ_COMPUTE_WINO_H2 || n->compute_mode == AGZ_COMPUTE_AUTO) && n->cfg == 0) return n->build_wino_h2_weights();
  return AGZ_OK;
}

int agz_wino_h2_tile(int H, int W) { return agz::wino_h2_pick_tm(H, W); }

int agz_wino_h2_chained(int H, int W, int K) {
  static const int form_env = [] { const char* e = getenv("AGZ_WINO_H2_FORM"); return e ? atoi(e) : -1; }();
  const int Kp = agz::round_up(K, 32);
  return form_env != 0 && agz::wino_h2c_ok(H, W, agz::wino_h2_pick_tm(H, W), Kp) ? 1 : 0;
}

int agz_net_set_wino_h2_form(agz_net* n, int form) {
  AGZ_REQUIRE(n, AGZ_E_INVALID, "agz_net_set_wino_h2_form: null net");
  AGZ_REQUIRE(form >= -1 && form <= 2, AGZ_E_INVALID, "agz_net_set_wino_h2_form: form %d (want -1, 0 or 1)", form);
  n->wino_form = form;
  return AGZ_OK;
}

int agz_net_min_same_batch(agz_net* n, int k, int G, int* batch) {
  AGZ_REQUIRE(n && batch && k >= 1 && G >= k, AGZ_E_INVALID, "agz_net_min_same_batch: bad argument");
  AGZ_REQUIRE(n->committed, AGZ_E_STATE, "agz_net_min_same_batch: commit the net first");
  *batch = n->min_same_batch(k, G);
  return AGZ_OK;
}

int agz_net_wino_h2_last_rows(agz_net* n, int* live_r, int* live_c) {
  AGZ_REQUIRE(n && live_r && live_c, AGZ_E_INVALID, "agz_net_wino_h2_last_rows: null argument");
  *live_r = n->wino_live_r; *live_c = n->wino_live_c;
  return AGZ_OK;
}

int agz_net_tower_out(agz_net* n, int B, float* host) {
  AGZ_REQUIRE(n && host, AGZ_E_INVALID, "agz_net_tower_out: null argument");
  AGZ_REQUIRE(n->last_tower && n->last_tower_B > 0, AGZ_E_STATE, "agz_net_tower_out: no whole-batch forward to read (none yet, or the last one was a split step)");
  AGZ_REQUIRE(B == n->last_tower_B, AGZ_E_INVALID, "agz_net_tower_out: batch %d, the last forward ran %d boards", B, n->last_tower_B);
  AGZ_HIP_TRY(hipSetDevice(n->ctx->device));
  AGZ_HIP_TRY(hipStreamSynchronize(n->ctx->stream));
  const int H = n->H, W = n->W, Hp = n->Hp, Wp = n->Wp, Kp = n->Kp, K = n->conf.K;
  std::vector<float> pad((size_t)B * Hp * Wp * Kp);
  AGZ_HIP_TRY(hipMemcpy(pad.data(), n->last_tower, pad.size() * sizeof(float), hipMemcpyDeviceToHost));
  for (int b = 0; b < B; b++)
    for (int k = 0; k < K; k++)
      for (int y = 0; y < H; y++)
        for (int x = 0; x < W; x++)
          host[(((size_t)b * K + k) * H + y) * W + x] = pad[(((size_t)b * Hp + y + 1) * Wp + x + 1) * Kp + k];
  return AGZ_OK;
}

int agz_net_last_paths(agz_net* n, int* input_conv, int* block, int* heads) {
  AGZ_REQUIRE(n && input_conv && block && heads, AGZ_E_INVALID, "agz_net_last_paths: null argument");
  *input_conv = n->path_input; *block = n->path_block; *heads = n->path_heads;
  return AGZ_OK;
}

int agz_net_set_wino_h2_gemm(agz_net* n, int variant) {
  AGZ_REQUIRE(n, AGZ_E_INVALID, "agz_net_set_wino_h2_gemm: null net");
  AGZ_REQUIRE(((variant & 63) <= 2 && (variant >> 6) <= 3) || ((variant & 15) == 2 && (variant >> 4) <= 3), AGZ_E_INVALID, "agz_net_set_wino_h2_gemm: variant %d (want 0, 1, 2, + 64, + 128, or 2 + 16 * mode)", variant);
  n->wino_gemm = variant;
  return AGZ_OK;
}

int agz_wino_stages(agz_ctx* ctx, const float* x, const float* w, int B, int H, int W, int C, int N, float* V, float* M) {
  AGZ_REQUIRE(ctx && x && w && V && M, AGZ_E_INVALID, "agz_wino_stages: NULL argument");
  AGZ_REQUIRE(B >= 1 && H >= 1 && W >= 1 && C >= 16 && C % 16 == 0 && N >= 1, AGZ_E_INVALID, "agz_wino_stages: bad shape");
  AGZ_HIP_TRY(hipSetDevice(ctx->device));
  const int Hp = H + 2, Wp = W + 2;
  std::vector<float> xp((size_t)B * Hp * Wp * C, 0.f);
  for (int b = 0; b < B; b++) for (int h = 0; h < H; h++)
    memcpy(&xp[(((size_t)b * Hp + h + 1) * Wp + 1) * C], &x[((size_t)b * H + h) * W * C], (size_t)W * C * sizeof(float));
  std::vector<unsigned short> u3;
  agz::wino_build_u3(u3, N, C, [&](int n, int ci, int tap) -> double { return (double)w[((size_t)n * C + ci) * 9 + tap]; });
  agz::WinoArgs a{};
  a.B = B; a.H = H; a.W = W; a.Hp = Hp; a.Wp = Wp; a.C = C; a.Cout_p = N; a.Ntot = N;
  const size_t T = (size_t)B * agz::ceil_div(H, 4) * agz::ceil_div(W, 4);
  AGZ_REQUIRE((size_t)36 * T * C * 4 < ((size_t)1 << 32), AGZ_E_UNSUPPORTED, "agz_wino_stages: V above 4 GiB");
  float *dx = nullptr, *dV = nullptr, *dM = nullptr;
  unsigned short* dU = nullptr;
  int rc = AGZ_OK;
  if (hipMalloc(&dx, xp.size() * 4) != hipSuccess || hipMalloc(&dV, (size_t)36 * T * C * 4) != hipSuccess ||
      hipMalloc(&dM, (size_t)36 * T * N * 4) != hipSuccess || hipMalloc(&dU, u3.size() * 2) != hipSuccess) {
    agz::set_error("agz_wino_stages: out of device memory");
    rc = AGZ_E_NOMEM;
  } else {
    hipStream_t s = ctx->stream;
    bool ok = hipMemcpyAsync(dx, xp.data(), xp.size() * 4, hipMemcpyHostToDevice, s) == hipSuccess &&
              hipMemcpyAsync(dU, u3.data(), u3.size() * 2, hipMemcpyHostToDevice, s) == hipSuccess;
    a.x = dx; a.V = dV; a.U3 = dU; a.Mb = dM;
    if (ok) agz::wino_launch(ctx, a, agz::WINO_IN | agz::WINO_GEMM);
    ok = ok && hipGetLastError() == hipSuccess &&
         hipMemcpyAsync(V, dV, (size_t)36 * T * C * 4, hipMemcpyDeviceToHost, s) == hipSuccess &&
         hipMemcpyAsync(M, dM, (size_t)36 * T * N * 4, hipMemcpyDeviceToHost, s) == hipSuccess && hipStreamSynchronize(s) == hipSuccess;
    if (!ok) { agz::set_error("agz_wino_stages: HIP failure: %s", hipGetErrorString(hipGetLastError())); rc = AGZ_E_HIP; }
  }
  if (dx) hipFree(dx);
  if (dV) hipFree(dV);
  if (dM) hipFree(dM);
  if (dU) hipFree(dU);
  return rc;
}

int agz_net_set_compute_mode(agz_net* n, int mode) {
  AGZ_REQUIRE(n, AGZ_E_INVALID, "agz_net_set_compute_mode: NULL net");
  const int base = mode & ~AGZ_COMPUTE_FORCE;
  AGZ_REQUIRE(base == AGZ_COMPUTE_F32_MFMA || base == AGZ_COMPUTE_BF16X3 || base == AGZ_COMPUTE_FP16X2 || base == AGZ_COMPUTE_WINO || base == AGZ_COMPUTE_AUTO ||
                  base == AGZ_COMPUTE_WINO_H2,
              AGZ_E_INVALID, "agz_net_set_compute_mode: unknown mode %d", mode);
  n->compute_mode = base;
  n->compute_force = (mode & AGZ_COMPUTE_FORCE) != 0;
  if (base == AGZ_COMPUTE_WINO && n->committed && n->cfg == 0 && n->d_u3_dual.empty()) return n->build_wino_weights();
  if ((base == AGZ_COMPUTE_WINO_H2 || base == AGZ_COMPUTE_AUTO) && n->committed && n->cfg == 0 && n->d_u2_dual.empty()) return n->build_wino_h2_weights();
  return AGZ_OK;
}

int agz_net_set_tower_queues(agz_net* n, int queues) {
  AGZ_REQUIRE(n && queues >= 0 && queues <= 2, AGZ_E_INVALID, "agz_net_set_tower_queues: queues must be 0 (auto), 1 or 2");
  n->tower_queues = queues;
  return AGZ_OK;
}

int agz_net_set_latency_mode(agz_net* n, int on) {
  AGZ_REQUIRE(n, AGZ_E_INVALID, "agz_net_set_latency_mode: NULL net");
  n->latency_mode = on != 0;
  return AGZ_OK;
}

int agz_net_infer_dev(agz_net* n, const float* planes_dev, int B, float* policy_dev, float* value_dev) {
  AGZ_REQUIRE(n && planes_dev && policy_dev && value_dev && B >= 1, AGZ_E_INVALID, "agz_net_infer_dev: bad argument");
  AGZ_HIP_TRY(hipSetDevice(n->ctx->device));
  return n->forward_dev(planes_dev, B, policy_dev, value_dev);
}

int agz_net_infer(agz_net* n, const float* planes, int B, float* policy, float* value) {
  AGZ_REQUIRE(n && planes && policy && value && B >= 1, AGZ_E_INVALID, "agz_net_infer: bad argument");
  AGZ_REQUIRE(n->committed, AGZ_E_STATE, "agz_net_infer: call agz_net_commit first");
  AGZ_HIP_TRY(hipSetDevice(n->ctx->device));
  int r = n->ensure_batch(B);
  if (r != AGZ_OK) return r;
  hipStream_t s = n->ctx->stream;
  size_t per = (size_t)n->conf.Features * n->HW;
  AGZ_HIP_TRY(hipMemcpyAsync(n->d_planes, planes, (size_t)B * per * sizeof(float), hipMemcpyHostToDevice, s));
  r = n->forward_dev(n->d_planes, B, n->d_policy, n->d_value);
  if (r != AGZ_OK) return r;
  AGZ_HIP_TRY(hipMemcpyAsync(policy, n->d_policy, (size_t)B * n->conf.ActionSpace * sizeof(float), hipMemcpyDeviceToHost, s));
  AGZ_HIP_TRY(hipMemcpyAsync(value, n->d_value, (size_t)B * sizeof(float), hipMemcpyDeviceToHost, s));
  AGZ_HIP_TRY(hipStreamSynchronize(s));
  return AGZ_OK;
}

int agz_net_save(const agz_net* n, const char* path) {
  AGZ_REQUIRE(n && path, AGZ_E_INVALID, "agz_net_save: NULL argument");
  FILE* f = fopen(path, "wb");
  AGZ_REQUIRE(f, AGZ_E_INVALID, "agz_net_save: cannot open %s", path);
  bool ok = fwrite("AGZNET01", 1, 8, f) == 8 && fwrite(&n->conf, sizeof(agz_net_conf), 1, f) == 1;
  uint64_t np = n->params.size();
  ok = ok && fwrite(&np, 8, 1, f) == 1;
  for (const Param& p : n->params) {
    uint64_t cnt = p.v.size();
    ok = ok && fwrite(&cnt, 8, 1, f) == 1 && fwrite(p.v.data(), 4, cnt, f) == cnt;
  }
  for (const BNStats& b : n->bn) {
    uint64_t C = b.mean.size();
    ok = ok && fwrite(&C, 8, 1, f) == 1 && fwrite(b.mean.data(), 4, C, f) == C && fwrite(b.var.data(), 4, C, f) == C;
  }
  ok = (fclose(f) == 0) && ok;
  AGZ_REQUIRE(ok, AGZ_E_INVALID, "agz_net_save: write to %s failed", path);
  return AGZ_OK;
}

int agz_net_load(agz_net* n, const char* path) {
  AGZ_REQUIRE(n && path, AGZ_E_INVALID, "agz_net_load: NULL argument");
  FILE* f = fopen(path, "rb");
  AGZ_REQUIRE(f, AGZ_E_INVALID, "agz_net_load: cannot open %s", path);
  char magic[8];
  agz_net_conf c;
  uint64_t np = 0;
  bool ok = fread(magic, 1, 8, f) == 8 && memcmp(magic, "AGZNET01", 8) == 0 && fread(&c, sizeof(c), 1, f) == 1 && fread(&np, 8, 1, f) == 1;
  if (ok) ok = memcmp(&c, &n->conf, sizeof(c)) == 0 && np == n->params.size();
  if (!ok) { fclose(f); agz::set_error("agz_net_load: %s is not a checkpoint of this network configuration", path); return AGZ_E_INVALID; }
  for (Param& p : n->params) {
    uint64_t cnt = 0;
    ok = ok && fread(&cnt, 8, 1, f) == 1 && cnt == p.v.size() && fread(p.v.data(), 4, cnt, f) == cnt;
  }
  for (BNStats& b : n->bn) {
    uint64_t C = 0;
    ok = ok && fread(&C, 8, 1, f) == 1 && C == b.mean.size() && fread(b.mean.data(), 4, C, f) == C && fread(b.var.data(), 4, C, f) == C;
  }
  fclose(f);
  AGZ_REQUIRE(ok, AGZ_E_INVALID, "agz_net_load: %s is truncated or mismatched", path);
  n->committed = false;
  return agz_net_commit(n);
}

double agz_net_flops_per_eval(const agz_net* n) {
  if (!n) return 0;
  double K = n->conf.K, F = n->conf.Features, hw = n->HW, A = n->conf.ActionSpace, L = n->conf.SharedLayers, FCn = n->conf.FC;
  return 2 * F * K * 9 * hw + L * 2 * (2 * K * K * 9 * hw) + (2 * K * 2 * hw + 2 * 2 * hw * A) + (2 * K * hw + 2 * hw * FCn + 2 * FCn);
}

}
```

### agogo_amd/csrc/net.hpp

```cpp
#pragma once
#include <string>
#include <vector>

#include "common.hpp"

namespace agz {
struct Param {
  std::string name;
  std::vector<float> v;
  std::vector<int> ref_shape;
  int kind;
};
struct BNStats { std::vector<float> mean, var; };
int conv3x3_raw(agz_ctx* ctx, const float* x, const float* w, float* y, int B, int H, int W, int Cin_p, int Cout_p);
int conv3x3_raw_x3(agz_ctx* ctx, const float* x, const unsigned short* w3, float* y, int B, int H, int W, int Cin_p, int Cout_p);
int split_w3(agz_ctx* ctx, const float* w, unsigned short* w3, int N, int Cin_p);
inline size_t w3_elems(int N, int Cin_p) { return (size_t)9 * 3 * N * Cin_p; }
struct WinoRawScratch {
  float* V = nullptr; float* M = nullptr; void* U2 = nullptr; unsigned* words = nullptr;
  size_t v_cap = 0, m_cap = 0, u_cap = 0; int b_cap = 0;
  void* w2 = nullptr; unsigned* h2_words = nullptr;
  size_t w2_cap = 0; int h2_b_cap = 0, h2_flip = 0;
};
int conv3x3_raw_h2(agz_ctx* ctx, const float* x, const float* w, float* y, int B, int H, int W, int Cin_p, int Cout_p, WinoRawScratch* sc,
                   const unsigned* ranges = nullptr);
bool conv3x3_raw_h2_fits(int B, int H, int W, int Cin_p, int Cout_p);
int conv3x3_raw_h2_weights(agz_ctx* ctx, const float* w, int Cin_p, int Cout_p, WinoRawScratch* sc, const void** w2, const unsigned** w_amax);
struct RawWeights { void* img = nullptr; unsigned* words = nullptr; size_t cap = 0; };
int conv3x3_raw_h2_weights_to(agz_ctx* ctx, hipStream_t st, const float* w, int Cin_p, int Cout_p, RawWeights* out);
int conv3x3_raw_wino_h2_weights_to(agz_ctx* ctx, hipStream_t st, const float* w, int H, int W, int Cin_p, int Cout_p, RawWeights* out);
void raw_weights_free(RawWeights* rw);
int conv3x3_raw_wino_h2(agz_ctx* ctx, const float* x, const float* w, float* y, int B, int H, int W, int Cin_p, int Cout_p, WinoRawScratch* sc,
                        const unsigned* ranges = nullptr, const RawWeights* pre = nullptr);
bool conv3x3_raw_wino_h2_fits(int B, int H, int W, int Cin_p, int Cout_p);
void wino_raw_scratch_free(WinoRawScratch* sc);
struct HeadArgs;
}

struct agz_net {
  agz_ctx* ctx = nullptr;
  agz_net_conf conf{};
  std::vector<agz::Param> params;
  std::vector<agz::BNStats> bn;
  bool committed = false;

  int H = 0, W = 0, HW = 0, Hp = 0, Wp = 0;
  int Kp = 0;
  int Fp = 32;
  int cfg = 0;

  float* d_w_init = nullptr;
  float* d_w_init_t = nullptr;
  float* d_ep_init = nullptr;
  unsigned short* d_w3_init = nullptr;
  std::vector<float*> d_w_dual;
  std::vector<float*> d_ep_dual;
  std::vector<unsigned short*> d_w3_dual;
  std::vector<_Float16*> d_w2_dual;
  std::vector<float> w_unscale;
  std::vector<unsigned short*> d_u3_dual;
  std::vector<_Float16*> d_u2_dual;
  std::vector<float> u_unscale;
  std::vector<float*> d_u2_tin;
  std::vector<float*> d_u2_colun;
  std::vector<_Float16*> d_u2c_dual;
  std::vector<float> wino_g1, wino_g0;
  int wino_gemm = 0;
  int wino_live_r = 0, wino_live_c = 0;
  int wino_form = -1;
  void free_u2c() { for (auto& p : d_u2c_dual) if (p) hipFree(p); d_u2c_dual.clear(); wino_g1.clear(); wino_g0.clear(); }
  int build_wino_h2_weights();
  int wino_tm = 4;
  size_t wino_v_cap = 0;
  float* d_wV = nullptr;
  float* d_wM = nullptr;
  int wino_chunk_cap = 0;
  int build_wino_weights();
  unsigned* d_amax = nullptr;
  size_t amax_cap = 0;
  int compute_mode = AGZ_COMPUTE_F32_MFMA;
  bool compute_force = false;
  float* d_head_conv = nullptr;
  float* d_head_bn = nullptr;
  float* d_Wp = nullptr;
  float* d_bp = nullptr;
  float* d_W1 = nullptr;
  float* d_b1 = nullptr;
  float* d_W2 = nullptr;
  float* d_b2 = nullptr;

  int max_batch = 0;
  float* d_act_in = nullptr;
  float* d_actA = nullptr;
  float* d_actB = nullptr;
  float* d_planes = nullptr;
  float* d_policy = nullptr;
  float* d_value = nullptr;
  float* d_ws = nullptr;
  std::vector<std::vector<float>> h_ep_dual;
  std::vector<float> h_ep_init;
  std::vector<float*> d_ep_h2;
  float* d_ep_init_h2 = nullptr;
  std::vector<_Float16*> d_lat_w2;
  std::vector<float*> d_lat_tin, d_lat_colun;
  float* d_lat_wmax[2] = {nullptr, nullptr};
  int lat_wmax_cap = 0;
  size_t ws_cap = 0;
  float* d_hs = nullptr;
  size_t hs_cap = 0;
  const float* last_tower = nullptr;
  int last_tower_B = 0;
  int path_input = 0, path_block = 0, path_heads = 0;
  int tower_queues = 0;
  bool latency_mode = true;

  int ensure_batch(int B);
  void free_device();
  int forward_dev(const float* planes_dev, int B, float* policy_dev, float* value_dev);
  int forward_packed(int B, float* policy_dev, float* value_dev);
  struct FwdPlan { bool half_init, half_dual, small, forced_split, latency, heads_spread, split_ok, heads_nb, wino_wide; };
  FwdPlan fwd_plan(int B) const;
  int min_same_batch(int n, int G) const;
  struct H2Tower { int npos, tpb, chunk, ns, n_scr, form_want; bool chained; size_t v_elems, m_elems, wm_board; };
  H2Tower wino_h2_tower(int B) const;
  int wino_h2_reserve(int B, const H2Tower& t, bool* amax_moved);
  void wino_h2c_block(int l, int B, int b0, int ci, const H2Tower& t, hipStream_t st, float* cur, float* nxt);
  void heads_spread_range(agz::HeadArgs h, bool nb4, int B, int b0, int nb, hipStream_t st);
  bool half_ok(int B) const;
  int forward_half_reserve(int B);
  int forward_half(int B, int half, hipStream_t st, float* policy_dev, float* value_dev, hipEvent_t mid);
};
```

### include/agz_debug.h

```cpp
#ifndef AGZ_DEBUG_H
#define AGZ_DEBUG_H

#include "agz.h"

#ifdef __cplusplus
extern "C" {
#endif

#define AGZ_PROF_CONV 0
#define AGZ_PROF_HEADS 1
#define AGZ_PROF_SELECT 2
#define AGZ_PROF_EXPAND 3
#define AGZ_PROF_MOVE 4
#define AGZ_PROF_CONV_INIT 5
#define AGZ_PROF_WINO_IN 6
#define AGZ_PROF_WINO_GEMM 7
#define AGZ_PROF_WINO_OUT 8
#define AGZ_PROF_NCLASS 9
int agz_ctx_prof_enable(agz_ctx* ctx, int enable);
int agz_ctx_prof_read(agz_ctx* ctx, int klass, int64_t* launches, double* total_ms);
int agz_ctx_prof_set_stride(agz_ctx* ctx, int klass, int stride);

int agz_wino_stages(agz_ctx* ctx, const float* x, const float* w, int B, int H, int W, int C, int N, float* V, float* M);

int agz_wino_h2_tile(int H, int W);

int agz_wino_h2_chained(int H, int W, int K);

int agz_net_set_wino_h2_form(agz_net* net, int form);

int agz_net_set_wino_h2_gemm(agz_net* net, int variant);

int agz_net_wino_h2_last_rows(agz_net* net, int* live_r, int* live_c);

int agz_arena_set_prep_compact(agz_arena* arena, int on);
int agz_arena_last_prep_batch(agz_arena* arena, int* boards, int* roots);

int agz_arena_set_cap_compact(agz_arena* arena, int on);
int agz_arena_last_cap_batch(agz_arena* arena, int* boards, int* games);

int agz_arena_set_split(agz_arena* arena, int mode);
int agz_arena_split_steps(agz_arena* arena, int64_t* split, int64_t* joined, int* last_split);

int agz_trainer_set_dma_forward(agz_trainer* t, int on);

#define AGZ_PATH_FWD_F32 1
#define AGZ_PATH_FWD_BF16X3 2
#define AGZ_PATH_FWD_H2W 3
#define AGZ_PATH_FWD_H2DMA 4
#define AGZ_PATH_FWD_H2DMA3 5
#define AGZ_PATH_WGRAD_F32 1
#define AGZ_PATH_WGRAD_X3 2
#define AGZ_PATH_WGRAD_H2 3
#define AGZ_PATH_WGRAD_H2T3 4
#define AGZ_PATH_DGRAD_RAW 1
#define AGZ_PATH_DGRAD_X3 2
#define AGZ_PATH_DGRAD_WINO_H2 3
#define AGZ_PATH_BN2_SCALAR 1
#define AGZ_PATH_BN2_V 2
int agz_trainer_last_paths(agz_trainer* t, int layer, int* fwd, int* wgrad, int* dgrad, int* bn_bwd2);

#define AGZ_ROWS_WGRAD_CHUNKS 0
#define AGZ_ROWS_SINGLE_PASS 1
#define AGZ_ROWS_APPLY_RPB 2
#define AGZ_ROWS_BWD2_RPB 3
#define AGZ_ROWS_APPLY_BOARD_WORDS 4
#define AGZ_ROWS_BWD2_BOARD_WORDS 5
#define AGZ_ROWS_SPLIT_BLOCKS 6
#define AGZ_ROWS_SPLIT_NEED 7
#define AGZ_ROWS_HEAD_SECOND_FORM 0
#define AGZ_ROWS_HEAD_CONV2_GRID 1
#define AGZ_ROWS_HEAD_STATS_GRID 2
#define AGZ_ROWS_HEAD_COST_GRID 3
int agz_trainer_last_rows(agz_trainer* t, int layer, int32_t out[8]);

int agz_trainer_last_planes(agz_trainer* t, int layer, int* fused, uint32_t* est_bits, uint32_t* range_bits);

#define AGZ_NPATH_IN_LAT 1
#define AGZ_NPATH_IN_X3 2
#define AGZ_NPATH_IN_F32_411 3
#define AGZ_NPATH_IN_F32_221 4
#define AGZ_NPATH_IN_F32_222 5
#define AGZ_NPATH_BLK_F32_411 1
#define AGZ_NPATH_BLK_F32_221 2
#define AGZ_NPATH_BLK_F32_222 3
#define AGZ_NPATH_BLK_F32_411_SPLITK 4
#define AGZ_NPATH_BLK_F32_221_SPLITK 5
#define AGZ_NPATH_BLK_F32_222_SPLITK 6
#define AGZ_NPATH_BLK_X3 7
#define AGZ_NPATH_BLK_H2W 8
#define AGZ_NPATH_BLK_H2 9
#define AGZ_NPATH_BLK_WINO 10
#define AGZ_NPATH_BLK_WINO_H2_3K 11
#define AGZ_NPATH_BLK_WINO_H2_3K_WIDE 12
#define AGZ_NPATH_BLK_WINO_H2_CHAINED 13
#define AGZ_NPATH_BLK_LAT_H2 14
#define AGZ_NPATH_HEADS_ONE 1
#define AGZ_NPATH_HEADS_SPREAD 2
#define AGZ_NPATH_HEADS_SPREAD_NB4 3
int agz_net_last_paths(agz_net* net, int* input_conv, int* block, int* heads);

int agz_net_tower_out(agz_net* net, int B, float* host);

int agz_net_min_same_batch(agz_net* net, int n, int G, int* batch);

#define AGZ_CNT_PATHMAX 15
int agz_arena_debug_counter(agz_arena* arena, int which, int64_t* value);

int agz_arena_pool_capacity(agz_arena* arena, int* nodes_per_pool, int* grows);

int agz_arena_set_ckpt_staging(agz_arena* arena, size_t bytes);

int agz_replay_set_ckpt_staging(agz_replay* rp, size_t bytes);

int agz_comm_debug_fail_slice(agz_comm* comm, int k);

int agz_comm_debug_fail_layer(agz_comm* comm, int layer);

#ifdef __cplusplus
}
#endif
#endif
```

Baseline: 44590.

## Optimize tower ends: fused last-layer output, zero-lo input conv, 4-pixel heads feature

The last Winograd layer now runs through the fused oip output kernel with a LAST variant. That variant skips the amax and scale computation for the next layer and writes fp32 results straight to the padded activation. The input 3x3 conv gains a block-level check: if the low 16 bits of every input word in its receptive window are zero, it runs a hi-only bf16 path that skips the low-piece work. The heads feature kernel now handles 4 pixels per wave so weight loads are reused across them. A mask knob can turn each piece off, and a debug counter records how often the skip fires.

```diff
diff --git a/agogo_amd/capi.py b/agogo_amd/capi.py
--- a/agogo_amd/capi.py
+++ b/agogo_amd/capi.py
@@ -324,6 +324,8 @@
     sig("agz_wino_h2_tile", i32, i32, i32)
     sig("agz_net_set_wino_h2_form", i32, vp, i32)
     sig("agz_net_set_wino_h2_gemm", i32, vp, i32)
+    sig("agz_net_set_tower_ends", i32, vp, i32)
+    sig("agz_net_tower_ends_last", i32, vp, C.POINTER(C.c_int64), C.POINTER(C.c_int64))
     sig("agz_net_wino_h2_last_rows", i32, vp, C.POINTER(C.c_int), C.POINTER(C.c_int))
     sig("agz_net_last_paths", i32, vp, C.POINTER(C.c_int), C.POINTER(C.c_int), C.POINTER(C.c_int))
     sig("agz_net_tower_out", i32, vp, i32, pf)
@@ -539,6 +541,14 @@
     def set_wino_h2_gemm(self, variant):
         _check(lib().agz_net_set_wino_h2_gemm(self.h, int(variant)), "agz_net_set_wino_h2_gemm")
 
+    def set_tower_ends(self, mask):
+        _check(lib().agz_net_set_tower_ends(self.h, int(mask)), "agz_net_set_tower_ends")
+
+    def tower_ends_last(self):
+        s, f = C.c_int64(0), C.c_int64(0)
+        _check(lib().agz_net_tower_ends_last(self.h, C.byref(s), C.byref(f)), "agz_net_tower_ends_last")
+        return s.value, f.value
+
     def wino_h2_last_rows(self):
         r, c = C.c_int(0), C.c_int(0)
         _check(lib().agz_net_wino_h2_last_rows(self.h, C.byref(r), C.byref(c)), "agz_net_wino_h2_last_rows")
diff --git a/agogo_amd/csrc/conv_wino_h2c.hpp b/agogo_amd/csrc/conv_wino_h2c.hpp
--- a/agogo_amd/csrc/conv_wino_h2c.hpp
+++ b/agogo_amd/csrc/conv_wino_h2c.hpp
@@ -546,6 +546,13 @@
   o[3] = d12 + 0.125f * d34 + 8.f * m[5];
   o[4] = s12 + 0.0625f * s34 + 16.f * m[5] + m[6];
 }
+template <int TM> __device__ __forceinline__ void wino_atv_p_plain(const f2c* m, f2c* o) { wino_atv_p<TM>(m, o); }
+template <> __device__ __forceinline__ void wino_atv_p_plain<4>(const f2c* m, f2c* o) {
+  o[0] = m[0] + m[1] + m[2] + m[3] + m[4];
+  o[1] = m[1] - m[2] + 2.f * m[3] - 2.f * m[4];
+  o[2] = m[1] + m[2] + 4.f * m[3] + 4.f * m[4];
+  o[3] = m[1] - m[2] + 8.f * m[3] - 8.f * m[4] + m[5];
+}
 template <int TM> __device__ __forceinline__ void wino_at_acc_p(int nu, f2c* Y, f2c t);
 template <> __device__ __forceinline__ void wino_at_acc_p<5>(int nu, f2c* Y, f2c t) {
   switch (nu) {
@@ -595,7 +602,7 @@
   for (int i = 0; i < TM + 2; i++) o[i] = wino_bt_row_p<TM>(i, d);
 }
 
-template <int TM, bool NT = true>
+template <int TM, bool NT = true, bool LAST = false>
 __global__ __launch_bounds__(256, 2) void wino_oip_h2c_kernel(WinoH2Args h) {
   constexpr int MAUX = 0, VAUX = NT ? 2 : 0;
   using WT = WinoT<TM>;
@@ -685,8 +692,8 @@
 #pragma unroll
         for (int xi = 0; xi < AL; xi++) m[nu % NPRE][xi] = h2_ldf4<MAUX>(mr, m_voff(g, xi, nu + NPRE), m_soff(g, s, xi, nu + NPRE));
       }
-      wino_atv_p<TM>(c0, o0);
-      wino_atv_p<TM>(c1, o1);
+      if constexpr (LAST) { wino_atv_p_plain<TM>(c0, o0); wino_atv_p_plain<TM>(c1, o1); }
+      else { wino_atv_p<TM>(c0, o0); wino_atv_p<TM>(c1, o1); }
 #pragma unroll
       for (int k = 0; k < TM; k++) {
         f2c y0[TM], y1[TM];
@@ -733,25 +740,28 @@
       }
       __builtin_amdgcn_sched_barrier(0);
     }
-#pragma unroll
-    for (int o = 8; o > 0; o >>= 1) mxv = fmaxf(mxv, __shfl_xor(mxv, o, 64));
-    if (pr == 0 && live) h.wm_out[(size_t)t * NS + s] = mxv;
-    float ax;
-    if (h.amax_true) ax = __uint_as_float(reinterpret_cast<const unsigned*>(h.amax_true)[b]);
-    else {
-      const int wmpb = a.TPB * NS;
-      const float* wp = h.wm_prev + (size_t)b * wmpb;
-      ax = 0.f;
-      for (int i = pr; i < wmpb; i += 16) ax = fmaxf(ax, wp[i]);
-#pragma unroll
-      for (int o = 8; o > 0; o >>= 1) ax = fmaxf(ax, __shfl_xor(ax, o, 64));
-    }
-    const float bound = h.g1 * ax + h.g0;
-    const unsigned bbits = __float_as_uint(bound);
-    if (s == 0 && tt == 0 && pr == 0 && live) h.amax_next[b] = bbits;
-    float sb, inv_;
-    wino_h2_scales(bbits, WT::VSHIFT, &sb, &inv_);
-    const float sv = live ? sb : 0.f;
+    float sv = 0.f;
+    if constexpr (!LAST) {
+#pragma unroll
+      for (int o = 8; o > 0; o >>= 1) mxv = fmaxf(mxv, __shfl_xor(mxv, o, 64));
+      if (pr == 0 && live) h.wm_out[(size_t)t * NS + s] = mxv;
+      float ax;
+      if (h.amax_true) ax = __uint_as_float(reinterpret_cast<const unsigned*>(h.amax_true)[b]);
+      else {
+        const int wmpb = a.TPB * NS;
+        const float* wp = h.wm_prev + (size_t)b * wmpb;
+        ax = 0.f;
+        for (int i = pr; i < wmpb; i += 16) ax = fmaxf(ax, wp[i]);
+#pragma unroll
+        for (int o = 8; o > 0; o >>= 1) ax = fmaxf(ax, __shfl_xor(ax, o, 64));
+      }
+      const float bound = h.g1 * ax + h.g0;
+      const unsigned bbits = __float_as_uint(bound);
+      if (s == 0 && tt == 0 && pr == 0 && live) h.amax_next[b] = bbits;
+      float sb, inv_;
+      wino_h2_scales(bbits, WT::VSHIFT, &sb, &inv_);
+      sv = live ? sb : 0.f;
+    }
     __syncthreads();
     {
       const int nx = item + (int)gridDim.x < n_items ? item + (int)gridDim.x : item;
@@ -762,6 +772,19 @@
         for (int xi = 0; xi < AL; xi++) m[nu][xi] = h2_ldf4<MAUX>(mr, m_voff(g2, xi, nu), m_soff(g2, s2, xi, nu));
     }
     __builtin_amdgcn_sched_barrier(0);
+    if constexpr (LAST) {
+      const int HW = a.H * a.W, npix = bpg * HW, q4 = (tid & 7) * 4;
+      for (int i = tid >> 3; i < npix; i += 32) {
+        const int blb = i / HW, p = i - blb * HW, hh = p / a.W, ww = p - hh * a.W;
+        const int bb = g * bpg + blb;
+        if (bb < a.B) {
+          const float4 v = *reinterpret_cast<const float4*>(ys + ((size_t)blb * PH * PW + (size_t)(hh + 1) * PW + ww + 1) * 32 + q4);
+          *reinterpret_cast<float4*>(a.y + (((size_t)bb * a.Hp + hh + 1) * a.Wp + ww + 1) * a.Cout_p + 32 * s + q4) = v;
+        }
+      }
+      __syncthreads();
+      continue;
+    }
     const unsigned v_pos = (unsigned)NS * 16384u;
     const unsigned v_slot = (unsigned)h.npos * v_pos;
     const unsigned rg0_r = maps::pack_group_rg0(S_r, g, gr_r), rg0_c = maps::pack_group_rg0(S_c, g, gr_c);
@@ -865,7 +888,9 @@
 static bool wino_h2c_oip_ready(agz_ctx* ctx) {
   if (!(ctx->func_attr_state & 2u)) {
     const bool ok = hipFuncSetAttribute(reinterpret_cast<const void*>(&wino_oip_h2c_kernel<5>), hipFuncAttributeMaxDynamicSharedMemorySize, 80 * 1024) == hipSuccess &&
-                    hipFuncSetAttribute(reinterpret_cast<const void*>(&wino_oip_h2c_kernel<4>), hipFuncAttributeMaxDynamicSharedMemorySize, 80 * 1024) == hipSuccess;
+                    hipFuncSetAttribute(reinterpret_cast<const void*>(&wino_oip_h2c_kernel<4>), hipFuncAttributeMaxDynamicSharedMemorySize, 80 * 1024) == hipSuccess &&
+                    hipFuncSetAttribute(reinterpret_cast<const void*>(&wino_oip_h2c_kernel<5, true, true>), hipFuncAttributeMaxDynamicSharedMemorySize, 80 * 1024) == hipSuccess &&
+                    hipFuncSetAttribute(reinterpret_cast<const void*>(&wino_oip_h2c_kernel<4, true, true>), hipFuncAttributeMaxDynamicSharedMemorySize, 80 * 1024) == hipSuccess;
     if (!ok) (void)hipGetLastError();
     ctx->func_attr_state |= 2u | (ok ? 1u : 0u);
   }
@@ -924,17 +949,22 @@
     default: hipLaunchKernelGGL((wino_gemm_h2c_kernel<16, 2>), g, dim3(256), 0, st, h); break;
   }
 }
-static void wino_h2c_oi(agz_ctx* ctx, WinoH2Args& h, bool last, hipStream_t st, int variant = 4) {
+static void wino_h2c_oi(agz_ctx* ctx, WinoH2Args& h, bool last, hipStream_t st, int variant = 4, bool last_plain = false) {
   wino_h2c_geometry(h);
   ProfScopeOn ps(ctx, AGZ_PROF_WINO_OUT, st == ctx->stream.raw());
   const WinoArgs& a = h.w;
   const dim3 g((unsigned)ceil_div(a.T, 16), (unsigned)(a.C >> 5));
   const size_t shm = last ? 0 : (size_t)(16 / a.TPB) * a.H * a.W * 32 * sizeof(float);
   const bool fits31 = wino_h2c_fits31(h);
-  if (variant == 4 && !last && fits31 && wino_h2c_oip_ready(ctx)) {
+  if (variant == 4 && !(last && last_plain) && fits31 && wino_h2c_oip_ready(ctx)) {
     const size_t shp = (size_t)(16 / a.TPB) * (h.tm * a.nty + 2) * (h.tm * a.ntx + 2) * 32 * sizeof(float);
     const int items = ceil_div(a.T, 16) * (a.C >> 5);
     const dim3 gp((unsigned)std::min(items, 2 * ctx->num_cus));
+    if (last) {
+      if (h.tm == 5) hipLaunchKernelGGL((wino_oip_h2c_kernel<5, true, true>), gp, dim3(256), shp, st, h);
+      else hipLaunchKernelGGL((wino_oip_h2c_kernel<4, true, true>), gp, dim3(256), shp, st, h);
+      return;
+    }
     if (h.tm == 5 && h.temporal_stores) {
       (void)hipFuncSetAttribute(reinterpret_cast<const void*>(&wino_oip_h2c_kernel<5, false>), hipFuncAttributeMaxDynamicSharedMemorySize, 80 * 1024);
       hipLaunchKernelGGL((wino_oip_h2c_kernel<5, false>), gp, dim3(256), shp, st, h);
diff --git a/agogo_amd/csrc/conv_x3.hpp b/agogo_amd/csrc/conv_x3.hpp
--- a/agogo_amd/csrc/conv_x3.hpp
+++ b/agogo_amd/csrc/conv_x3.hpp
@@ -68,7 +68,7 @@
   } \
   if (!DUAL && a.amax_out && amx_b >= 0) x3_amax_flush(a.amax_out, amx_b, amx_m, lane);
 
-template <bool DUAL>
+template <bool DUAL, bool ZS = false>
 __global__ __launch_bounds__(256, 3) void conv3x3_x3_kernel(ConvArgs a, const unsigned short* __restrict__ w3) {
   constexpr int BM = 128, BNT = 128;
   constexpr int PIECE = 128 * 32;
@@ -188,14 +188,65 @@
     __syncthreads();                                                                         \
   }
 
-  X3_GLOAD(ya0, ya1, yb0, yb1, yb2)
-  X3_GLOAD(xa0, xa1, xb0, xb1, xb2)
-  X3_STORE_A(ya0, ya1, 0)
-  X3_STORE_B(yb0, yb1, yb2, 0)
+#define X3_PROLOGUE()                     \
+  X3_GLOAD(ya0, ya1, yb0, yb1, yb2)       \
+  X3_GLOAD(xa0, xa1, xb0, xb1, xb2)       \
+  X3_STORE_A(ya0, ya1, 0)                 \
+  X3_STORE_B(yb0, yb1, yb2, 0)            \
   __syncthreads();
-  for (int it = 0; it < NK; it += 2) {
-    X3_ITER(0, xa0, xa1, xb0, xb1, xb2, ya0, ya1, yb0, yb1, yb2)
-    if (it + 1 < NK) X3_ITER(1, ya0, ya1, yb0, yb1, yb2, xa0, xa1, xb0, xb1, xb2)
+  bool skip_ = false;
+  if constexpr (!DUAL && ZS) {
+    {
+      int ml = m0 + BM - 1 < a.M ? m0 + BM - 1 : a.M - 1;
+      const int b0 = m0 / a.HW, p0 = m0 - b0 * a.HW, h0 = p0 / a.W, w0 = p0 - h0 * a.W;
+      const int b1 = ml / a.HW, p1 = ml - b1 * a.HW, h1 = p1 / a.W, w1 = p1 - h1 * a.W;
+      const int q0 = (b0 * a.HpWp + (h0 + 1) * a.Wp + (w0 + 1) - a.Wp - 1) * (a.Cin_p >> 2);
+      const int q1 = (b1 * a.HpWp + (h1 + 1) * a.Wp + (w1 + 1) + a.Wp + 2) * (a.Cin_p >> 2);
+      const u32x4_t* x4 = reinterpret_cast<const u32x4_t*>(a.x);
+      unsigned or_ = 0u;
+      for (int q = q0 + tid; q < q1; q += 256) { const u32x4_t v = x4[q]; or_ |= v[0] | v[1] | v[2] | v[3]; }
+      skip_ = __syncthreads_or((int)(or_ & 0xffffu)) == 0;
+    }
+  }
+  if (__builtin_expect(skip_, 1)) {
+#define X3_STORE_A_HI(A0, A1, BUF)                                                           \
+  {                                                                                          \
+    u32x4_t ph_ = {x3_pack(__float_as_uint(A0.x), __float_as_uint(A0.y)), x3_pack(__float_as_uint(A0.z), __float_as_uint(A0.w)),   \
+                   x3_pack(__float_as_uint(A1.x), __float_as_uint(A1.y)), x3_pack(__float_as_uint(A1.z), __float_as_uint(A1.w))};  \
+    *reinterpret_cast<u32x4_t*>(lds + (BUF) * STAGE + s_off) = ph_;                          \
+  }
+#define X3_ITER_HI(BUF, XA0, XA1, XB0, XB1, XB2, YA0, YA1, YB0, YB1, YB2)                    \
+  {                                                                                          \
+    const unsigned char* st = lds + (BUF) * STAGE;                                           \
+    bf16x8_t A_[2][1], B_[2][3];                                                             \
+    _Pragma("unroll") for (int i = 0; i < 2; i++) A_[i][0] = *reinterpret_cast<const bf16x8_t*>(st + fa[i]);                       \
+    _Pragma("unroll") for (int p = 0; p < 3; p++) {                                          \
+      _Pragma("unroll") for (int j = 0; j < 2; j++) B_[j][p] = *reinterpret_cast<const bf16x8_t*>(st + (3 + p) * PIECE + fb[j]);   \
+    }                                                                                        \
+    X3_GLOAD(YA0, YA1, YB0, YB1, YB2)                                                        \
+    X3_QUAD(0, 2)                                                                            \
+    X3_STORE_A_HI(XA0, XA1, (BUF) ^ 1)                                                       \
+    X3_STORE_B(XB0, XB1, XB2, (BUF) ^ 1)                                                     \
+    X3_QUAD(0, 1) X3_QUAD(0, 0)                                                              \
+    __syncthreads();                                                                         \
+  }
+    X3_PROLOGUE()
+    for (int it = 0; it < NK; it += 2) {
+      X3_ITER_HI(0, xa0, xa1, xb0, xb1, xb2, ya0, ya1, yb0, yb1, yb2)
+      if (it + 1 < NK) X3_ITER_HI(1, ya0, ya1, yb0, yb1, yb2, xa0, xa1, xb0, xb1, xb2)
+    }
+#undef X3_ITER_HI
+#undef X3_STORE_A_HI
+  } else {
+    X3_PROLOGUE()
+    for (int it = 0; it < NK; it += 2) {
+      X3_ITER(0, xa0, xa1, xb0, xb1, xb2, ya0, ya1, yb0, yb1, yb2)
+      if (it + 1 < NK) X3_ITER(1, ya0, ya1, yb0, yb1, yb2, xa0, xa1, xb0, xb1, xb2)
+    }
+  }
+#undef X3_PROLOGUE
+  if constexpr (!DUAL && ZS) {
+    if (a.cnt && tid == 0 && skip_) atomicAdd(a.cnt, (unsigned long long)NK);
   }
 
   X3_EPILOGUE
diff --git a/agogo_amd/csrc/net.hip b/agogo_amd/csrc/net.hip
--- a/agogo_amd/csrc/net.hip
+++ b/agogo_amd/csrc/net.hip
@@ -27,6 +27,7 @@
   float w_unscale;
   const unsigned* w_amax_dev;
   unsigned* amax_out;
+  unsigned long long* cnt;
 };
 
 __device__ __forceinline__ int swz_off(int row, int chunk) { return row * 32 + ((chunk ^ ((row >> 1) & 7)) << 2); }
@@ -426,6 +427,20 @@
   if (tid == 0) a.value[b] = tanhf(red[0] + red[1] + red[2] + red[3] + a.b2[0]);
 }
 
+__device__ __forceinline__ void heads_feat_dot(const float4 xv, const float4 w0, const float4 w1, const float4 w2, float& s0, float& s1, float& s2) {
+#pragma clang fp contract(off)
+  s0 = s0 + (((xv.x * w0.x + xv.y * w0.y) + xv.z * w0.z) + xv.w * w0.w);
+  s1 = s1 + __builtin_fmaf(xv.w, w1.w, __builtin_fmaf(xv.z, w1.z, __builtin_fmaf(xv.x, w1.x, xv.y * w1.y)));
+  s2 = s2 + __builtin_fmaf(xv.w, w2.w, __builtin_fmaf(xv.z, w2.z, __builtin_fmaf(xv.y, w2.y, xv.x * w2.x)));
+}
+__device__ __forceinline__ void heads_feat_store(const HeadArgs& a, float* f, int p, float s0, float s1, float s2) {
+  const float v0 = __builtin_fmaf(s0, a.bn[(0 * a.HW + p) * 2], a.bn[(0 * a.HW + p) * 2 + 1]);
+  const float v1 = __builtin_fmaf(s1, a.bn[(1 * a.HW + p) * 2], a.bn[(1 * a.HW + p) * 2 + 1]);
+  const float v2 = __builtin_fmaf(s2, a.bn[(2 * a.HW + p) * 2], a.bn[(2 * a.HW + p) * 2 + 1]);
+  f[p] = v0 > 0.f ? v0 : 0.f;
+  f[a.HW + p] = v1 > 0.f ? v1 : 0.f;
+  f[2 * a.HW + p] = v2 > 0.f ? v2 : 0.f;
+}
 __global__ __launch_bounds__(256) void heads_feat_kernel(HeadArgs a) {
   const int b = blockIdx.y, lane = threadIdx.x & 63, p = blockIdx.x * 4 + (threadIdx.x >> 6);
   if (p >= a.HW) return;
@@ -437,19 +452,39 @@
     float4 w0 = *reinterpret_cast<const float4*>(a.conv + c);
     float4 w1 = *reinterpret_cast<const float4*>(a.conv + a.Kp + c);
     float4 w2 = *reinterpret_cast<const float4*>(a.conv + 2 * a.Kp + c);
-    s0 += xv.x * w0.x + xv.y * w0.y + xv.z * w0.z + xv.w * w0.w;
-    s1 += xv.x * w1.x + xv.y * w1.y + xv.z * w1.z + xv.w * w1.w;
-    s2 += xv.x * w2.x + xv.y * w2.y + xv.z * w2.z + xv.w * w2.w;
+    heads_feat_dot(xv, w0, w1, w2, s0, s1, s2);
   }
   s0 = wave_sum(s0); s1 = wave_sum(s1); s2 = wave_sum(s2);
+  if (lane == 0) heads_feat_store(a, a.feat + (size_t)b * 3 * a.HW, p, s0, s1, s2);
+}
+__global__ __launch_bounds__(256) void heads_feat4_kernel(HeadArgs a) {
+  const int b = blockIdx.y, lane = threadIdx.x & 63, p0 = (blockIdx.x * 4 + (threadIdx.x >> 6)) * 4;
+  if (p0 >= a.HW) return;
+  const float* xp[4];
+#pragma unroll
+  for (int u = 0; u < 4; u++) {
+    const int p = p0 + u < a.HW ? p0 + u : a.HW - 1;
+    const int h = p / a.W, w = p - h * a.W;
+    xp[u] = a.x + ((size_t)b * a.HpWp + (h + 1) * a.Wp_ + (w + 1)) * a.Kp;
+  }
+  float s0[4] = {0.f, 0.f, 0.f, 0.f}, s1[4] = {0.f, 0.f, 0.f, 0.f}, s2[4] = {0.f, 0.f, 0.f, 0.f};
+  for (int c = lane * 4; c < a.Kp; c += 256) {
+    float4 xs[4];
+#pragma unroll
+    for (int u = 0; u < 4; u++) xs[u] = *reinterpret_cast<const float4*>(xp[u] + c);
+    const float4 w0 = *reinterpret_cast<const float4*>(a.conv + c);
+    const float4 w1 = *reinterpret_cast<const float4*>(a.conv + a.Kp + c);
+    const float4 w2 = *reinterpret_cast<const float4*>(a.conv + 2 * a.Kp + c);
+#pragma unroll
+    for (int u = 0; u < 4; u++) heads_feat_dot(xs[u], w0, w1, w2, s0[u], s1[u], s2[u]);
+  }
+#pragma unroll
+  for (int u = 0; u < 4; u++) { s0[u] = wave_sum(s0[u]); s1[u] = wave_sum(s1[u]); s2[u] = wave_sum(s2[u]); }
   if (lane == 0) {
     float* f = a.feat + (size_t)b * 3 * a.HW;
-    float v0 = s0 * a.bn[(0 * a.HW + p) * 2] + a.bn[(0 * a.HW + p) * 2 + 1];
-    float v1 = s1 * a.bn[(1 * a.HW + p) * 2] + a.bn[(1 * a.HW + p) * 2 + 1];
-    float v2 = s2 * a.bn[(2 * a.HW + p) * 2] + a.bn[(2 * a.HW + p) * 2 + 1];
-    f[p] = v0 > 0.f ? v0 : 0.f;
-    f[a.HW + p] = v1 > 0.f ? v1 : 0.f;
-    f[2 * a.HW + p] = v2 > 0.f ? v2 : 0.f;
+#pragma unroll
+    for (int u = 0; u < 4; u++)
+      if (p0 + u < a.HW) heads_feat_store(a, f, p0 + u, s0[u], s1[u], s2[u]);
   }
 }
 __global__ __launch_bounds__(1024) void heads_fc_kernel(HeadArgs a) {
@@ -598,6 +633,7 @@
   for (auto& p : d_w2_dual) if (p) { hipFree(p); p = nullptr; }
   if (d_amax) { hipFree(d_amax); d_amax = nullptr; }
   amax_cap = 0;
+  if (d_ends_cnt) { hipFree(d_ends_cnt); d_ends_cnt = nullptr; }
   for (auto& p : d_u3_dual) if (p) { hipFree(p); p = nullptr; }
   for (auto& p : d_u2_dual) if (p) { hipFree(p); p = nullptr; }
   d_u2_dual.clear();
@@ -1134,14 +1170,23 @@
   }
   if (l == 0) agz::wino_h2c_in(ctx, hh, st);
   agz::wino_h2c_gemm(ctx, hh, st);
-  agz::wino_h2c_oi(ctx, hh, last, st, t.form_want == 1 ? 1 : 4);
+  agz::wino_h2c_oi(ctx, hh, last, st, t.form_want == 1 ? 1 : 4, (tower_ends & 1) != 0);
+}
+
+void agz_net::launch_input_x3(agz::ConvArgs& a, hipStream_t st) {
+  const dim3 g(a.n_mtiles * a.n_ntiles);
+  a.cnt = (tower_ends & 8) ? d_ends_cnt : nullptr;
+  if (a.cnt) ends_steps += (int64_t)g.x * 9 * (a.Cin_p >> 4);
+  if (tower_ends & 2) hipLaunchKernelGGL((conv3x3_x3_kernel<false>), g, dim3(256), 0, st, a, d_w3_init);
+  else hipLaunchKernelGGL((conv3x3_x3_kernel<false, true>), g, dim3(256), 0, st, a, d_w3_init);
 }
 
 void agz_net::heads_spread_range(agz::HeadArgs h, bool nb4, int B, int b0, int nb, hipStream_t st) {
   h.x += (size_t)b0 * Hp * Wp * Kp;
   h.feat = d_hs + (size_t)b0 * 3 * HW; h.cols = d_hs + (size_t)B * 3 * HW + (size_t)b0 * (conf.ActionSpace + conf.FC);
   h.policy += (size_t)b0 * conf.ActionSpace; h.value += b0;
-  hipLaunchKernelGGL(heads_feat_kernel, dim3(ceil_div(HW, 4), nb), dim3(256), 0, st, h);
+  if (tower_ends & 4) hipLaunchKernelGGL(heads_feat_kernel, dim3(ceil_div(HW, 4), nb), dim3(256), 0, st, h);
+  else hipLaunchKernelGGL(heads_feat4_kernel, dim3(ceil_div(HW, 16), nb), dim3(256), 0, st, h);
   if (nb4)
     hipLaunchKernelGGL(heads_fc_nb_kernel<4>, dim3(ceil_div(conf.ActionSpace + conf.FC, 64), ceil_div(nb, 4)), dim3(1024), 0, st, h, nb);
   else
@@ -1190,7 +1235,7 @@
   a.splits = 1; a.per = 0; a.ws = nullptr; a.raw = 0;
   AGZ_HIP_TRY(hipMemsetAsync(d_amax + b0, 0, (size_t)nb * sizeof(unsigned), st));
   a.amax_out = d_amax + b0;
-  hipLaunchKernelGGL((conv3x3_x3_kernel<false>), dim3(a.n_mtiles * a.n_ntiles), dim3(256), 0, st, a, d_w3_init);
+  launch_input_x3(a, st);
   const int L = conf.SharedLayers;
   for (int l = 0; l < L; l++) {
     wino_h2c_block(l, B, b0, half, t, st, d_actA, d_actB);
@@ -1260,7 +1305,7 @@
       AGZ_HIP_TRY(hipMemsetAsync(d_amax, 0, (size_t)B * sizeof(unsigned), ctx->stream));
       a.amax_out = d_amax; amax0_done = true;
     }
-    hipLaunchKernelGGL((conv3x3_x3_kernel<false>), dim3(a.n_mtiles * a.n_ntiles), dim3(256), 0, ctx->stream, a, d_w3_init);
+    launch_input_x3(a, ctx->stream);
     a.amax_out = nullptr;
     path_input = AGZ_NPATH_IN_X3;
     rc = AGZ_OK;
@@ -1839,6 +1884,31 @@
   return AGZ_OK;
 }
 
+int agz_net_set_tower_ends(agz_net* n, int mask) {
+  AGZ_REQUIRE(n, AGZ_E_INVALID, "agz_net_set_tower_ends: null net");
+  AGZ_REQUIRE(mask >= 0 && mask <= 15, AGZ_E_INVALID, "agz_net_set_tower_ends: mask %d (want bits 0 .. 3)", mask);
+  AGZ_HIP_TRY(hipSetDevice(n->ctx->device));
+  AGZ_HIP_TRY(hipDeviceSynchronize());
+  if ((mask & 8) && !n->d_ends_cnt) AGZ_HIP_TRY(hipMalloc(&n->d_ends_cnt, sizeof(unsigned long long)));
+  if (n->d_ends_cnt) AGZ_HIP_TRY(hipMemset(n->d_ends_cnt, 0, sizeof(unsigned long long)));
+  n->ends_steps = 0;
+  n->tower_ends = mask;
+  return AGZ_OK;
+}
+
+int agz_net_tower_ends_last(agz_net* n, int64_t* steps_skipped, int64_t* steps_full) {
+  AGZ_REQUIRE(n && steps_skipped && steps_full, AGZ_E_INVALID, "agz_net_tower_ends_last: null argument");
+  unsigned long long skipped = 0;
+  if (n->d_ends_cnt) {
+    AGZ_HIP_TRY(hipSetDevice(n->ctx->device));
+    AGZ_HIP_TRY(hipDeviceSynchronize());
+    AGZ_HIP_TRY(hipMemcpy(&skipped, n->d_ends_cnt, sizeof(skipped), hipMemcpyDeviceToHost));
+  }
+  *steps_skipped = (int64_t)skipped;
+  *steps_full = n->ends_steps - (int64_t)skipped;
+  return AGZ_OK;
+}
+
 int agz_wino_stages(agz_ctx* ctx, const float* x, const float* w, int B, int H, int W, int C, int N, float* V, float* M) {
   AGZ_REQUIRE(ctx && x && w && V && M, AGZ_E_INVALID, "agz_wino_stages: NULL argument");
   AGZ_REQUIRE(B >= 1 && H >= 1 && W >= 1 && C >= 16 && C % 16 == 0 && N >= 1, AGZ_E_INVALID, "agz_wino_stages: bad shape");
diff --git a/agogo_amd/csrc/net.hpp b/agogo_amd/csrc/net.hpp
--- a/agogo_amd/csrc/net.hpp
+++ b/agogo_amd/csrc/net.hpp
@@ -35,6 +35,7 @@
 bool conv3x3_raw_wino_h2_fits(int B, int H, int W, int Cin_p, int Cout_p);
 void wino_raw_scratch_free(WinoRawScratch* sc);
 struct HeadArgs;
+struct ConvArgs;
 }
 
 struct agz_net {
@@ -67,6 +68,9 @@
   std::vector<float> wino_g1, wino_g0;
   int wino_gemm = 0;
   int wino_live_r = 0, wino_live_c = 0;
+  int tower_ends = 0;
+  unsigned long long* d_ends_cnt = nullptr;
+  int64_t ends_steps = 0;
   int wino_form = -1;
   void free_u2c() { for (auto& p : d_u2c_dual) if (p) hipFree(p); d_u2c_dual.clear(); wino_g1.clear(); wino_g0.clear(); }
   int build_wino_h2_weights();
@@ -125,6 +129,7 @@
   H2Tower wino_h2_tower(int B) const;
   int wino_h2_reserve(int B, const H2Tower& t, bool* amax_moved);
   void wino_h2c_block(int l, int B, int b0, int ci, const H2Tower& t, hipStream_t st, float* cur, float* nxt);
+  void launch_input_x3(agz::ConvArgs& a, hipStream_t st);
   void heads_spread_range(agz::HeadArgs h, bool nb4, int B, int b0, int nb, hipStream_t st);
   bool half_ok(int B) const;
   int forward_half_reserve(int B);
diff --git a/include/agz_debug.h b/include/agz_debug.h
--- a/include/agz_debug.h
+++ b/include/agz_debug.h
@@ -30,6 +30,9 @@
 int agz_net_set_wino_h2_form(agz_net* net, int form);
 
 int agz_net_set_wino_h2_gemm(agz_net* net, int variant);
+
+int agz_net_set_tower_ends(agz_net* net, int mask);
+int agz_net_tower_ends_last(agz_net* net, int64_t* steps_skipped, int64_t* steps_full);
 
 int agz_net_wino_h2_last_rows(agz_net* net, int* live_r, int* live_c);
 
```

Result: no change. 44850 (median of 6 runs) (+0.6%).
